# NazirNayal8/RbA

Hardware: AMD Instinct MI355X
Metric: images/sec @1024x2048 Swin-B-1dl (RbA inference hot path) (higher is better)
Workload: dtype f32 (f16x3 split-MFMA GEMMs, fp32 accumulate)

## Files before the change

### include/rba_hip.h

```cpp
#ifndef RBA_HIP_H
#define RBA_HIP_H

#include <stdint.h>

#ifdef __cplusplus
extern "C" {
#endif

int rba_hip_version(void);

int rba_set_concurrent_streams(int n);

int rba_reduce_f32(const float* mask, const float* cls_prob, float* rba, float* sem_seg, int32_t* argmax,
                   int Q, int K, int64_t HW, int score_mode, void* stream);

int rba_reduce_ws_f32(const float* mask, const float* cls_prob, float* rba, float* sem_seg, int32_t* argmax, int Q, int K,
                      int64_t HW, int score_mode, void* workspace, void* stream);

int rba_reduce_up4_f32(const float* mask_lowres, const float* cls_prob, float* rba, float* sem_seg,
                       int32_t* argmax, int Q, int K, int h, int w, int crop_h, int crop_w, int score_mode, void* stream);

int rba_reduce_bwd_workspace_f32(int Q, int K, int64_t HW, int64_t* bytes);
int rba_reduce_bwd_f32(const float* mask, const float* cls_prob, const float* grad_score,
                       float* grad_mask , float* grad_prob ,
                       int Q, int K, int64_t HW, int score_mode,
                       void* workspace, int64_t workspace_bytes, void* stream);

int rba_resample_bilinear_f32(const float* in, const float* add, float* out, int C, int h, int w, int H, int W,
                              void* stream);

int rba_ms_deform_attn_fwd_f32(const float* value, const int64_t* spatial_shapes, const int64_t* level_start_index,
                               const float* sampling_loc, const float* attn_weight, float* out,
                               int N, int S, int M, int D, int L, int Lq, int P, void* stream);
int rba_ms_deform_attn_fwd_f64(const double* value, const int64_t* spatial_shapes, const int64_t* level_start_index,
                               const double* sampling_loc, const double* attn_weight, double* out,
                               int N, int S, int M, int D, int L, int Lq, int P, void* stream);

int rba_ms_deform_attn_bwd_f32(const float* value, const int64_t* spatial_shapes, const int64_t* level_start_index,
                               const float* sampling_loc, const float* attn_weight, const float* grad_out,
                               float* grad_value, float* grad_sampling_loc, float* grad_attn_weight,
                               int N, int S, int M, int D, int L, int Lq, int P, void* stream);
int rba_ms_deform_attn_bwd_f64(const double* value, const int64_t* spatial_shapes, const int64_t* level_start_index,
                               const double* sampling_loc, const double* attn_weight, const double* grad_out,
                               double* grad_value, double* grad_sampling_loc, double* grad_attn_weight,
                               int N, int S, int M, int D, int L, int Lq, int P, void* stream);

int rba_msda_prepare_f32(const float* raw, const float* reference_points, const int64_t* spatial_shapes, float* loc, float* attw,
                         int64_t rows, int M, int L, int P, void* stream);

int rba_msda_fused_f32(const float* value, const int64_t* spatial_shapes, const int64_t* level_start_index, const float* raw,
                       const float* reference_points, float* out, int N, int S, int M, int D, int L, int Lq, int P, void* stream);

int64_t rba_masked_xattn_workspace_bytes(int B, int Q, int S, int nH);
int rba_masked_xattn_f32(const float* q, const float* k, const float* v, const float* mask_logits, float* out,
                         float* workspace, int B, int Q, int S, int nH, int hd, void* stream);

int rba_mask_logits_f32(const float* embed, const float* feat, float* out, int B, int Q, int C, int64_t N,
                        void* stream);
int rba_mask_logits_f16x3_f32(const float* embed, const float* feat, float* out, int B, int Q, int C, int64_t N,
                              void* stream);

int rba_mask_logits_bwd_workspace_f32(int B, int Q, int C, int64_t N, int64_t* bytes);
int rba_mask_logits_bwd_f32(const float* embed, const float* feat, const float* grad_out,
                            float* grad_embed , float* grad_feat ,
                            int B, int Q, int C, int64_t N, void* workspace, int64_t workspace_bytes, void* stream);

int rba_point_sample_f32(const float* planes, const int64_t* plane_index , const float* coords, float* out,
                         int64_t num_planes, int N, int h, int w, int P, int shared_coords, void* stream);

int rba_mask_point_loss_fwd_f32(const float* pred_masks, const int64_t* plane_index, const float* coords, const float* labels,
                                float* sums, float* losses, int64_t num_planes, int N, int h, int w, int P, float num_masks, void* stream);
int rba_mask_point_loss_bwd_f32(const float* pred_masks, const int64_t* plane_index, const float* coords, const float* labels,
                                const float* sums, const float* grad_loss_mask , const float* grad_loss_dice ,
                                float* grad_masks, int64_t num_planes, int N, int h, int w, int P, float num_masks, void* stream);

int rba_match_cost_workspace_f32(int Q, int T, int P, int64_t* bytes);
int rba_match_cost_f32(const float* pred_masks, const float* tgt_masks, const float* coords, const float* cls_prob, const int64_t* tgt_ids,
                       float* cost, int Q, int T, int P, int h, int w, int H, int W, int K1, float w_mask, float w_class, float w_dice,
                       void* workspace, int64_t workspace_bytes, void* stream);

int rba_swin_window_attn_f32(const float* qkv, const float* qkv_bias, const float* bias, const float* bias_frag,
                             float* out, int B, int H, int W, int nH, int hd, int ws, int shift, void* stream);
int64_t rba_swin_bias_fragments_elems(int nH, int ws);
int rba_swin_bias_fragments_f32(const float* bias, float* frag, int nH, int ws, void* stream);

int64_t rba_group_norm_workspace_bytes(int B, int C, int HW, int G);
int rba_group_norm_f32(const float* x, const float* gamma, const float* beta, float* y, float* workspace,
                       int B, int C, int HW, int G, float eps, int relu, void* stream);

int64_t rba_group_norm_nhwc_workspace_bytes(int B, int P, int C, int G);
int rba_group_norm_nhwc_f32(const float* x, const float* gamma, const float* beta, float* y, float* workspace, int B, int P, int C,
                            int G, float eps, int relu, void* stream);
int rba_resample_bilinear_nhwc_f32(const float* in, const float* add, float* out, int C, int h, int w, int H, int W, void* stream);

int rba_add_layer_norm_f32(const float* x, const float* t, const float* t_bias, const float* gamma, const float* beta,
                           float* sum_out, float* y, int64_t rows, int C, float eps, void* stream);

int rba_merge_layer_norm_f32(const float* x, const float* gamma, const float* beta, float* y, int B, int H, int W, int Cin, float eps,
                             void* stream);

int rba_skinny_linear_f32(const float* x, const float* weight, const float* bias, float* out, int M, int N, int K,
                          int relu, void* stream);
int rba_skinny_linear_add_f32(const float* x, const float* x_add, int add_cols, const float* weight, const float* bias, float* out,
                              int M, int N, int K, int relu, int seg_n, void* stream);

int rba_split_weight_bf16x3(const float* weight, void* packed, int N, int K, void* stream);
int rba_split_linear_f32(const float* x, const void* weight_packed, const float* bias, float* out, int64_t M, int N, int K,
                         int act, void* stream);

int rba_split_weight_f16x2(const float* weight, void* packed, int N, int K, void* stream);
int rba_split_linear_f16x3_f32(const float* x, const void* weight_packed, const float* bias, float* out, int64_t M, int N, int K,
                               int act, void* stream);
int rba_split_linear_f16x3_res_f32(const float* x, const void* weight_packed, const float* bias, const float* residual, float* out,
                                   int64_t M, int N, int K, void* stream);

int rba_add_layer_norm_frag_f32(const float* x, const float* t, const float* t_bias, const float* gamma, const float* beta,
                                float* sum_out, void* y_frag, int64_t rows, int C, float eps, void* stream);
int rba_split_linear_f16x3_frag_f32(const void* x_frag, const void* weight_packed, const float* bias, const float* residual, float* out,
                                    int64_t M, int N, int K, int act, void* stream);
int rba_swin_window_attn_split_out_f32(const float* qkv, const float* qkv_bias, const float* bias_frag, void* out_frag, int B, int H, int W,
                                       int nH, int hd, int ws, int shift, void* stream);
int rba_swin_attn_block_supported(int C, int ws);
int64_t rba_swin_attn_block_weight_bytes(int C);
int rba_swin_attn_block_pack_f32(const float* qkv_weight, const float* proj_weight, void* image, int C, void* stream);
int rba_swin_attn_block_f32(float* x, float* y2, const float* norm1_weight, const float* norm1_bias, float eps1, const void* weight_image,
                            const float* qkv_bias, const float* bias_frag, const float* proj_bias, const float* norm2_weight,
                            const float* norm2_bias, float eps2, int B, int H, int W, int C, int ws, int shift, void* stream);
int rba_swin_attn_qkv_supported(int C, int ws);
int rba_swin_attn_qkv_split_out_f32(const float* x, void* out_frag, const float* norm1_weight, const float* norm1_bias, float eps1,
                                    const void* weight_image, const float* qkv_bias, const float* bias_frag, int B, int H, int W, int C, int ws,
                                    int shift, void* stream);
int rba_resample_bilinear_nhwc_split_out_f32(const float* in, const float* add, void* out_frag, int C, int h, int w, int H, int W,
                                             int64_t row0, void* stream);

int rba_resample_bilinear_nhwc_gn_f32(const float* in, const float* in_mr, const float* in_gamma, const float* in_beta, int in_relu,
                                      const float* add, const float* add_mr, const float* add_gamma, const float* add_beta, void* out,
                                      int split_out, int C, int G, int h, int w, int H, int W, int64_t row0, void* stream);
int rba_group_norm_nhwc_stats_f32(const float* x, float* mr, float* workspace, int B, int P, int C, int G, float eps, void* stream);
int rba_conv3x3_nhwc_f16x3_split_in_f32(const void* x_frag, const void* weight_packed, const float* bias, float* out, int B, int H, int W,
                                        int C, int N, void* stream);
int rba_swin_mlp_fused_f16x3_f32(const float* x, const void* w1_packed, const float* b1, const void* w2_packed, const float* b2,
                                 const float* residual, float* out, int64_t M, int C, int HID, void* stream);
int rba_swin_mlp_fused_ln_f16x3_f32(float* x, const float* norm_weight, const float* norm_bias, float eps, const void* w1_packed, const float* b1,
                                    const void* w2_packed, const float* b2, int64_t M, int C, int HID, void* stream);
int rba_split_linear_f16x3_gelu_split_out(const void* x, int x_is_split, const void* weight_packed, const float* bias, void* out_frag,
                                          int64_t M, int N, int K, void* stream);

int rba_split_linear_nchw_out_f32(const float* x, const void* weight_packed, const float* bias, float* out, int64_t M, int N,
                                  int K, int rows_per_image, void* stream);

int rba_split_linear_nchw_out_f16x3_f32(const float* x, const void* weight_packed, const float* bias, float* out, int64_t M, int N, int K,
                                        int rows_per_image, void* stream);

int rba_split_linear_nchw_out_gn_f16x3_f32(const float* x, const float* mr, const float* gamma, const float* beta, int G, int relu,
                                           const void* weight_packed, const float* bias, float* out, int64_t M, int N, int K,
                                           int rows_per_image, void* stream);

int rba_conv3x3_nhwc_f32(const float* x, const void* weight_packed, const float* bias, float* out, int B, int H, int W, int C,
                         int N, void* stream);

int rba_conv3x3_nhwc_f16x3_f32(const float* x, const void* weight_packed, const float* bias, float* out, int B, int H, int W, int C,
                               int N, void* stream);

int rba_split_linear_f16x3_gn_moments_f32(const float* x, const void* weight_packed, const float* bias, float* out, int64_t M, int N, int K,
                                          int rows_per_image, int G, float* moments, void* stream);
int rba_conv3x3_nhwc_f16x3_split_in_gn_moments_f32(const void* x_frag, const void* weight_packed, const float* bias, float* out, int B, int H,
                                                   int W, int C, int N, int G, float* moments, void* stream);
int rba_group_norm_nhwc_merge_f32(const float* moments, float* mr, int B, int G, int splits, float eps, void* stream);

int rba_patch_im2col_u8(const uint8_t* image, float* out, int h, int w, int Hp, int Wp, const float* mean, const float* std, void* stream);
int rba_patch_im2col_f32(const float* image, float* out, int h, int w, int Hp, int Wp, const float* mean, const float* std, void* stream);

int rba_gaussian_blur_f32(const float* in, float* out, int H, int W, int kernel_size, float sigma, void* stream);

int rba_quad_mean_f32(const float* v, float* out, int64_t rows, int S, void* stream);
int rba_softmax_drop_last_f32(const float* logits, float* prob, int64_t rows, int K1, void* stream);

int rba_threshold_u8(const float* score, uint8_t* out, int64_t n, float threshold, void* stream);
int rba_morph3x3_u8(const uint8_t* in, uint8_t* out, int H, int W, int dilate, void* stream);
int rba_ccl4_roots_i32(const uint8_t* mask, int32_t* roots, int H, int W, void* stream);

int rba_bn_relu_conv1x1_f32(const float* x, const float* scale, const float* shift, const float* weight, const float* bias, float* out,
                            int B, int C, int O, int64_t P, void* stream);
int rba_resample_bilinear_ac_f32(const float* x, float* out, int C, int h, int w, int H, int W, void* stream);

typedef struct {
  const float* x_add;
  const void* packed;
  const float* bias;
  float* out;
  int N;
  int ld_out;
  int act;
} rba_token_linear_problem;
int rba_token_linear_pack_f16x2(const float* weight, void* packed, int N, int K, void* stream);
int rba_token_linear_f32(const float* x, const float* x_add, const void* packed, const float* bias, const float* residual,
                         const float* ln_weight, const float* ln_bias, float ln_eps, float* out, int64_t M, int N, int K, int act,
                         void* stream);
int rba_token_linear_multi_f32(const float* x, const rba_token_linear_problem* problems, int n_problems, int64_t M, int K, void* stream);

#ifdef __cplusplus
}
#endif
#endif
```

### rba_amd/_lib.py

```python
import ctypes
import os

_HERE = os.path.dirname(os.path.abspath(__file__))
LIB_PATH = os.environ.get("RBA_HIP_LIB") or os.path.join(_HERE, "csrc", "librba_hip.so")
KNOBS_LIB_PATH = os.path.join(_HERE, "csrc", "librba_hip_knobs.so")

_i = ctypes.c_int
_i64 = ctypes.c_int64
_vp = ctypes.c_void_p

SIGNATURES = {
    "rba_hip_version": [],
    "rba_set_concurrent_streams": [_i],
    "rba_reduce_f32": [_vp, _vp, _vp, _vp, _vp, _i, _i, _i64, _i, _vp],
    "rba_reduce_ws_f32": [_vp, _vp, _vp, _vp, _vp, _i, _i, _i64, _i, _vp, _vp],
    "rba_reduce_up4_f32": [_vp, _vp, _vp, _vp, _vp, _i, _i, _i, _i, _i, _i, _i, _vp],
    "rba_reduce_bwd_workspace_f32": [_i, _i, _i64, _vp],
    "rba_reduce_bwd_f32": [_vp, _vp, _vp, _vp, _vp, _i, _i, _i64, _i, _vp, _i64, _vp],
    "rba_resample_bilinear_f32": [_vp, _vp, _vp, _i, _i, _i, _i, _i, _vp],
    "rba_ms_deform_attn_fwd_f32": [_vp, _vp, _vp, _vp, _vp, _vp, _i, _i, _i, _i, _i, _i, _i, _vp],
    "rba_ms_deform_attn_fwd_f64": [_vp, _vp, _vp, _vp, _vp, _vp, _i, _i, _i, _i, _i, _i, _i, _vp],
    "rba_ms_deform_attn_bwd_f32": [_vp, _vp, _vp, _vp, _vp, _vp, _vp, _vp, _vp, _i, _i, _i, _i, _i, _i, _i, _vp],
    "rba_ms_deform_attn_bwd_f64": [_vp, _vp, _vp, _vp, _vp, _vp, _vp, _vp, _vp, _i, _i, _i, _i, _i, _i, _i, _vp],
    "rba_msda_prepare_f32": [_vp, _vp, _vp, _vp, _vp, _i64, _i, _i, _i, _vp],
    "rba_resample_bilinear_nhwc_gn_f32": [_vp, _vp, _vp, _vp, _i, _vp, _vp, _vp, _vp, _vp, _i, _i, _i, _i, _i, _i, _i, _i64, _vp],
    "rba_group_norm_nhwc_stats_f32": [_vp, _vp, _vp, _i, _i, _i, _i, ctypes.c_float, _vp],
    "rba_msda_fused_f32": [_vp, _vp, _vp, _vp, _vp, _vp, _i, _i, _i, _i, _i, _i, _i, _vp],
    "rba_masked_xattn_workspace_bytes": [_i, _i, _i, _i],
    "rba_masked_xattn_f32": [_vp, _vp, _vp, _vp, _vp, _vp, _i, _i, _i, _i, _i, _vp],
    "rba_mask_logits_f32": [_vp, _vp, _vp, _i, _i, _i, _i64, _vp],
    "rba_mask_logits_f16x3_f32": [_vp, _vp, _vp, _i, _i, _i, _i64, _vp],
    "rba_mask_logits_bwd_workspace_f32": [_i, _i, _i, _i64, _vp],
    "rba_mask_logits_bwd_f32": [_vp, _vp, _vp, _vp, _vp, _i, _i, _i, _i64, _vp, _i64, _vp],
    "rba_point_sample_f32": [_vp, _vp, _vp, _vp, _i64, _i, _i, _i, _i, _i, _vp],
    "rba_mask_point_loss_fwd_f32": [_vp, _vp, _vp, _vp, _vp, _vp, _i64, _i, _i, _i, _i, ctypes.c_float, _vp],
    "rba_mask_point_loss_bwd_f32": [_vp, _vp, _vp, _vp, _vp, _vp, _vp, _vp, _i64, _i, _i, _i, _i, ctypes.c_float, _vp],
    "rba_match_cost_workspace_f32": [_i, _i, _i, _vp],
    "rba_match_cost_f32": [_vp, _vp, _vp, _vp, _vp, _vp, _i, _i, _i, _i, _i, _i, _i, _i, ctypes.c_float, ctypes.c_float, ctypes.c_float, _vp, _i64, _vp],
    "rba_swin_window_attn_f32": [_vp, _vp, _vp, _vp, _vp, _i, _i, _i, _i, _i, _i, _i, _vp],
    "rba_swin_window_attn_split_out_f32": [_vp, _vp, _vp, _vp, _i, _i, _i, _i, _i, _i, _i, _vp],
    "rba_swin_bias_fragments_elems": [_i, _i],
    "rba_swin_attn_block_supported": [_i, _i],
    "rba_swin_attn_block_weight_bytes": [_i],
    "rba_swin_attn_qkv_supported": [_i, _i],
    "rba_swin_attn_qkv_split_out_f32": [_vp, _vp, _vp, _vp, ctypes.c_float, _vp, _vp, _vp, _i, _i, _i, _i, _i, _i, _vp],
    "rba_swin_attn_block_pack_f32": [_vp, _vp, _vp, _i, _vp],
    "rba_swin_attn_block_f32": [_vp, _vp, _vp, _vp, ctypes.c_float, _vp, _vp, _vp, _vp, _vp, _vp, ctypes.c_float, _i, _i, _i, _i, _i, _i, _vp],
    "rba_swin_bias_fragments_f32": [_vp, _vp, _i, _i, _vp],
    "rba_skinny_linear_f32": [_vp, _vp, _vp, _vp, _i, _i, _i, _i, _vp],
    "rba_skinny_linear_add_f32": [_vp, _vp, _i, _vp, _vp, _vp, _i, _i, _i, _i, _i, _vp],
    "rba_split_weight_bf16x3": [_vp, _vp, _i, _i, _vp],
    "rba_split_linear_f32": [_vp, _vp, _vp, _vp, _i64, _i, _i, _i, _vp],
    "rba_split_weight_f16x2": [_vp, _vp, _i, _i, _vp],
    "rba_split_linear_f16x3_f32": [_vp, _vp, _vp, _vp, _i64, _i, _i, _i, _vp],
    "rba_split_linear_f16x3_res_f32": [_vp, _vp, _vp, _vp, _vp, _i64, _i, _i, _vp],
    "rba_split_linear_f16x3_frag_f32": [_vp, _vp, _vp, _vp, _vp, _i64, _i, _i, _i, _vp],
    "rba_swin_mlp_fused_f16x3_f32": [_vp, _vp, _vp, _vp, _vp, _vp, _vp, _i64, _i, _i, _vp],
    "rba_swin_mlp_fused_ln_f16x3_f32": [_vp, _vp, _vp, ctypes.c_float, _vp, _vp, _vp, _vp, _i64, _i, _i, _vp],
    "rba_split_linear_f16x3_gelu_split_out": [_vp, _i, _vp, _vp, _vp, _i64, _i, _i, _vp],
    "rba_split_linear_nchw_out_f32": [_vp, _vp, _vp, _vp, _i64, _i, _i, _i, _vp],
    "rba_split_linear_nchw_out_f16x3_f32": [_vp, _vp, _vp, _vp, _i64, _i, _i, _i, _vp],
    "rba_split_linear_f16x3_gn_moments_f32": [_vp, _vp, _vp, _vp, _i64, _i, _i, _i, _i, _vp, _vp],
    "rba_conv3x3_nhwc_f16x3_split_in_gn_moments_f32": [_vp, _vp, _vp, _vp, _i, _i, _i, _i, _i, _i, _vp, _vp],
    "rba_group_norm_nhwc_merge_f32": [_vp, _vp, _i, _i, _i, ctypes.c_float, _vp],
    "rba_split_linear_nchw_out_gn_f16x3_f32": [_vp, _vp, _vp, _vp, _i, _i, _vp, _vp, _vp, _i64, _i, _i, _i, _vp],
    "rba_conv3x3_nhwc_f32": [_vp, _vp, _vp, _vp, _i, _i, _i, _i, _i, _vp],
    "rba_conv3x3_nhwc_f16x3_f32": [_vp, _vp, _vp, _vp, _i, _i, _i, _i, _i, _vp],
    "rba_conv3x3_nhwc_f16x3_split_in_f32": [_vp, _vp, _vp, _vp, _i, _i, _i, _i, _i, _vp],
    "rba_resample_bilinear_nhwc_split_out_f32": [_vp, _vp, _vp, _i, _i, _i, _i, _i, _i64, _vp],
    "rba_patch_im2col_u8": [_vp, _vp, _i, _i, _i, _i, _vp, _vp, _vp],
    "rba_patch_im2col_f32": [_vp, _vp, _i, _i, _i, _i, _vp, _vp, _vp],
    "rba_group_norm_nhwc_workspace_bytes": [_i, _i, _i, _i],
    "rba_group_norm_nhwc_f32": [_vp, _vp, _vp, _vp, _vp, _i, _i, _i, _i, ctypes.c_float, _i, _vp],
    "rba_resample_bilinear_nhwc_f32": [_vp, _vp, _vp, _i, _i, _i, _i, _i, _vp],
    "rba_bn_relu_conv1x1_f32": [_vp, _vp, _vp, _vp, _vp, _vp, _i, _i, _i, _i64, _vp],
    "rba_resample_bilinear_ac_f32": [_vp, _vp, _i, _i, _i, _i, _i, _vp],
    "rba_gaussian_blur_f32": [_vp, _vp, _i, _i, _i, ctypes.c_float, _vp],
    "rba_quad_mean_f32": [_vp, _vp, _i64, _i, _vp],
    "rba_softmax_drop_last_f32": [_vp, _vp, _i64, _i, _vp],
    "rba_threshold_u8": [_vp, _vp, _i64, ctypes.c_float, _vp],
    "rba_morph3x3_u8": [_vp, _vp, _i, _i, _i, _vp],
    "rba_ccl4_roots_i32": [_vp, _vp, _i, _i, _vp],
    "rba_add_layer_norm_f32": [_vp, _vp, _vp, _vp, _vp, _vp, _vp, _i64, _i, ctypes.c_float, _vp],
    "rba_add_layer_norm_frag_f32": [_vp, _vp, _vp, _vp, _vp, _vp, _vp, _i64, _i, ctypes.c_float, _vp],
    "rba_merge_layer_norm_f32": [_vp, _vp, _vp, _vp, _i, _i, _i, _i, ctypes.c_float, _vp],
    "rba_group_norm_workspace_bytes": [_i, _i, _i, _i],
    "rba_group_norm_f32": [_vp, _vp, _vp, _vp, _vp, _i, _i, _i, _i, ctypes.c_float, _i, _vp],
    "rba_token_linear_pack_f16x2": [_vp, _vp, _i, _i, _vp],
    "rba_token_linear_f32": [_vp, _vp, _vp, _vp, _vp, _vp, _vp, ctypes.c_float, _vp, _i64, _i, _i, _i, _vp],
    "rba_token_linear_multi_f32": [_vp, _vp, _i, _i64, _i, _vp],
}

class TokenLinearProblem(ctypes.Structure):
    _fields_ = [("x_add", ctypes.c_void_p), ("packed", ctypes.c_void_p), ("bias", ctypes.c_void_p), ("out", ctypes.c_void_p),
                ("N", ctypes.c_int), ("ld_out", ctypes.c_int), ("act", ctypes.c_int)]


EXPECTED_ABI = 191

_lib = None


class RbaHipError(RuntimeError):
    pass


def load():
    global _lib
    if _lib is not None:
        return _lib
    _lib = _open(LIB_PATH)
    return _lib


_handles = {}


def _open(path):
    if path in _handles:
        return _handles[path]
    import torch
    if not os.path.exists(path):
        raise RbaHipError(
            f"{path} not found: build it with `python -m rba_amd.csrc.build` (hipcc --offload-arch=gfx950; --knobs for the knobs build). "
            "rba_amd has no CPU or PyTorch fallback for its HIP kernels.")
    lib = ctypes.CDLL(path)
    for name, argtypes in SIGNATURES.items():
        try:
            fn = getattr(lib, name)
        except AttributeError as e:
            raise RbaHipError(f"{path} does not export {name}; rebuild it") from e
        fn.argtypes = argtypes
        fn.restype = ctypes.c_int64 if name.endswith(("_bytes", "_elems")) else ctypes.c_int
    abi = int(lib.rba_hip_version())
    if abi != EXPECTED_ABI:
        raise RbaHipError(f"{path} has ABI version {abi}, these bindings are written for {EXPECTED_ABI}; rebuild it "
                          "(python -m rba_amd.csrc.build)")
    _handles[path] = lib
    return lib


class use_library:

    def __init__(self, path):
        self.path = path

    def __enter__(self):
        global _lib
        self.prev = _lib
        _lib = _open(self.path)
        return _lib

    def __exit__(self, *exc):
        global _lib
        _lib = self.prev
        return False


def knob(name):
    try:
        return ctypes.c_int.in_dll(load(), name)
    except ValueError as e:
        raise RbaHipError(f"{name} is a compile-time constant in the product library: run on the knobs build (RBA_HIP_LIB={KNOBS_LIB_PATH} or "
                          "rba_amd._lib.use_library(KNOBS_LIB_PATH); python -m rba_amd.csrc.build --knobs)") from e


def hip_error_string(code: int) -> str:
    try:
        hip = ctypes.CDLL("libamdhip64.so")
        hip.hipGetErrorString.restype = ctypes.c_char_p
        hip.hipGetErrorString.argtypes = [ctypes.c_int]
        return hip.hipGetErrorString(code).decode()
    except Exception:
        return "hipError"


def check(code: int, what: str):
    if code != 0:
        raise RbaHipError(f"{what} failed: hipError {code} ({hip_error_string(code)})")
```

### rba_amd/csrc/split_linear_dma.hip

```cpp
#include "split_linear_h3.h"
#include "split_linear_h3q.h"
#include "mlp_fused_h3.h"

RBA_KNOB(rba_k6_variant, 0);
RBA_KNOB_DEFINE(rba_k6_stagger, 0);
RBA_KNOB_DEFINE(rba_k6_occ, 2);
RBA_KNOB_DEFINE(rba_k6_rs_min_k, 512);
RBA_KNOB_DEFINE(rba_k6_ks, 0);
RBA_KNOB_DEFINE(rba_k6_rs, 0);
extern "C" __attribute__((visibility("hidden"))) int rba_concurrent_streams_hint = 1;

extern "C" int rba_set_concurrent_streams(int n) {
  const int prev = rba_concurrent_streams_hint;
  rba_concurrent_streams_hint = n >= 1 ? n : 1;
  return prev;
}

extern "C" int rba_split_linear_f32(const float* x, const void* weight_planes, const float* bias, float* out, int64_t M, int N,
                                    int K, int act, void* stream) {
  RBA_CHECK_ARG(N >= 1 && act >= 0 && act <= 2);
  RBA_GEMM_PROLOGUE(M, K, x && weight_planes && out, x, weight_planes, out);
  const u32x4_t* wp = reinterpret_cast<const u32x4_t*>(weight_planes);
  hipStream_t st = (hipStream_t)stream;
  return rba_gemm_status((tiles128(M, N) < 256 && N > 64 && (K >> 5) >= 2) ? launch_v5_act<1, 2, 2, 2, 4>(act, x, wp, bias, out, M, N, K, 2, st)
                                                                           : launch_v4_act<1, 4, 1, 2, 4>(act, x, wp, bias, out, M, N, K, st));
}

extern "C" int rba_split_weight_f16x2(const float* weight, void* packed, int N, int K, void* stream) {
  RBA_CHECK_ARG(N >= 0 && K >= 0 && (K % 32) == 0);
  if (N == 0 || K == 0) return 0;
  RBA_CHECK_ARG(weight && packed && (((uintptr_t)weight | (uintptr_t)packed) & 15) == 0);
  rba_begin();
  const int64_t total = (int64_t)((N + 127) >> 7) * (K >> 4) * 256;
  const unsigned grid = (unsigned)((total + 255) / 256 < 4096 ? (total + 255) / 256 : 4096);
  hipLaunchKernelGGL(split_weight_f16x2_kernel, dim3(grid), dim3(256), 0, (hipStream_t)stream, weight, reinterpret_cast<u32x4_t*>(packed),
                     N, K);
  return rba_launch_status();
}

extern "C" int rba_split_linear_f16x3_f32(const float* x, const void* weight_packed, const float* bias, float* out, int64_t M, int N,
                                          int K, int act, void* stream) {
  RBA_CHECK_ARG(N >= 1 && act >= 0 && act <= 2);
  RBA_GEMM_PROLOGUE(M, K, x && weight_packed && out, x, weight_packed, out);
  const H3Args a{x, reinterpret_cast<const u32x4_t*>(weight_packed), bias, out, M, N, K, (hipStream_t)stream};
  return rba_gemm_status(h3_with_act(act, [&](auto ACT) { return launch_h3_rows<ACT, 0>(a); }));
}

extern "C" int rba_conv3x3_nhwc_f16x3_f32(const float* x, const void* weight_packed, const float* bias, float* out, int B, int H, int W,
                                          int C, int N, void* stream) {
  RBA_CHECK_ARG(B >= 0 && H >= 1 && W >= 1 && N >= 1);
  const int64_t M = (int64_t)B * H * W;
  RBA_GEMM_PROLOGUE(M, C, x && weight_packed && out && M * C < (int64_t)1 << 30, x, weight_packed, out);
  H3Args a{x, reinterpret_cast<const u32x4_t*>(weight_packed), bias, out, M, N, 9 * C, (hipStream_t)stream};
  a.cs = ConvShape{H, W, C};
  return rba_gemm_status((tiles128(M, N) >= 256 || N <= 64) ? launch_h3l<0, 4, H3_CONV>(a) : launch_h3l<0, 2, H3_CONV>(a));
}

extern "C" int rba_split_linear_f16x3_gn_moments_f32(const float* x, const void* weight_packed, const float* bias, float* out, int64_t M, int N, int K,
                                                     int rows_per_image, int G, float* moments, void* stream) {
  RBA_CHECK_ARG(N >= 128 && (N % 128) == 0 && K <= 256 && G >= 1 && (N % G) == 0 && rows_per_image >= 128);
  const int cpg = N / G;
  RBA_CHECK_ARG((cpg == 4 || cpg == 8 || cpg == 16 || cpg == 32) && (rows_per_image % 128) == 0);
  RBA_GEMM_PROLOGUE(M, K, x && weight_packed && out && moments && (M % rows_per_image) == 0, x, weight_packed, out);
  H3Args a{x, reinterpret_cast<const u32x4_t*>(weight_packed), bias, out, M, N, K, (hipStream_t)stream};
  a.gm = GnMoments{moments, G, cpg, rows_per_image};
  return rba_gemm_status(launch_h3l<0, 4, H3_GNM>(a));
}

extern "C" int rba_conv3x3_nhwc_f16x3_split_in_gn_moments_f32(const void* x_frag, const void* weight_packed, const float* bias, float* out, int B, int H,
                                                              int W, int C, int N, int G, float* moments, void* stream) {
  RBA_CHECK_ARG(B >= 0 && H >= 1 && W >= 1 && C <= 2048 && N >= 128 && (N % 128) == 0 && G >= 1 && (N % G) == 0);
  const int cpg = N / G;
  const int64_t P = (int64_t)H * W, M = (int64_t)B * P;
  RBA_CHECK_ARG((cpg == 4 || cpg == 8 || cpg == 16 || cpg == 32) && (P % 128) == 0 && P < (int64_t)1 << 31);
  RBA_GEMM_PROLOGUE(M, C, x_frag && weight_packed && out && moments, x_frag, weight_packed, out, bias);
  H3Args a{x_frag, reinterpret_cast<const u32x4_t*>(weight_packed), bias, out, M, N, 9 * C, (hipStream_t)stream};
  a.cs = ConvShape{H, W, C};
  a.gm = GnMoments{moments, G, cpg, (int)P};
  return rba_gemm_status(launch_h3p_by_shape<0, H3_PRE | H3_CONVP | H3_GNM, H3_RS2>(a));
}

extern "C" int rba_split_linear_f16x3_res_f32(const float* x, const void* weight_packed, const float* bias, const float* residual, float* out,
                                              int64_t M, int N, int K, void* stream) {
  RBA_CHECK_ARG(N >= 1);
  RBA_GEMM_PROLOGUE(M, K, x && weight_packed && residual && out, x, weight_packed, out, residual);
  H3Args a{x, reinterpret_cast<const u32x4_t*>(weight_packed), bias, out, M, N, K, (hipStream_t)stream};
  a.res = residual;
  return rba_gemm_status(launch_h3_rows<0, H3_RES>(a));
}

extern "C" int rba_split_linear_f16x3_frag_f32(const void* x_frag, const void* weight_packed, const float* bias, const float* residual,
                                               float* out, int64_t M, int N, int K, int act, void* stream) {
  RBA_CHECK_ARG(N >= 1 && act >= 0 && act <= 2 && !(residual && act));
  RBA_GEMM_PROLOGUE(M, K, x_frag && weight_packed && out, x_frag, weight_packed, out, residual);
  const u32x4_t* wp = reinterpret_cast<const u32x4_t*>(weight_packed);
  hipStream_t st = (hipStream_t)stream;
  int rc;
  const bool sub_tiles = rba_k6_variant == 2 || (rba_k6_variant == 0 && tiles128(M, N) < (residual ? 256 : 200));
  if (sub_tiles && h3q_supported(M, N, K)) {
    rc = residual ? launch_h3q<H3Q_RES, 0>(x_frag, wp, bias, residual, out, M, N, K, st)
                  : h3_with_act(act, [&](auto ACT) { return launch_h3q<H3Q_F32, ACT>(x_frag, wp, bias, nullptr, out, M, N, K, st); });
  } else {
    constexpr unsigned GEOMETRIES = H3_OCC1 | H3_KS2 | H3_RS2;
    H3Args a{x_frag, wp, bias, out, M, N, K, st};
    a.res = residual;
    a.stagger = rba_k6_stagger;
    rc = residual ? launch_h3p_by_shape<0, H3_PRE | H3_RES, GEOMETRIES>(a)
                  : h3_with_act(act, [&](auto ACT) { return launch_h3p_by_shape<ACT, H3_PRE, GEOMETRIES>(a); });
  }
  return rba_gemm_status(rc);
}

extern "C" int rba_split_linear_f16x3_gelu_split_out(const void* x, int x_is_split, const void* weight_packed, const float* bias,
                                                     void* out_frag, int64_t M, int N, int K, void* stream) {
  RBA_CHECK_ARG(N >= 32 && (N % 32) == 0);
  RBA_GEMM_PROLOGUE(M, K, x && weight_packed && out_frag, x, weight_packed, out_frag, bias);
  const u32x4_t* wp = reinterpret_cast<const u32x4_t*>(weight_packed);
  hipStream_t st = (hipStream_t)stream;
  int rc;
  if (x_is_split && rba_k6_variant >= 100 && h3q_supported(M, N, K)) {
    switch (rba_k6_variant - 100) {
#define H3Q_PROBE(P) case P: rc = launch_h3q<H3Q_SPLIT, 1, P>(x, wp, bias, nullptr, out_frag, M, N, K, st); break;
      H3Q_PROBE(1) H3Q_PROBE(2) H3Q_PROBE(4) H3Q_PROBE(8) H3Q_PROBE(16) H3Q_PROBE(3) H3Q_PROBE(7) H3Q_PROBE(15) H3Q_PROBE(31) H3Q_PROBE(5)
#undef H3Q_PROBE
      default: rc = launch_h3q<H3Q_SPLIT, 1>(x, wp, bias, nullptr, out_frag, M, N, K, st);
    }
  } else if (x_is_split && h3q_supported(M, N, K) &&
             (rba_k6_variant == 2 || (rba_k6_variant == 0 && K >= 768 && tiles128(M, N) > 512 && !h3p_use_rs2(M, N, K))))
    rc = launch_h3q<H3Q_SPLIT, 1>(x, wp, bias, nullptr, out_frag, M, N, K, st);
  else {
    H3Args a{x, wp, bias, out_frag, M, N, K, st};
    a.stagger = rba_k6_stagger;
    rc = x_is_split ? launch_h3p_by_shape<1, H3_PRE | H3_FOUT, H3_OCC1 | H3_RS2>(a) : launch_h3p_by_shape<1, H3_FOUT, H3_OCC1>(a);
  }
  return rba_gemm_status(rc);
}

extern "C" int rba_conv3x3_nhwc_f16x3_split_in_f32(const void* x_frag, const void* weight_packed, const float* bias, float* out, int B, int H,
                                                   int W, int C, int N, void* stream) {
  RBA_CHECK_ARG(B >= 0 && H >= 1 && W >= 1 && C <= 2048 && N >= 1);
  const int64_t M = (int64_t)B * H * W;
  RBA_GEMM_PROLOGUE(M, C, x_frag && weight_packed && out, x_frag, weight_packed, out, bias);
  H3Args a{x_frag, reinterpret_cast<const u32x4_t*>(weight_packed), bias, out, M, N, 9 * C, (hipStream_t)stream};
  a.cs = ConvShape{H, W, C};
  return rba_gemm_status(launch_h3p_by_shape<0, H3_PRE | H3_CONVP, H3_RS2>(a));
}

extern "C" int rba_swin_mlp_fused_f16x3_f32(const float* x, const void* w1_packed, const float* b1, const void* w2_packed, const float* b2,
                                            const float* residual, float* out, int64_t M, int C, int HID, void* stream) {
  RBA_CHECK_ARG(C == 128 && HID >= 64 && (HID % 32) == 0);
  RBA_GEMM_PROLOGUE(M, C, x && w1_packed && b1 && w2_packed && residual && out, x, w1_packed, w2_packed, residual, out, b1);
  return rba_gemm_status(launch_mlp_fused(x, reinterpret_cast<const u32x4_t*>(w1_packed), b1, reinterpret_cast<const u32x4_t*>(w2_packed), b2, residual, out, M,
                                          HID, (hipStream_t)stream));
}

extern "C" int rba_swin_mlp_fused_ln_f16x3_f32(float* x, const float* norm_weight, const float* norm_bias, float eps, const void* w1_packed, const float* b1,
                                               const void* w2_packed, const float* b2, int64_t M, int C, int HID, void* stream) {
  RBA_CHECK_ARG(C == 128 && HID >= 64 && (HID % 32) == 0);
  RBA_GEMM_PROLOGUE(M, C, x && norm_weight && norm_bias && w1_packed && b1 && w2_packed, x, w1_packed, w2_packed, b1, norm_weight, norm_bias);
  return rba_gemm_status(launch_mlp_fused(x, reinterpret_cast<const u32x4_t*>(w1_packed), b1, reinterpret_cast<const u32x4_t*>(w2_packed), b2, x, x, M, HID,
                                          (hipStream_t)stream, norm_weight, norm_bias, eps));
}

extern "C" int rba_split_linear_nchw_out_f16x3_f32(const float* x, const void* weight_packed, const float* bias, float* out, int64_t M, int N,
                                                   int K, int rows_per_image, void* stream) {
  RBA_CHECK_ARG(N >= 1 && rows_per_image >= 1);
  RBA_GEMM_PROLOGUE(M, K, x && weight_packed && out && (M % rows_per_image) == 0, x, weight_packed, out);
  H3Args a{x, reinterpret_cast<const u32x4_t*>(weight_packed), bias, out, M, N, K, (hipStream_t)stream};
  a.rows_per_image = rows_per_image;
  return rba_gemm_status(h3_wide(M, N) ? launch_h3l<0, 4, H3_NCHW>(a) : launch_h3l<0, 2, H3_NCHW>(a));
}
```

### rba_amd/csrc/split_linear_gnf.hip

```cpp
#include "split_linear_h3.h"

extern "C" int rba_split_linear_nchw_out_gn_f16x3_f32(const float* x, const float* mr, const float* gamma, const float* beta, int G, int relu,
                                                      const void* weight_packed, const float* bias, float* out, int64_t M, int N, int K,
                                                      int rows_per_image, void* stream) {
  RBA_CHECK_ARG(N >= 1 && rows_per_image >= 1 && G >= 1 && (K % G) == 0 && ((K / G) % 4) == 0);
  RBA_GEMM_PROLOGUE(M, K, x && mr && gamma && beta && weight_packed && out && (M % rows_per_image) == 0 && (rows_per_image % 128) == 0, x, weight_packed, out,
                    gamma, beta);
  H3Args a{x, reinterpret_cast<const u32x4_t*>(weight_packed), bias, out, M, N, K, (hipStream_t)stream};
  a.rows_per_image = rows_per_image;
  a.gn = GnFold{mr, gamma, beta, G, K / G, relu ? 1 : 0};
  return rba_gemm_status(h3_wide(M, N) ? launch_h3l<0, 4, H3_NCHW | H3_GNF>(a) : launch_h3l<0, 2, H3_NCHW | H3_GNF>(a));
}
```

### rba_amd/csrc/split_linear_h3.h

```cpp
#pragma once
#include <type_traits>

#include "split_linear_dma.h"

RBA_KNOB_EXTERN(rba_k6_stagger, 0);

namespace {

typedef _Float16 f16x8_t __attribute__((ext_vector_type(8)));

__device__ __forceinline__ void split_h3(const f32x4 u, const f32x4 v, f16x8_t& h, f16x8_t& l) {
  const float x[8] = {u.x, u.y, u.z, u.w, v.x, v.y, v.z, v.w};
  u32x4_t hp, lp;
#pragma unroll
  for (int i = 0; i < 4; ++i) {
    uint32_t a, r;
    rba_split_f16x2(x[2 * i], x[2 * i + 1], a, r);
    hp[i] = a;
    lp[i] = r;
  }
  h = __builtin_bit_cast(f16x8_t, hp);
  l = __builtin_bit_cast(f16x8_t, lp);
}

__device__ __forceinline__ f32x2 gelu_erf2(f32x2 v) {
  const f32x2 a = {fabsf(v.x), fabsf(v.y)};
  const f32x2 d = a * 0.23164189f + 1.0f;
  const f32x2 t = {__builtin_amdgcn_rcpf(d.x), __builtin_amdgcn_rcpf(d.y)};
  f32x2 p = t * 0.5307027145f + -0.7265760135f;
  p = p * t + 0.7107068705f;
  p = p * t + -0.142248368f;
  p = p * t + 0.127414796f;
  const f32x2 u = a * 0.8493218003f;
  const f32x2 s = -u * u;
  const f32x2 ex = {__builtin_amdgcn_exp2f(s.x), __builtin_amdgcn_exp2f(s.y)};
  const f32x2 q = p * t * ex;
  const f32x2 r = (v + a) * 0.5f;
  return r - a * q;
}

#ifndef RBA_H3_HELPERS_ONLY
__global__ void split_weight_f16x2_kernel(const float* __restrict__ w, u32x4_t* __restrict__ packed, int N, int K) {
  const int S = K >> 4;
  const int64_t total = (int64_t)((N + 127) >> 7) * S * 256;
  for (int64_t i = (int64_t)blockIdx.x * blockDim.x + threadIdx.x; i < total; i += (int64_t)gridDim.x * blockDim.x) {
    const int slot = (int)(i & 1), r = (int)((i >> 1) & 127);
    const int64_t ts = i >> 8;
    const int s = (int)(ts % S), nt = (int)(ts / S);
    const int h = slot ^ ((r >> 3) & 1);
    const int k0 = 32 * (s >> 1) + 16 * h + 8 * (s & 1);
    const int n = nt * 128 + r;
    f16x8_t p0, p1;
    if (n < N) {
      const f32x4* src = reinterpret_cast<const f32x4*>(w + (int64_t)n * K + k0);
      split_h3(src[0], src[1], p0, p1);
    } else {
#pragma unroll
      for (int e = 0; e < 8; ++e) p0[e] = p1[e] = (_Float16)0.f;
    }
    u32x4_t* dst = packed + ts * 512 + r * 2 + slot;
    dst[0] = __builtin_bit_cast(u32x4_t, p0);
    dst[256] = __builtin_bit_cast(u32x4_t, p1);
  }
}

#endif

struct GnMoments {
  float* ws;
  int G, cpg, P;
};
template <int ACT, int CT, int PROBE, bool RES, bool GNM = false>
__device__ __forceinline__ void h3_epilogue(const f32x16_t (&accm)[CT], const f32x16_t (&accl)[CT], const float* __restrict__ bias,
                                            float* C, const float* R, int M, int N, int m0, int n0, int BM, int BN, int wave, int l31,
                                            int lh, GnMoments gm = GnMoments{nullptr, 1, 1, 128}, float* sh = nullptr) {
  const bool interior = m0 + BM <= M && n0 + BN <= N;
  if (GNM) __syncthreads();
#pragma unroll
  for (int j = 0; j < CT; ++j) {
    const int col = n0 + 32 * j + l31;
    const float bv = (bias && col < N) ? bias[col] : 0.f;
    const int rbase = m0 + 32 * wave + 4 * lh;
    float* dst = C + (int64_t)rbase * N + col;
    f32x16_t res;
    if (RES) {
      const float* src = R + (int64_t)rbase * N + col;
#pragma unroll
      for (int r = 0; r < 16; ++r) {
        const int ro = 8 * (r >> 2) + (r & 3);
        res[r] = (interior || (col < N && rbase + ro < M)) ? src[(int64_t)ro * N] : 0.f;
      }
    }
    f32x16_t v;
#pragma unroll
    for (int r = 0; r < 16; r += 2) {
      f32x2 y = (f32x2){accl[j][r], accl[j][r + 1]} * 0.00048828125f + (f32x2){accm[j][r], accm[j][r + 1]};
      if (RES) y = (f32x2){res[r], res[r + 1]} + y;
      y = y + bv;
      if (ACT == 1) y = gelu_erf2(y);
      if (ACT == 2) y = (f32x2){rba_relu(y.x), rba_relu(y.y)};
      v[r] = y.x;
      v[r + 1] = y.y;
    }
    if (GNM) {
      float sm = 0.f, sq = 0.f;
#pragma unroll
      for (int r = 0; r < 16; ++r) {
        sm += v[r];
        sq = fmaf(v[r], v[r], sq);
      }
      sm += __shfl_xor(sm, 32, 64);
      sq += __shfl_xor(sq, 32, 64);
      for (int o = 1; o < gm.cpg; o <<= 1) {
        sm += __shfl_xor(sm, o, 64);
        sq += __shfl_xor(sq, o, 64);
      }
      if (lh == 0 && (l31 & (gm.cpg - 1)) == 0) {
        float* d = sh + ((wave * (BN / gm.cpg)) + (32 * j + l31) / gm.cpg) * 2;
        d[0] = sm;
        d[1] = sq;
      }
    }
    if (PROBE & 4) {
      float sum = 0.f;
#pragma unroll
      for (int r = 0; r < 16; ++r) sum += v[r];
      if (sum == 1234.5f) dst[0] = sum;
    } else if (interior) {
#pragma unroll
      for (int r = 0; r < 16; ++r) dst[(int64_t)(8 * (r >> 2) + (r & 3)) * N] = v[r];
    } else if (col < N) {
#pragma unroll
      for (int r = 0; r < 16; ++r) {
        const int ro = 8 * (r >> 2) + (r & 3);
        if (rbase + ro < M) dst[(int64_t)ro * N] = v[r];
      }
    }
  }
  if (GNM) {
    __syncthreads();
    const int gpt = BN / gm.cpg, t = 64 * wave + 32 * lh + l31;
    if (t < gpt && m0 < M) {
      double ds = 0, dq = 0;
#pragma unroll
      for (int w = 0; w < 4; ++w) {
        ds += (double)sh[(w * gpt + t) * 2];
        dq += (double)sh[(w * gpt + t) * 2 + 1];
      }
      const double n = 128.0 * gm.cpg, mean = ds / n, m2 = dq - ds * mean;
      const int b = m0 / gm.P, sp = (m0 - b * gm.P) >> 7, splits = gm.P >> 7, g = n0 / gm.cpg + t;
      float* o = gm.ws + (((int64_t)b * gm.G + g) * splits + sp) * 3;
      o[0] = (float)n;
      o[1] = (float)mean;
      o[2] = (float)(m2 > 0 ? m2 : 0);
    }
  }
}

#ifndef RBA_H3_HELPERS_ONLY
template <int CT>
__device__ __forceinline__ void h3_epilogue_nchw(const f32x16_t (&accm)[CT], const f32x16_t (&accl)[CT], const float* __restrict__ bias, float* C,
                                                 int M, int N, int P, int m0, int n0, int wave, int l31, int lh) {
  const bool vec = (P & 3) == 0;
#pragma unroll
  for (int j = 0; j < CT; ++j) {
    const int col = n0 + 32 * j + l31;
    if (col >= N) continue;
    const float bv = bias ? bias[col] : 0.f;
#pragma unroll
    for (int q = 0; q < 4; ++q) {
      const int row = m0 + 32 * wave + 8 * q + 4 * lh;
      if (row >= M) continue;
      f32x4 v;
#pragma unroll
      for (int i = 0; i < 4; ++i) v[i] = fmaf(accl[j][4 * q + i], 0.00048828125f, accm[j][4 * q + i]) + bv;
      if (vec && row + 3 < M) {
        const int b = row / P, p = row - b * P;
        *reinterpret_cast<f32x4*>(C + ((int64_t)b * N + col) * P + p) = v;
      } else {
#pragma unroll
        for (int i = 0; i < 4; ++i)
          if (row + i < M) {
            const int b = (row + i) / P, p = row + i - b * P;
            C[((int64_t)b * N + col) * P + p] = v[i];
          }
      }
    }
  }
}

enum : unsigned {
  H3_TIMING = 1u << 0,
  H3_RES = 1u << 1,
  H3_GNM = 1u << 2,
  H3_CONV = 1u << 3,
  H3_NCHW = 1u << 4,
  H3_GNF = 1u << 5,
  H3_PRE = 1u << 6,
  H3_FOUT = 1u << 7,
  H3_CONVP = 1u << 8,
  H3_OCC1 = 1u << 9,
  H3_KS2 = 1u << 10,
  H3_RS2 = 1u << 11,
  H3_PROBE_SHIFT = 16,
};
constexpr unsigned h3_probe(int p) { return (unsigned)p << H3_PROBE_SHIFT; }
constexpr int h3_probe_of(unsigned form) { return (int)(form >> H3_PROBE_SHIFT); }
constexpr unsigned H3_FORMS = H3_TIMING | H3_RES, H3L_FORMS = H3_FORMS | H3_GNM | H3_CONV | H3_NCHW | H3_GNF,
                   H3P_FORMS = H3_FORMS | H3_GNM | H3_PRE | H3_FOUT | H3_CONVP | H3_OCC1 | H3_KS2 | H3_RS2;
constexpr bool h3_form_within(unsigned form, unsigned allowed) { return (form & ~allowed & ((1u << H3_PROBE_SHIFT) - 1)) == 0; }
constexpr int h3_tile_rows(unsigned form) { return (form & H3_RS2) ? 256 : 128; }
constexpr int h3_threads(unsigned form) { return (form & (H3_KS2 | H3_RS2)) ? 512 : 256; }
constexpr int h3_occupancy(unsigned form) { return (form & (H3_KS2 | H3_RS2 | H3_OCC1)) ? 1 : 2; }

template <int ACT, int CT, unsigned FORM = 0>
__global__ __launch_bounds__(256, 2) void split_linear_h3_kernel(const float* __restrict__ A, const u32x4_t* __restrict__ Wp,
                                                                const float* __restrict__ bias, float* C, int M, int N,
                                                                int K, int MT, int NT, unsigned long long* dbg = nullptr,
                                                                const float* R = nullptr) {
  static_assert(h3_form_within(FORM, H3_FORMS), "split_linear_h3_kernel: H3_TIMING, H3_RES, h3_probe()");
  constexpr int PROBE = h3_probe_of(FORM);
  constexpr bool TIMING = FORM & H3_TIMING, RES = FORM & H3_RES;
  unsigned long long tm[4];
  if (TIMING) tm[0] = wall_clock64();
  constexpr int BM = 128, BN = 32 * CT;
  constexpr int SUBW = 4 * BN;
  constexpr int BLK = 2 * SUBW;
  constexpr int UPL = BLK / 256;
  static_assert(BLK % 256 == 0 && 128 % BN == 0, "tile width");
  __shared__ __attribute__((aligned(16))) u32x4_t lds[2 * BLK];

  const int tid = threadIdx.x, lane = tid & 63;
  const int wave = __builtin_amdgcn_readfirstlane(tid >> 6);
  int bid = blockIdx.x;
  const int nb = MT * NT;
  if ((nb & 7) == 0) bid = (bid & 7) * (nb >> 3) + (bid >> 3);
  const int mt = bid / NT, nt = bid - mt * NT;
  const int m0 = mt * BM, n0 = nt * BN;
  const int NB = K >> 5, S16 = K >> 4;
  const int l31 = lane & 31, lh = lane >> 5;

  constexpr int QSTEP = (CT == 4) ? 256 : 512;
  const char* wbase = reinterpret_cast<const char*>(Wp + (int64_t)(n0 >> 7) * S16 * 512 + (n0 & 127) * 2);
  uint32_t woff;
  {
    const int g = tid / SUBW, rem = tid - g * SUBW, p = rem / (2 * BN), rr = rem - p * (2 * BN);
    woff = (uint32_t)(g * 512 + p * 256 + rr) * 16u;
  }
  int row = m0 + 32 * wave + l31;
  row = (row < M ? row : M - 1) - m0;
  const char* xbase = reinterpret_cast<const char*>(A + (int64_t)m0 * K);
  const uint32_t xoff = ((uint32_t)row * (uint32_t)K + 16u * lh) * 4u;

  f32x16_t accm[CT], accl[CT];
#pragma unroll
  for (int j = 0; j < CT; ++j)
#pragma unroll
    for (int r = 0; r < 16; ++r) accm[j][r] = accl[j][r] = 0.f;

  u32x4_t wr[UPL];
  f32x4 xr[2][4];
  const int last = NB - 1;
  auto wload = [&](int c, u32x4_t (&r)[UPL]) {
    const char* src = wbase + (int64_t)(c < last ? c : last) * 16384;
#pragma unroll
    for (int q = 0; q < UPL; ++q) r[q] = *reinterpret_cast<const u32x4_t*>(src + q * (QSTEP * 16) + woff);
  };
  auto xload = [&](int c, f32x4 (&r)[4]) {
    const char* src = xbase + (c < last ? c : last) * 128;
#pragma unroll
    for (int q = 0; q < 4; ++q) r[q] = *reinterpret_cast<const f32x4*>(src + q * 16 + xoff);
  };
  wload(0, wr);
  xload(0, xr[0]);
  xload(1, xr[1]);
#pragma unroll
  for (int q = 0; q < UPL; ++q) lds[tid + 256 * q] = wr[q];
  wload(1, wr);
  asm volatile("s_waitcnt lgkmcnt(0)\n\ts_barrier" ::: "memory");

  const int fb = l31 * 2 + (lh ^ ((l31 >> 3) & 1));
  if (TIMING) tm[1] = wall_clock64();
  auto block = [&](int b, const u32x4_t* img, u32x4_t* nxt, f32x4 (&xc)[4]) {
    if (!(PROBE & 32)) {
#pragma unroll
      for (int q = 0; q < UPL; ++q) nxt[tid + 256 * q] = wr[q];
    }
    if (!(PROBE & 1)) wload(b + 2, wr);
    f16x8_t ah[2], al[2];
    if (PROBE & 16) {
      ah[0] = __builtin_bit_cast(f16x8_t, xc[0]); al[0] = __builtin_bit_cast(f16x8_t, xc[1]);
      ah[1] = __builtin_bit_cast(f16x8_t, xc[2]); al[1] = __builtin_bit_cast(f16x8_t, xc[3]);
    } else {
      split_h3(xc[0], xc[1], ah[0], al[0]);
      split_h3(xc[2], xc[3], ah[1], al[1]);
    }
    if (!(PROBE & 2)) xload(b + 2, xc);
#pragma unroll
    for (int g = 0; g < 2; ++g) {
      __builtin_amdgcn_sched_barrier(0);
      f16x8_t bh[CT], bl[CT];
#pragma unroll
      for (int j = 0; j < CT; ++j) {
        const u32x4_t* im = (PROBE & 8) ? lds : img;
        bh[j] = __builtin_bit_cast(f16x8_t, im[g * SUBW + fb + 64 * j]);
        bl[j] = __builtin_bit_cast(f16x8_t, im[g * SUBW + fb + 2 * BN + 64 * j]);
      }
#pragma unroll
      for (int j = 0; j < CT; ++j) accm[j] = __builtin_amdgcn_mfma_f32_32x32x16_f16(ah[g], bh[j], accm[j], 0, 0, 0);
#pragma unroll
      for (int j = 0; j < CT; ++j) accl[j] = __builtin_amdgcn_mfma_f32_32x32x16_f16(ah[g], bl[j], accl[j], 0, 0, 0);
#pragma unroll
      for (int j = 0; j < CT; ++j) accl[j] = __builtin_amdgcn_mfma_f32_32x32x16_f16(al[g], bh[j], accl[j], 0, 0, 0);
    }
    if (!(PROBE & 64)) asm volatile("s_waitcnt lgkmcnt(0)\n\ts_barrier" ::: "memory");
  };
  int b = 0;
  if (NB & 1) {
    block(0, lds, lds + BLK, xr[0]);
    b = 1;
    for (; b < NB; b += 2) {
      block(b, lds + BLK, lds, xr[1]);
      block(b + 1, lds, lds + BLK, xr[0]);
    }
  } else {
    for (; b < NB; b += 2) {
      block(b, lds, lds + BLK, xr[0]);
      block(b + 1, lds + BLK, lds, xr[1]);
    }
  }

  if (TIMING) tm[2] = wall_clock64();
  h3_epilogue<ACT, CT, PROBE, RES>(accm, accl, bias, C, R, M, N, m0, n0, BM, BN, wave, l31, lh);
  if (TIMING && tid == 0) {
    tm[3] = wall_clock64();
    unsigned xcc;
    asm volatile("s_getreg_b32 %0, hwreg(HW_REG_XCC_ID)" : "=s"(xcc));
    unsigned hw;
    asm volatile("s_getreg_b32 %0, hwreg(HW_REG_HW_ID)" : "=s"(hw));
#pragma unroll
    for (int i = 0; i < 4; ++i) dbg[6 * blockIdx.x + i] = tm[i];
    dbg[6 * blockIdx.x + 4] = xcc;
    dbg[6 * blockIdx.x + 5] = hw;
  }
}

struct ConvShape {
  int H, W, Cin;
};
struct GnFold {
  const float* mr;
  const float* gamma;
  const float* beta;
  int G, cpg, relu;
};
template <int ACT, int CT, unsigned FORM = 0>
__global__ __launch_bounds__(256, 2) void split_linear_h3l_kernel(const float* __restrict__ A, const u32x4_t* __restrict__ Wp,
                                                                 const float* __restrict__ bias, float* C, int M, int N,
                                                                 int K, int MT, int NT, unsigned long long* dbg = nullptr,
                                                                 ConvShape cs = ConvShape{0, 0, 0}, const float* R = nullptr, int rows_per_image = 0,
                                                                 GnFold gn = GnFold{nullptr, nullptr, nullptr, 1, 1, 0},
                                                                 GnMoments gm = GnMoments{nullptr, 1, 1, 128}) {
  static_assert(h3_form_within(FORM, H3L_FORMS), "split_linear_h3l_kernel: H3_TIMING, H3_RES, H3_GNM, H3_CONV, H3_NCHW, H3_GNF, h3_probe()");
  constexpr int PROBE = h3_probe_of(FORM);
  constexpr bool TIMING = FORM & H3_TIMING, CONV = FORM & H3_CONV, RES = FORM & H3_RES, NCHW = FORM & H3_NCHW, GNF = FORM & H3_GNF, GNM = FORM & H3_GNM;
  unsigned long long tm[4];
  if (TIMING) tm[0] = wall_clock64();
  constexpr int BM = 128, BN = 32 * CT;
  constexpr int SUBW = 4 * BN;
  constexpr int BLK = 2 * SUBW;
  constexpr int UPL = BLK / 256;
  constexpr int XBLK = BM * 8;
  constexpr int BUF = BLK + XBLK;
  static_assert(BLK % 256 == 0 && 128 % BN == 0, "tile width");
  __shared__ __attribute__((aligned(16))) u32x4_t lds[2 * BUF];

  const int tid = threadIdx.x, lane = tid & 63;
  const int wave = __builtin_amdgcn_readfirstlane(tid >> 6);
  int bid = blockIdx.x;
  const int nb = MT * NT;
  if ((nb & 7) == 0) bid = (bid & 7) * (nb >> 3) + (bid >> 3);
  const int mt = bid / NT, nt = bid - mt * NT;
  const int m0 = mt * BM, n0 = nt * BN;
  const int NB = K >> 5, S16 = K >> 4;
  const int l31 = lane & 31, lh = lane >> 5;

  constexpr int QSTEP = (CT == 4) ? 256 : 512;
  const char* wbase = reinterpret_cast<const char*>(Wp + (int64_t)(n0 >> 7) * S16 * 512 + (n0 & 127) * 2);
  uint32_t woff;
  {
    const int g = tid / SUBW, rem = tid - g * SUBW, p = rem / (2 * BN), rr = rem - p * (2 * BN);
    woff = (uint32_t)(g * 512 + p * 256 + rr) * 16u;
  }
  const char* xbase = reinterpret_cast<const char*>(CONV ? A : A + (int64_t)m0 * K);
  uint32_t xoff[4];
  int py[4], px[4];
#pragma unroll
  for (int q = 0; q < 4; ++q) {
    int r = m0 + (tid >> 3) + 32 * q;
    r = r < M ? r : M - 1;
    if (CONV) {
      const int pix = r % (cs.H * cs.W);
      py[q] = pix / cs.W;
      px[q] = pix - py[q] * cs.W;
      xoff[q] = ((uint32_t)r * (uint32_t)cs.Cin + 4u * (tid & 7)) * 4u;
    } else {
      xoff[q] = ((uint32_t)(r - m0) * (uint32_t)K + 4u * (tid & 7)) * 4u;
    }
  }
  const int xdst = BLK + (tid >> 3) * 8 + ((tid & 7) ^ ((tid >> 4) & 7));
  const int frow = 32 * wave + l31;
  const int fa = BLK + frow * 8, fsw = (frow >> 1) & 7;

  f32x16_t accm[CT], accl[CT];
#pragma unroll
  for (int j = 0; j < CT; ++j)
#pragma unroll
    for (int r = 0; r < 16; ++r) accm[j][r] = accl[j][r] = 0.f;

  u32x4_t wr[UPL];
  f32x4 xr[4];
  f32x4 gga = {0.f, 0.f, 0.f, 0.f}, gbe = {0.f, 0.f, 0.f, 0.f};
  float gmean = 0.f, grstd = 0.f;
  const float* gmr = GNF ? gn.mr + (int64_t)(m0 / rows_per_image) * gn.G * 2 : nullptr;
  const int last = NB - 1;
  auto gload = [&](int c) {
    const int cc = c < last ? c : last;
    const char* ws = wbase + (int64_t)cc * 16384;
#pragma unroll
    for (int q = 0; q < UPL; ++q) wr[q] = *reinterpret_cast<const u32x4_t*>(ws + q * (QSTEP * 16) + woff);
    if (GNF) {
      const int ch = cc * 32 + 4 * (tid & 7);
      gga = *reinterpret_cast<const f32x4*>(gn.gamma + ch);
      gbe = *reinterpret_cast<const f32x4*>(gn.beta + ch);
      const int g = ch / gn.cpg;
      gmean = gmr[2 * g];
      grstd = gmr[2 * g + 1];
    }
    if (CONV) {
      const int k0 = cc * 32, tap = k0 / cs.Cin, ch0 = k0 - tap * cs.Cin;
      const int ky = tap / 3, dy = ky - 1, dx = tap - 3 * ky - 1;
      const int delta = ((dy * cs.W + dx) * cs.Cin + ch0) * 4;
#pragma unroll
      for (int q = 0; q < 4; ++q) {
        const bool ok = (unsigned)(py[q] + dy) < (unsigned)cs.H && (unsigned)(px[q] + dx) < (unsigned)cs.W;
        const f32x4 v = *reinterpret_cast<const f32x4*>(xbase + (int64_t)(ok ? delta : ch0 * 4) + xoff[q]);
        xr[q] = ok ? v : (f32x4){0.f, 0.f, 0.f, 0.f};
      }
    } else {
      const char* xs = xbase + cc * 128;
#pragma unroll
      for (int q = 0; q < 4; ++q) xr[q] = *reinterpret_cast<const f32x4*>(xs + xoff[q]);
    }
  };
  f32x4 xst[4];
#if defined(RBA_GNF_DEBUG)
  int gnf_blk = 0;
#endif
  auto lstore = [&](u32x4_t* buf) {
#pragma unroll
    for (int q = 0; q < UPL; ++q) buf[tid + 256 * q] = wr[q];
    if (GNF) {
      f32x4 a, b;
      const float relu_floor = gn.relu ? 0.f : -INFINITY;
      const float poison = (grstd - grstd) + (gmean - gmean);
#pragma unroll
      for (int i = 0; i < 4; ++i) {
        a[i] = gga[i] * grstd;
        b[i] = fmaf(-gmean, a[i], gbe[i]);
      }
#pragma unroll
      for (int q = 0; q < 4; ++q)
#pragma unroll
        for (int i = 0; i < 4; ++i) {
#if defined(RBA_GNF_FORM) && RBA_GNF_FORM == 1
          const float y = fmaf(xr[q][i], a[i], b[i]);
          xst[q][i] = fmaxf(y, relu_floor) + (y - y);
#else
          xst[q][i] = fmaxf(fmaf(xr[q][i], a[i], b[i]), relu_floor) + poison;
#endif
        }
#if defined(RBA_GNF_DEBUG)
      if (dbg && gnf_blk < NB) {
        float* d = reinterpret_cast<float*>(dbg) + (((int64_t)(mt * NT + nt) * NB + gnf_blk) * 256 + tid) * 40;
#pragma unroll
        for (int q = 0; q < 4; ++q) {
          *reinterpret_cast<f32x4*>(d + 4 * q) = xr[q];
          *reinterpret_cast<f32x4*>(d + 16 + 4 * q) = xst[q];
        }
        *reinterpret_cast<f32x4*>(d + 32) = a;
        *reinterpret_cast<f32x4*>(d + 36) = b;
      }
      ++gnf_blk;
#endif
#pragma unroll
      for (int q = 0; q < 4; ++q) buf[xdst + 256 * q] = __builtin_bit_cast(u32x4_t, xst[q]);
    } else {
#pragma unroll
      for (int q = 0; q < 4; ++q) buf[xdst + 256 * q] = __builtin_bit_cast(u32x4_t, xr[q]);
    }
  };
  gload(0);
  lstore(lds);
  gload(1);
  asm volatile("s_waitcnt lgkmcnt(0)\n\ts_barrier" ::: "memory");

  const int fb = l31 * 2 + (lh ^ ((l31 >> 3) & 1));
  if (TIMING) tm[1] = wall_clock64();
  for (int b = 0; b < NB; ++b) {
    const u32x4_t* img = lds + (b & 1) * BUF;
    if (!(PROBE & 32)) lstore(lds + ((b + 1) & 1) * BUF);
    if (!(PROBE & 1)) gload(b + 2);
    f16x8_t ah[2], al[2];
#pragma unroll
    for (int g = 0; g < 2; ++g) {
      const f32x4 u = __builtin_bit_cast(f32x4, img[fa + ((4 * lh + 2 * g) ^ fsw)]);
      const f32x4 v = __builtin_bit_cast(f32x4, img[fa + ((4 * lh + 2 * g + 1) ^ fsw)]);
      if (PROBE & 16) {
        ah[g] = __builtin_bit_cast(f16x8_t, u);
        al[g] = __builtin_bit_cast(f16x8_t, v);
      } else {
        split_h3(u, v, ah[g], al[g]);
      }
    }
#pragma unroll
    for (int g = 0; g < 2; ++g) {
      if (PROBE & 128) __builtin_amdgcn_sched_barrier(0);
      f16x8_t bh[CT], bl[CT];
#pragma unroll
      for (int j = 0; j < CT; ++j) {
        bh[j] = __builtin_bit_cast(f16x8_t, img[g * SUBW + fb + 64 * j]);
        bl[j] = __builtin_bit_cast(f16x8_t, img[g * SUBW + fb + 2 * BN + 64 * j]);
      }
#pragma unroll
      for (int j = 0; j < CT; ++j) accm[j] = __builtin_amdgcn_mfma_f32_32x32x16_f16(ah[g], bh[j], accm[j], 0, 0, 0);
#pragma unroll
      for (int j = 0; j < CT; ++j) accl[j] = __builtin_amdgcn_mfma_f32_32x32x16_f16(ah[g], bl[j], accl[j], 0, 0, 0);
#pragma unroll
      for (int j = 0; j < CT; ++j) accl[j] = __builtin_amdgcn_mfma_f32_32x32x16_f16(al[g], bh[j], accl[j], 0, 0, 0);
    }
    if (!(PROBE & 64)) asm volatile("s_waitcnt lgkmcnt(0)\n\ts_barrier" ::: "memory");
  }

  if (TIMING) tm[2] = wall_clock64();
  if (NCHW) h3_epilogue_nchw<CT>(accm, accl, bias, C, M, N, rows_per_image, m0, n0, wave, l31, lh);
  else h3_epilogue<ACT, CT, PROBE, RES, GNM>(accm, accl, bias, C, R, M, N, m0, n0, BM, BN, wave, l31, lh, gm, reinterpret_cast<float*>(lds));
  if (TIMING && tid == 0) {
    tm[3] = wall_clock64();
#pragma unroll
    for (int i = 0; i < 4; ++i) dbg[6 * blockIdx.x + i] = tm[i];
    dbg[6 * blockIdx.x + 4] = dbg[6 * blockIdx.x + 5] = 0;
  }
}

#endif

template <int ACT, int CT>
__device__ __forceinline__ void h3_epilogue_split(const f32x16_t (&accm)[CT], const f32x16_t (&accl)[CT], const float* __restrict__ bias,
                                                  void* out_frag, int M, int N, int m0, int n0, int wave, int l31, int lh) {
  const int row = m0 + 32 * wave + l31;
  const bool full = m0 + 128 <= M;
  const int NBo = N >> 5;
  char* base = reinterpret_cast<char*>(out_frag) + ((int64_t)((m0 >> 5) + wave) * NBo) * 4096 + l31 * 16 + lh * 1024;
#pragma unroll
  for (int j = 0; j < CT; ++j) {
    const int nj = n0 + 32 * j;
    if (nj >= N) break;
#pragma unroll
    for (int q = 0; q < 4; ++q) {
      const int n = nj + 8 * q + 4 * lh;
      const f32x4 bv = bias ? *reinterpret_cast<const f32x4*>(bias + n) : (f32x4){0.f, 0.f, 0.f, 0.f};
      f32x2 y0 = (f32x2){accl[j][4 * q], accl[j][4 * q + 1]} * 0.00048828125f + (f32x2){accm[j][4 * q], accm[j][4 * q + 1]};
      f32x2 y1 = (f32x2){accl[j][4 * q + 2], accl[j][4 * q + 3]} * 0.00048828125f + (f32x2){accm[j][4 * q + 2], accm[j][4 * q + 3]};
      y0 = y0 + (f32x2){bv.x, bv.y};
      y1 = y1 + (f32x2){bv.z, bv.w};
      if (ACT == 1) {
        y0 = gelu_erf2(y0);
        y1 = gelu_erf2(y1);
      }
      if (ACT == 2) {
        y0 = (f32x2){rba_relu(y0.x), rba_relu(y0.y)};
        y1 = (f32x2){rba_relu(y1.x), rba_relu(y1.y)};
      }
      uint32_t h0, l0, h1, l1;
      rba_split_f16x2(y0.x, y0.y, h0, l0);
      rba_split_f16x2(y1.x, y1.y, h1, l1);
      const auto p0 = __builtin_amdgcn_permlane32_swap(h0, l0, false, false), p1 = __builtin_amdgcn_permlane32_swap(h1, l1, false, false);
      const u32x4_t piece = {p0[0], p1[0], p0[1], p1[1]};
      if (full || row < M) *reinterpret_cast<u32x4_t*>(base + (int64_t)((nj >> 5)) * 4096 + (q & 1) * 2048 + (q >> 1) * 512) = piece;
    }
  }
}

#ifndef RBA_H3_HELPERS_ONLY
template <int ACT, unsigned FORM = 0>
__global__ __launch_bounds__(h3_threads(FORM), h3_occupancy(FORM)) void split_linear_h3p_kernel(const float* __restrict__ A, const u32x4_t* __restrict__ Wp,
                                                                 const float* __restrict__ bias, float* C, int M, int N,
                                                                 int K, int MT, int NT, unsigned long long* dbg = nullptr,
                                                                 const float* R = nullptr, ConvShape cs = ConvShape{0, 0, 0}, int stagger = 0,
                                                                 GnMoments gm = GnMoments{nullptr, 1, 1, 128}) {
  static_assert(h3_form_within(FORM, H3P_FORMS), "split_linear_h3p_kernel: H3_TIMING, H3_RES, H3_GNM, H3_PRE, H3_FOUT, H3_CONVP, H3_OCC1, H3_KS2, H3_RS2, h3_probe()");
  constexpr int PROBE = h3_probe_of(FORM), OCC = (FORM & H3_OCC1) ? 1 : 2, KS = (FORM & H3_KS2) ? 2 : 1, RS = (FORM & H3_RS2) ? 2 : 1;
  constexpr bool TIMING = FORM & H3_TIMING, RES = FORM & H3_RES, PRE = FORM & H3_PRE, FOUT = FORM & H3_FOUT, CONVP = FORM & H3_CONVP, GNM = FORM & H3_GNM;
  static_assert(!GNM || (KS == 1 && !FOUT), "output moments: fp32-row epilogue, one wave set per K");
  unsigned long long tm[4];
  if (TIMING) tm[0] = wall_clock64();
  if (stagger > 0 && blockIdx.x >= 256 && blockIdx.x < 512) {
    const unsigned long long t0 = wall_clock64();
    while (wall_clock64() - t0 < (unsigned long long)stagger) __builtin_amdgcn_s_sleep(8);
  }
  constexpr int CT = 4, BM = 128, BN = 128;
  constexpr int SUBW = 4 * BN, BLK = 2 * SUBW, UPL = BLK / 256;
  __shared__ __attribute__((aligned(16))) u32x4_t lds_all[2 * BLK * KS];

  static_assert(KS * RS <= 2, "K split and row split are alternatives");
  const int tid = threadIdx.x & 255, lane = tid & 63;
  const int ks = KS == 2 ? __builtin_amdgcn_readfirstlane(threadIdx.x >> 8) : 0;
  const int rs = RS == 2 ? __builtin_amdgcn_readfirstlane(threadIdx.x >> 8) : 0;
  const int wtid = RS == 2 ? (int)threadIdx.x : tid;
  constexpr int UPLW = UPL / RS;
  u32x4_t* const lds = lds_all + ks * 2 * BLK;
  const int wave = __builtin_amdgcn_readfirstlane(tid >> 6);
  int bid = blockIdx.x;
  const int nb = MT * NT;
  if ((nb & 7) == 0) bid = (bid & 7) * (nb >> 3) + (bid >> 3);
  const int mt = bid / NT, nt = bid - mt * NT;
  const int m0 = (mt * RS + rs) * BM, n0 = nt * BN;
  const int NB = (K >> 5) / KS, S16 = K >> 4;
  const int l31 = lane & 31, lh = lane >> 5;

  const char* wbase = reinterpret_cast<const char*>(Wp + (int64_t)(n0 >> 7) * S16 * 512);
  const uint32_t woff = (uint32_t)wtid * 16u;
  int row = m0 + 32 * wave + l31;
  row = (row < M ? row : M - 1) - m0;
  const char* xbase = reinterpret_cast<const char*>(A + (int64_t)m0 * K);
  const uint32_t xoff = ((uint32_t)row * (uint32_t)K + 16u * lh) * 4u;

  f32x16_t accm[CT], accl[CT];
#pragma unroll
  for (int j = 0; j < CT; ++j)
#pragma unroll
    for (int r = 0; r < 16; ++r) accm[j][r] = accl[j][r] = 0.f;

  u32x4_t wr[UPLW];
  constexpr bool TWO = OCC == 2 || KS == 2 || RS == 2;
  constexpr bool DEEP = !TWO;
  constexpr bool DIRECT = PRE && TWO;
  f32x4 xr[DEEP ? 2 : 1][4];
  f16x8_t ah[2][2], al[2][2];
  u32x4_t bq[2][4];
  const int last = NB - 1;
  auto bix = [&](int c) { return (c < last ? c : last) * KS + ks; };
  auto wload = [&](int c) {
    const char* src = wbase + (int64_t)bix(c) * 16384;
#pragma unroll
    for (int q = 0; q < UPLW; ++q) wr[q] = *reinterpret_cast<const u32x4_t*>(src + q * (4096 * RS) + woff);
  };
  const int rgrp = min((m0 >> 5) + wave, ((M + 31) >> 5) - 1);
  const char* fbase = reinterpret_cast<const char*>(A) + ((int64_t)rgrp * (K >> 5)) * 4096 + lane * 16;
  auto xload = [&](int c, f32x4 (&d)[4]) {
    if (PRE) {
      const char* src = fbase + bix(c) * 4096;
#pragma unroll
      for (int q = 0; q < 4; ++q) d[q] = *reinterpret_cast<const f32x4*>(src + q * 1024);
      return;
    }
    if (PROBE & 2048) {
      const char* src = xbase + (uint32_t)(32 * wave) * (uint32_t)K * 4u + bix(c) * 4096 + lane * 16;
#pragma unroll
      for (int q = 0; q < 4; ++q) d[q] = *reinterpret_cast<const f32x4*>(src + q * 1024);
      return;
    }
    const char* src = xbase + bix(c) * 128;
#pragma unroll
    for (int q = 0; q < 4; ++q) d[q] = *reinterpret_cast<const f32x4*>(src + q * 16 + xoff);
  };
  const int fb = l31 * 2 + (lh ^ ((l31 >> 3) & 1));
  auto bread = [&](const u32x4_t* img, int j, u32x4_t (&d)[4]) {
    d[0] = img[fb + 64 * j];
    d[1] = img[fb + 2 * BN + 64 * j];
    d[2] = img[SUBW + fb + 64 * j];
    d[3] = img[SUBW + fb + 2 * BN + 64 * j];
  };

  int cpy = 0, cpx = 0, crow = 0, cNB = 1, cinv = 0;
  if (CONVP) {
    crow = min(m0 + 32 * wave + l31, M - 1);
    const int pix = crow % (cs.H * cs.W);
    cpy = pix / cs.W;
    cpx = pix - cpy * cs.W;
    cNB = cs.Cin >> 5;
    cinv = (65536 + cNB - 1) / cNB;
  }
  auto xloadset = [&](int c, int p) {
    if (CONVP) {
      const int cc = bix(c);
      const int tap = (cc * cinv) >> 16, cb = cc - tap * cNB;
      const int ky = (tap * 11) >> 5, dy = ky - 1, dx = tap - 3 * ky - 1;
      const bool ok = (unsigned)(cpy + dy) < (unsigned)cs.H && (unsigned)(cpx + dx) < (unsigned)cs.W;
      const int rs = ok ? crow + dy * cs.W + dx : crow;
      const char* src = reinterpret_cast<const char*>(A) + ((int64_t)(rs >> 5) * cNB + cb) * 4096 + (lh * 32 + (rs & 31)) * 16;
      const f16x8_t z = {0, 0, 0, 0, 0, 0, 0, 0};
      const f16x8_t v0 = *reinterpret_cast<const f16x8_t*>(src), v1 = *reinterpret_cast<const f16x8_t*>(src + 1024);
      const f16x8_t v2 = *reinterpret_cast<const f16x8_t*>(src + 2048), v3 = *reinterpret_cast<const f16x8_t*>(src + 3072);
      ah[p][0] = ok ? v0 : z;
      al[p][0] = ok ? v1 : z;
      ah[p][1] = ok ? v2 : z;
      al[p][1] = ok ? v3 : z;
      return;
    }
    const char* src = fbase + bix(c) * 4096;
    ah[p][0] = *reinterpret_cast<const f16x8_t*>(src);
    al[p][0] = *reinterpret_cast<const f16x8_t*>(src + 1024);
    ah[p][1] = *reinterpret_cast<const f16x8_t*>(src + 2048);
    al[p][1] = *reinterpret_cast<const f16x8_t*>(src + 3072);
  };
  auto psplit = [&](const f32x4 u, const f32x4 v, f16x8_t& h, f16x8_t& l) {
    if (PRE || (PROBE & 512)) {
      h = __builtin_bit_cast(f16x8_t, u);
      l = __builtin_bit_cast(f16x8_t, v);
    } else {
      split_h3(u, v, h, l);
    }
  };
  auto pbread = [&](const u32x4_t* img, int j, u32x4_t (&d)[4]) {
    if (!(PROBE & 1024)) bread(img, j, d);
  };
  wload(0);
  if (DIRECT) xloadset(0, 0);
  else xload(0, xr[0]);
#pragma unroll
  for (int q = 0; q < UPLW; ++q) lds[wtid + 256 * RS * q] = wr[q];
  if (!DIRECT) {
    psplit(xr[0][0], xr[0][1], ah[0][0], al[0][0]);
    psplit(xr[0][2], xr[0][3], ah[0][1], al[0][1]);
  }
  wload(1);
  if (DIRECT) {
  } else if (DEEP) {
    xload(1, xr[DEEP ? 1 : 0]);
    xload(2, xr[0]);
  } else {
    xload(1, xr[0]);
  }
  asm volatile("s_waitcnt lgkmcnt(0)\n\ts_barrier" ::: "memory");
  bread(lds, 0, bq[0]);
  bread(lds, 1, bq[1]);
  unsigned long long cyc = 0;
  if (TIMING) {
    tm[1] = wall_clock64();
    cyc = __builtin_readcyclecounter();
  }

  auto mm = [](const f16x8_t a, const f16x8_t b, const f32x16_t c) {
    return FOUT ? __builtin_amdgcn_mfma_f32_32x32x16_f16(b, a, c, 0, 0, 0) : __builtin_amdgcn_mfma_f32_32x32x16_f16(a, b, c, 0, 0, 0);
  };
#define RBA_MFMA6(J, Q, P)                                                                                              \
  {                                                                                                                     \
    const f16x8_t bh0 = __builtin_bit_cast(f16x8_t, bq[Q][0]), bl0 = __builtin_bit_cast(f16x8_t, bq[Q][1]);             \
    const f16x8_t bh1 = __builtin_bit_cast(f16x8_t, bq[Q][2]), bl1 = __builtin_bit_cast(f16x8_t, bq[Q][3]);             \
    accm[J] = mm(ah[P][0], bh0, accm[J]);                                                                               \
    accl[J] = mm(ah[P][0], bl0, accl[J]);                                                                               \
    accm[J] = mm(ah[P][1], bh1, accm[J]);                                                                               \
    accl[J] = mm(al[P][0], bh0, accl[J]);                                                                               \
    accl[J] = mm(ah[P][1], bl1, accl[J]);                                                                               \
    accl[J] = mm(al[P][1], bh1, accl[J]);                                                                               \
  }
#define RBA_PIPE_MFMA_DSR                                                                                               \
  _Pragma("unroll") for (int i_ = 0; i_ < 4; ++i_) {                                                                    \
    __builtin_amdgcn_sched_group_barrier(0x008, 1, 0);                                                                  \
    __builtin_amdgcn_sched_group_barrier(0x100, 1, 0);                                                                  \
  }                                                                                                                     \
  __builtin_amdgcn_sched_group_barrier(0x008, 2, 0);
#define RBA_PIPE_MFMA_DSR_VALU                                                                                          \
  _Pragma("unroll") for (int i_ = 0; i_ < 4; ++i_) {                                                                    \
    __builtin_amdgcn_sched_group_barrier(0x008, 1, 0);                                                                  \
    __builtin_amdgcn_sched_group_barrier(0x100, 1, 0);                                                                  \
    __builtin_amdgcn_sched_group_barrier(0x002, 4, 0);                                                                  \
  }                                                                                                                     \
  __builtin_amdgcn_sched_group_barrier(0x008, 1, 0);                                                                    \
  __builtin_amdgcn_sched_group_barrier(0x002, 4, 0);                                                                    \
  __builtin_amdgcn_sched_group_barrier(0x008, 1, 0);
#define RBA_XI(P) (DEEP ? (P) ^ 1 : 0)
#define RBA_BLOCK(B, P, CUR, NXT)                                                                                       \
  {                                                                                                                     \
    if (!(PROBE & 256)) { _Pragma("unroll") for (int q = 0; q < UPLW; ++q)(NXT)[wtid + 256 * RS * q] = wr[q]; }        \
    if (!(PROBE & 1)) wload((B) + 2);                                                                                   \
    if (DIRECT) xloadset((B) + 1, (P) ^ 1);                                                                             \
    __builtin_amdgcn_sched_barrier(0);                                                                                  \
    RBA_MFMA6(0, 0, P)                                                                                                  \
    pbread(CUR, 2, bq[0]);                                                                                              \
    if (!DIRECT) psplit(xr[RBA_XI(P)][0], xr[RBA_XI(P)][1], ah[(P) ^ 1][0], al[(P) ^ 1][0]);                                                           \
    RBA_PIPE_MFMA_DSR_VALU                                                                                              \
    __builtin_amdgcn_sched_barrier(0);                                                                                  \
    RBA_MFMA6(1, 1, P)                                                                                                  \
    pbread(CUR, 3, bq[1]);                                                                                              \
    if (!DIRECT) psplit(xr[RBA_XI(P)][2], xr[RBA_XI(P)][3], ah[(P) ^ 1][1], al[(P) ^ 1][1]);                                                           \
    RBA_PIPE_MFMA_DSR_VALU                                                                                              \
    __builtin_amdgcn_sched_barrier(0);                                                                                  \
    if (!DIRECT && !(PROBE & 2)) xload((B) + (DEEP ? 3 : 2), xr[RBA_XI(P)]);                                                                                 \
    RBA_MFMA6(2, 0, P)                                                                                                  \
    if (!(PROBE & 64)) asm volatile("s_waitcnt lgkmcnt(0)\n\ts_barrier" ::: "memory");                               \
    __builtin_amdgcn_sched_barrier(0);                                                                                  \
    RBA_MFMA6(3, 1, P)                                                                                                  \
    pbread(NXT, 0, bq[0]);                                                                                              \
    RBA_PIPE_MFMA_DSR                                                                                                   \
    __builtin_amdgcn_sched_barrier(0);                                                                                  \
    pbread(NXT, 1, bq[1]);                                                                                              \
    __builtin_amdgcn_sched_barrier(0);                                                                                  \
  }
  int b = 0;
  if (NB & 1) {
    RBA_BLOCK(0, 0, lds, lds + BLK)
    for (b = 1; b < NB; b += 2) {
      RBA_BLOCK(b, 1, lds + BLK, lds)
      RBA_BLOCK(b + 1, 0, lds, lds + BLK)
    }
  } else {
    for (; b < NB; b += 2) {
      RBA_BLOCK(b, 0, lds, lds + BLK)
      RBA_BLOCK(b + 1, 1, lds + BLK, lds)
    }
  }
#undef RBA_BLOCK
#undef RBA_XI
#undef RBA_PIPE_MFMA_DSR
#undef RBA_PIPE_MFMA_DSR_VALU
#undef RBA_MFMA6

  if (TIMING) {
    tm[2] = wall_clock64();
    cyc = __builtin_readcyclecounter() - cyc;
  }
  if (KS == 2) {
    f32x4* red = reinterpret_cast<f32x4*>(lds_all);
#pragma unroll
    for (int pass = 0; pass < 2; ++pass) {
      __syncthreads();
      if (ks == 1) {
#pragma unroll
        for (int j = 0; j < CT; ++j)
#pragma unroll
          for (int q = 0; q < 4; ++q) {
            const f32x16_t& a = pass ? accl[j] : accm[j];
            red[(j * 4 + q) * 256 + tid] = (f32x4){a[4 * q], a[4 * q + 1], a[4 * q + 2], a[4 * q + 3]};
          }
      }
      __syncthreads();
      if (ks == 0) {
#pragma unroll
        for (int j = 0; j < CT; ++j)
#pragma unroll
          for (int q = 0; q < 4; ++q) {
            const f32x4 v = red[(j * 4 + q) * 256 + tid];
            f32x16_t& a = pass ? accl[j] : accm[j];
            a[4 * q] += v.x;
            a[4 * q + 1] += v.y;
            a[4 * q + 2] += v.z;
            a[4 * q + 3] += v.w;
          }
      }
    }
    if (ks == 1) return;
  }
  if (FOUT) h3_epilogue_split<ACT, CT>(accm, accl, bias, C, M, N, m0, n0, wave, l31, lh);
  else h3_epilogue<ACT, CT, PROBE, RES, GNM>(accm, accl, bias, C, R, M, N, m0, n0, BM, BN, wave, l31, lh, gm, reinterpret_cast<float*>(lds_all) + rs * 512);
  if (TIMING && tid == 0) {
    tm[3] = wall_clock64();
#pragma unroll
    for (int i = 0; i < 4; ++i) dbg[6 * blockIdx.x + i] = tm[i];
    dbg[6 * blockIdx.x + 4] = cyc;
    dbg[6 * blockIdx.x + 5] = 0;
  }
}

struct H3Args {
  const void* x;
  const u32x4_t* wp;
  const float* bias;
  void* out;
  int64_t M;
  int N, K;
  hipStream_t stream;
  const float* res = nullptr;
  unsigned long long* dbg = nullptr;
  ConvShape cs = ConvShape{0, 0, 0};
  int rows_per_image = 0;
  GnFold gn = GnFold{nullptr, nullptr, nullptr, 1, 1, 0};
  GnMoments gm = GnMoments{nullptr, 1, 1, 128};
  int stagger = 0;
};

inline bool h3_grid(const H3Args& a, int rows, int cols, int& MT, int& NT) {
  const int64_t mt = (a.M + rows - 1) / rows;
  MT = (int)mt;
  NT = (a.N + cols - 1) / cols;
  return mt * NT < (int64_t)1 << 31;
}

template <int ACT, int CT, unsigned FORM = 0>
int launch_h3(const H3Args& a) {
  int MT, NT;
  if (!h3_grid(a, 128, 32 * CT, MT, NT)) return (int)hipErrorInvalidValue;
  hipLaunchKernelGGL((split_linear_h3_kernel<ACT, CT, FORM>), dim3((unsigned)MT * NT), dim3(256), 0, a.stream, reinterpret_cast<const float*>(a.x), a.wp, a.bias,
                     reinterpret_cast<float*>(a.out), (int)a.M, a.N, a.K, MT, NT, a.dbg, a.res);
  return 0;
}

template <int ACT, int CT, unsigned FORM = 0>
int launch_h3l(const H3Args& a) {
  int MT, NT;
  if (!h3_grid(a, 128, 32 * CT, MT, NT)) return (int)hipErrorInvalidValue;
  hipLaunchKernelGGL((split_linear_h3l_kernel<ACT, CT, FORM>), dim3((unsigned)MT * NT), dim3(256), 0, a.stream, reinterpret_cast<const float*>(a.x), a.wp, a.bias,
                     reinterpret_cast<float*>(a.out), (int)a.M, a.N, a.K, MT, NT, a.dbg, a.cs, a.res, a.rows_per_image, a.gn, a.gm);
  return 0;
}

template <int ACT, unsigned FORM = 0>
int launch_h3p(const H3Args& a) {
  int MT, NT;
  if (!h3_grid(a, h3_tile_rows(FORM), 128, MT, NT)) return (int)hipErrorInvalidValue;
  hipLaunchKernelGGL((split_linear_h3p_kernel<ACT, FORM>), dim3((unsigned)MT * NT), dim3(h3_threads(FORM)), 0, a.stream, reinterpret_cast<const float*>(a.x), a.wp,
                     a.bias, reinterpret_cast<float*>(a.out), (int)a.M, a.N, a.K, MT, NT, a.dbg, a.res, a.cs, h3_threads(FORM) == 256 ? a.stagger : 0, a.gm);
  return 0;
}

template <class F>
int h3_with_act(int act, F&& f) {
  if (act == 1) return f(std::integral_constant<int, 1>{});
  if (act == 2) return f(std::integral_constant<int, 2>{});
  return f(std::integral_constant<int, 0>{});
}

inline int64_t tiles128(int64_t M, int N) { return ((M + 127) / 128) * ((N + 127) / 128); }

RBA_KNOB_EXTERN(rba_k6_occ, 2);
inline bool h3p_single_resident(int64_t M, int N) { return rba_k6_occ == 1 && tiles128(M, N) <= 256; }

RBA_KNOB_EXTERN(rba_k6_rs, 0);
RBA_KNOB_EXTERN(rba_k6_rs_min_k, 512);
extern "C" int rba_concurrent_streams_hint;
inline bool h3p_multi_stream() { return rba_k6_rs == 3 || (rba_k6_rs == 0 && rba_concurrent_streams_hint >= 2); }
inline bool h3p_use_rs2(int64_t M, int N, int K) {
  if (rba_k6_rs == 1 || K < rba_k6_rs_min_k) return false;
  const int64_t t = ((M + 255) / 256) * ((N + 127) / 128);
  if (h3p_multi_stream()) return t >= 64;
  if (t < 160) return false;
  if (rba_k6_rs == 2) return true;
  const int64_t last = t % 256;
  return last == 0 || last >= 192;
}

RBA_KNOB_EXTERN(rba_k6_ks, 0);
inline bool h3p_use_ks2(int64_t M, int N, int K) {
  if (rba_k6_ks == 1 || (K & 63) || K < 128) return false;
  if (rba_k6_ks == 2) return true;
  const int64_t t = tiles128(M, N);
  return !h3p_multi_stream() && t > 128 && t <= 256 && K >= 1024;
}

template <int ACT, unsigned FORM, unsigned ALT>
int launch_h3p_by_shape(const H3Args& a) {
  static_assert((ALT & ~(H3_OCC1 | H3_KS2 | H3_RS2)) == 0 && (FORM & (H3_OCC1 | H3_KS2 | H3_RS2)) == 0, "FORM: the base form; ALT: geometry bits");
  if constexpr ((ALT & H3_OCC1) != 0) {
    if (h3p_single_resident(a.M, a.N)) return launch_h3p<ACT, FORM | H3_OCC1>(a);
  }
  if constexpr ((ALT & H3_KS2) != 0) {
    if (h3p_use_ks2(a.M, a.N, a.K)) return launch_h3p<ACT, FORM | H3_KS2>(a);
  }
  if constexpr ((ALT & H3_RS2) != 0) {
    if ((!(FORM & H3_GNM) || (a.M & 255) == 0) && h3p_use_rs2(a.M, a.N, a.K)) return launch_h3p<ACT, FORM | H3_RS2>(a);
  }
  return launch_h3p<ACT, FORM>(a);
}

inline bool h3_wide(int64_t M, int N) { return tiles128(M, N) >= 160 || N <= 64; }
template <int ACT, unsigned FORM>
int launch_h3_rows(const H3Args& a) {
  const bool wide = h3_wide(a.M, a.N);
  if (a.K <= 256) return wide ? launch_h3l<ACT, 4, FORM>(a) : launch_h3l<ACT, 2, FORM>(a);
  return wide ? launch_h3p_by_shape<ACT, FORM, H3_OCC1>(a) : launch_h3<ACT, 2, FORM>(a);
}

inline int h3_forms_compiled_in_every_unit(const H3Args& a) {
  return h3_with_act(0, [&](auto ACT) { return launch_h3p_by_shape<ACT, 0, H3_OCC1>(a); }) | launch_h3p_by_shape<0, H3_RES, H3_OCC1>(a) |
         launch_h3p_by_shape<0, H3_PRE | H3_CONVP, H3_RS2>(a) | launch_h3p_by_shape<0, H3_PRE | H3_CONVP | H3_GNM, H3_RS2>(a) | launch_h3l<0, 4, H3_GNM>(a);
}

#endif

}
```

### rba_amd/maskformer_model.py

```python
import itertools

import torch
import torch.nn as nn
import torch.nn.functional as F

from . import ops
from .h2d import to_device
from .arch import backbone_name as _backbone_name, complete
from .graph_replay import GraphKey, GraphReplay, capture
from .lru import ShapeCache
from .modeling.backbone import resnet as _resnet
from .modeling.backbone import swin as _swin
from .modeling.meta_arch import mask_former_head as _head
from .registry import BACKBONE_REGISTRY, META_ARCH_REGISTRY, SEM_SEG_HEADS_REGISTRY

_REGISTRATIONS = [0]
_EPOCHS = itertools.count(1)


def _registered(*_):
    _REGISTRATIONS[0] += 1


for _hook in (nn.modules.module.register_module_parameter_registration_hook, nn.modules.module.register_module_buffer_registration_hook,
              nn.modules.module.register_module_module_registration_hook):
    _hook(_registered)


def _class_prob(mask_cls):
    if 2 <= mask_cls.shape[-1] <= 64:
        return ops.softmax_drop_last(mask_cls.contiguous())
    return F.softmax(mask_cls, dim=-1)[..., :-1].contiguous()


@META_ARCH_REGISTRY.register()
class MaskFormer(nn.Module):
    def __init__(self, arch, backbone_name=None, head_name="MaskFormerHead"):
        super().__init__()
        a = complete(arch)
        self.arch = a
        self.backbone = BACKBONE_REGISTRY.get(backbone_name or _backbone_name(a))(a)
        self.sem_seg_head = SEM_SEG_HEADS_REGISTRY.get(head_name)(a)
        self.num_queries = a["num_queries"]
        self.size_divisibility = a["size_divisibility"] if a["size_divisibility"] > 0 else self.backbone.size_divisibility
        self.register_buffer("pixel_mean", torch.tensor(a["pixel_mean"], dtype=torch.float32).view(-1, 1, 1), False)
        self.register_buffer("pixel_std", torch.tensor(a["pixel_std"], dtype=torch.float32).view(-1, 1, 1), False)
        self._mean3 = tuple(float(torch.tensor(v, dtype=torch.float32)) for v in a["pixel_mean"])
        self._std3 = tuple(float(torch.tensor(v, dtype=torch.float32)) for v in a["pixel_std"])
        self.fused_front_end = True
        self.graph_replay = "auto"
        self.fused_upsample = True
        self.panoptic_on, self.open_panoptic = bool(a["panoptic_on"]), bool(a["open_panoptic"])
        self.sem_seg_postprocess_before_inference = bool(a["postprocess_before_inference"]) or self.panoptic_on
        self.object_mask_threshold, self.overlap_threshold = float(a["object_mask_threshold"]), float(a["overlap_threshold"])
        self.thing_classes = frozenset(int(c) for c in a["thing_classes"])
        self.eval()

    @property
    def device(self):
        return self.pixel_mean.device

    def preprocess(self, batched_inputs):
        images = [(to_device(x["image"], self.device).float() - self.pixel_mean) / self.pixel_std for x in batched_inputs]
        sizes = [tuple(int(v) for v in im.shape[-2:]) for im in images]
        d = self.size_divisibility
        H = (max(s[0] for s in sizes) + d - 1) // d * d
        W = (max(s[1] for s in sizes) + d - 1) // d * d
        batch = images[0].new_zeros((len(images), images[0].shape[0], H, W))
        for i, im in enumerate(images):
            batch[i, :, : sizes[i][0], : sizes[i][1]] = im
        return batch, sizes

    @torch.no_grad()
    def _predict_outputs(self, batched_inputs):
        pe = getattr(self.backbone, "patch_embed", None)
        if (self.fused_front_end and pe is not None and hasattr(self.backbone, "forward_images") and pe.fused_ok()
                and all(x["image"].dim() == 3 and x["image"].shape[0] == 3 and x["image"].dtype in (torch.uint8, torch.float32)
                        for x in batched_inputs)):
            images = [to_device(x["image"], self.device).contiguous() for x in batched_inputs]
            sizes = [tuple(int(v) for v in im.shape[-2:]) for im in images]
            d = self.size_divisibility
            H = (max(s[0] for s in sizes) + d - 1) // d * d
            W = (max(s[1] for s in sizes) + d - 1) // d * d
            features = self.backbone.forward_images(images, self._mean3, self._std3, H, W)
            return self.sem_seg_head(features), sizes, (H, W)
        batch, sizes = self.preprocess(batched_inputs)
        features = self.backbone(batch)
        return self.sem_seg_head(features), sizes, tuple(batch.shape[-2:])

    @torch.no_grad()
    def predict(self, batched_inputs):
        outputs, sizes, padded = self._predict_outputs(batched_inputs)
        return outputs["pred_logits"], outputs["pred_masks"], sizes, padded

    def finetune_outputs(self, batched_inputs):
        predictor = self.sem_seg_head.predictor
        if not getattr(predictor, "differentiable_heads", False):
            raise ops.RbaHipError("finetune_outputs: set model.sem_seg_head.predictor.differentiable_heads = True first (without it the outputs "
                                  "carry no autograd graph)")
        with torch.no_grad():
            pe = getattr(self.backbone, "patch_embed", None)
            if (self.fused_front_end and pe is not None and hasattr(self.backbone, "forward_images") and pe.fused_ok()
                    and all(x["image"].dim() == 3 and x["image"].shape[0] == 3 and x["image"].dtype in (torch.uint8, torch.float32)
                            for x in batched_inputs)):
                images = [to_device(x["image"], self.device).contiguous() for x in batched_inputs]
                sizes = [tuple(int(v) for v in im.shape[-2:]) for im in images]
                d = self.size_divisibility
                padded = ((max(s[0] for s in sizes) + d - 1) // d * d, (max(s[1] for s in sizes) + d - 1) // d * d)
                features = self.backbone.forward_images(images, self._mean3, self._std3, *padded)
            else:
                batch, sizes = self.preprocess(batched_inputs)
                padded = tuple(batch.shape[-2:])
                features = self.backbone(batch)
            mask_features, _, multi_scale_features = self.sem_seg_head.pixel_decoder.forward_features(features)
        return predictor(multi_scale_features, mask_features), sizes, padded

    def _post(self, mask_cls, mask_pred, image_size, padded, want_sem_seg, want_argmax, score="rba"):
        prob = _class_prob(mask_cls)
        H, W = padded
        exact4 = mask_pred.shape[-2] * 4 == H and mask_pred.shape[-1] * 4 == W
        if self.fused_upsample and exact4 and prob.shape[1] <= 32:
            return ops.rba_reduce_up4(mask_pred.contiguous(), prob, image_size, want_sem_seg, want_argmax, score)
        up = ops.resample_bilinear(mask_pred.contiguous(), (H, W))
        rba, sem, arg = ops.rba_reduce(up, prob, want_sem_seg, want_argmax, score)
        h, w = image_size
        if (h, w) != (H, W):
            rba = rba[:h, :w].contiguous()
            sem = sem[:, :h, :w].contiguous() if sem is not None else None
            arg = arg[:h, :w].contiguous() if arg is not None else None
        return rba, sem, arg

    @torch.no_grad()
    def panoptic_inference(self, mask_cls, mask_pred, open_panoptic=False, ood_threshold=-0.1, pixel_min=300,
                           return_ood_pred=False):
        Q, H, W = mask_pred.shape
        K = mask_cls.shape[-1] - 1
        prob_all = F.softmax(mask_cls, dim=-1)
        scores, labels = prob_all.max(-1)
        keep = labels.ne(K) & (scores > self.object_mask_threshold)
        panoptic_seg = torch.zeros((H, W), dtype=torch.int32, device=mask_pred.device)
        segments_info = []
        if not bool(keep.any()):
            return panoptic_seg, segments_info
        cur_scores, cur_classes = scores[keep], labels[keep]
        cur_masks = mask_pred[keep].sigmoid()
        cur_mask_ids = (cur_scores.view(-1, 1, 1) * cur_masks).argmax(0)
        current = 0
        stuff_ids = {}
        for k in range(cur_classes.shape[0]):
            cls = int(cur_classes[k])
            won = cur_mask_ids == k
            solid = cur_masks[k] >= 0.5
            mask = won & solid
            mask_area, original_area, inter = int(won.sum()), int(solid.sum()), int(mask.sum())
            if mask_area == 0 or original_area == 0 or inter == 0 or mask_area / original_area < self.overlap_threshold:
                continue
            isthing = cls in self.thing_classes
            if not isthing:
                if cls in stuff_ids:
                    panoptic_seg[mask] = stuff_ids[cls]
                    continue
                stuff_ids[cls] = current + 1
            current += 1
            panoptic_seg[mask] = current
            segments_info.append({"id": current, "isthing": bool(isthing), "category_id": cls})
        if not open_panoptic:
            return panoptic_seg, segments_info
        ood_mask = ops.rba_reduce(mask_pred.contiguous(), prob_all[:, :-1].contiguous())[0]
        comp, n = ops.ood_components(ood_mask, ood_threshold)
        if n:
            free = panoptic_seg == 0
            sizes = torch.bincount(comp[free].long(), minlength=n + 1)
            ok = sizes >= pixel_min
            ok[0] = False
            new_id = current + torch.cumsum(ok.to(torch.int32), 0, dtype=torch.int32)
            sel = free & ok[comp.long()]
            panoptic_seg[sel] = new_id[comp.long()][sel]
            for _ in range(int(ok.sum())):
                current += 1
                segments_info.append({"id": current, "isthing": True, "category_id": 255})
        if return_ood_pred:
            return panoptic_seg, segments_info, ood_mask
        return panoptic_seg, segments_info

    @torch.no_grad()
    def forward(self, batched_inputs, include_void=False, return_separately=False, return_aux=False,
                return_ood_pred=False, return_argmax=False, panoptic_ood_threshold=-0.3, panoptic_pixel_min=200,
                return_panoptic_ood=False, **kwargs):
        if include_void or return_separately or return_aux or kwargs:
            raise NotImplementedError("only the semantic and (open-set) panoptic inference paths of MaskFormer.forward are provided")
        outputs, sizes, padded = self._predict_outputs(batched_inputs)
        mask_cls, mask_pred = outputs["pred_logits"], outputs["pred_masks"]
        ood_pred = None
        if return_ood_pred:
            if "ood_pred" not in outputs:
                raise KeyError("ood_pred: the model has no DenseHybrid head (MODEL.MASK_FORMER.DENSE_HYBRID_LOSS)")
            ood_pred = ops.resample_bilinear_ac(outputs["ood_pred"].contiguous(), sizes[0])
        results = []
        for i, inp in enumerate(batched_inputs):
            height, width = inp.get("height", sizes[i][0]), inp.get("width", sizes[i][1])
            if (height, width) != sizes[i] and self.sem_seg_postprocess_before_inference:
                up = ops.resample_bilinear(mask_pred[i].contiguous(), padded)[:, : sizes[i][0], : sizes[i][1]].contiguous()
                up = ops.resample_bilinear(up, (height, width))
                prob = _class_prob(mask_cls[i])
                rba, sem, arg = ops.rba_reduce(up, prob, True, return_argmax)
            else:
                rba, sem, arg = self._post(mask_cls[i], mask_pred[i], sizes[i], padded, True, return_argmax)
                if (height, width) != sizes[i]:
                    sem = ops.resample_bilinear(sem, (height, width))
                    rba = -sem.tanh().sum(dim=0)
                    arg = sem.argmax(0).to(torch.int32) if return_argmax else None
            r = {"sem_seg": sem, "rba": rba}
            if return_argmax:
                r["argmax"] = arg
            if self.panoptic_on:
                mp = ops.resample_bilinear(mask_pred[i].contiguous(), padded)[:, : sizes[i][0], : sizes[i][1]].contiguous()
                if (height, width) != sizes[i]:
                    mp = ops.resample_bilinear(mp, (height, width))
                r["panoptic_seg"] = self.panoptic_inference(mask_cls[i], mp, self.open_panoptic, panoptic_ood_threshold,
                                                            panoptic_pixel_min, return_panoptic_ood)
            results.append(r)
        if return_ood_pred:
            return results, ood_pred
        return results

    GRAPH_MAX = 8
    GRAPH_THRASH_MAX = 4
    LAUNCH_BOUND_RATIO = 0.95
    GRAPH_REMEASURE_EVERY = 32

    def _replay_state(self):
        return self.__dict__.get("_replay") or self.__dict__.setdefault("_replay", GraphReplay())

    def graph_decisions(self):
        return dict(self._replay_state().decisions)

    def _measured_eager(self, key, batched_inputs, return_argmax, score):
        import time
        dev = self.device
        e0, e1 = torch.cuda.Event(enable_timing=True), torch.cuda.Event(enable_timing=True)
        t0 = time.perf_counter()
        e0.record(torch.cuda.current_stream(dev))
        out = self._rba_scores_eager(batched_inputs, return_argmax, score)
        e1.record(torch.cuda.current_stream(dev))
        self._replay_state().measured(key, time.perf_counter() - t0, e0, e1)
        return out

    def _weights_version(self):
        st = self.__dict__.get("_param_flat")
        gen = _REGISTRATIONS[0]
        if st is None or st[0] != gen:
            flat = list(self.parameters()) + list(self.buffers())
            same = st is not None and len(flat) == len(st[2]) and all(a is b for a, b in zip(flat, st[2]))
            st = self.__dict__["_param_flat"] = [gen, st[1] if same else next(_EPOCHS), flat, st[3] if same else None]
        v = 0
        for t_ in st[2]:
            v += t_._version
        ptrs = [t_.data_ptr() for t_ in st[2]]
        if ptrs != st[3]:
            if st[3] is not None:
                st[1] = next(_EPOCHS)
            st[3] = ptrs
        return st[1], v

    def _graph_key(self, image, return_argmax, score):
        return GraphKey(tuple(image.shape), image.dtype, image.device, torch.cuda.current_stream(image.device).cuda_stream, bool(return_argmax), score,
                        self.fused_upsample, self.fused_front_end, ops.SPLIT_MODE, ops.SPLIT_ACTIVATIONS, ops.TILES_MIN, ops.MLP_FUSED_MIN_ROWS,
                        ops.concurrent_streams(), ops.SWIN_ATTN_FUSED,
                        getattr(self.sem_seg_head.predictor, "sparse_intermediate_heads", None), self._weights_version())

    def drop_graphs(self, release_constants=False):
        if release_constants:
            for m_ in self.modules():
                for v_ in vars(m_).values():
                    if isinstance(v_, ShapeCache):
                        v_.unpin()
        self._replay_state().drop()

    _TRANSIENT = ("_replay", "_param_flat")

    def __getstate__(self):
        st = dict(super().__getstate__() if hasattr(super(), "__getstate__") else self.__dict__)
        for k in self._TRANSIENT:
            st.pop(k, None)
        return st

    def __deepcopy__(self, memo):
        import copy
        cls = self.__class__
        new = cls.__new__(cls)
        memo[id(self)] = new
        for k, v in self.__dict__.items():
            if k not in self._TRANSIENT:
                new.__dict__[k] = copy.deepcopy(v, memo)
        return new

    def _apply(self, fn, *args, **kwargs):
        self.__dict__.pop("_param_flat", None)
        self.drop_graphs(release_constants=True)
        return super()._apply(fn, *args, **kwargs)

    def _graphed_scores(self, image, return_argmax, score):
        state = self._replay_state()
        key = self._graph_key(image, return_argmax, score)
        what = state.step(key, self.graph_replay == "auto", self)
        if what == "measure":
            return key
        if what == "capture":
            try:
                cap = torch.cuda.Stream(device=image.device)
                state.captured(key, *capture(lambda x: self._rba_scores_eager([{"image": x}], return_argmax, score)[0], image, cap), stream=cap)
            except Exception as e:
                import sys
                print(f"[rba_amd] hipGraph capture failed for image shape {tuple(image.shape)} ({type(e).__name__}: {e}); eager launches",
                      file=sys.stderr)
                torch.cuda.synchronize(image.device)
                state.captured(key)
        rec = state.graphs.get(key) if what in ("replay", "capture") else None
        if rec is None or rec.state != "captured":
            return None
        rec.static_in.copy_(image, non_blocking=True)
        rec.graph.replay()
        r = rec.static_out
        return (r[0].clone(), r[1].clone()) if return_argmax else r.clone()

    def live_graphs(self):
        return self._replay_state().live()

    @torch.no_grad()
    def rba_scores(self, batched_inputs, return_argmax=False, score="rba"):
        if (self.graph_replay and len(batched_inputs) == 1 and self.device.type == "cuda"
                and not torch.cuda.is_current_stream_capturing()):
            image = batched_inputs[0]["image"]
            if torch.is_tensor(image) and image.dim() == 3 and image.dtype in (torch.uint8, torch.float32) \
                    and set(batched_inputs[0]) <= {"image"}:
                image = to_device(image, self.device).contiguous()
                batched_inputs = [{"image": image}]
                if self.graph_replay == "auto":
                    fast = self._replay_state().eager_left
                    fk = (tuple(image.shape), image.dtype, bool(return_argmax), score, ops.SPLIT_MODE, torch.cuda.current_stream(image.device).cuda_stream)
                    left = fast.get(fk, 0)
                    if left > 0:
                        fast[fk] = left - 1
                        return self._rba_scores_eager(batched_inputs, return_argmax, score)
                r = self._graphed_scores(image, return_argmax, score)
                if isinstance(r, GraphKey):
                    return self._measured_eager(r, batched_inputs, return_argmax, score)
                if r is not None:
                    return [r]
        return self._rba_scores_eager(batched_inputs, return_argmax, score)

    @torch.no_grad()
    def _rba_scores_eager(self, batched_inputs, return_argmax=False, score="rba"):
        mask_cls, mask_pred, sizes, padded = self.predict(batched_inputs)
        out = []
        for i in range(len(batched_inputs)):
            rba, _, arg = self._post(mask_cls[i], mask_pred[i], sizes[i], padded, False, return_argmax, score)
            out.append((rba, arg) if return_argmax else rba)
        return out
```

### rba_amd/modeling/meta_arch/mask_former_head.py

```python
import torch.nn as nn

from ...registry import SEM_SEG_HEADS_REGISTRY, TRANSFORMER_DECODER_REGISTRY
from ..pixel_decoder import msdeformattn as _pd
from ..transformer_decoder import mask2former_transformer_decoder as _td


@SEM_SEG_HEADS_REGISTRY.register()
class MaskFormerHead(nn.Module):
    def __init__(self, arch, pixel_decoder_name="MSDeformAttnPixelDecoder",
                 transformer_decoder_name="MultiScaleMaskedTransformerDecoder"):
        super().__init__()
        self.num_classes = arch["num_classes"]
        self.pixel_decoder = SEM_SEG_HEADS_REGISTRY.get(pixel_decoder_name)(arch)
        self.predictor = TRANSFORMER_DECODER_REGISTRY.get(transformer_decoder_name)(arch)
        self.transformer_in_feature = "multi_scale_pixel_decoder"

    def _load_from_state_dict(self, state_dict, prefix, *args, **kwargs):
        for k in list(state_dict.keys()):
            if k.startswith(prefix) and not k.startswith(prefix + "predictor") and not k.startswith(prefix + "pixel_decoder"):
                state_dict[k.replace(prefix, prefix + "pixel_decoder.", 1)] = state_dict.pop(k)
        super()._load_from_state_dict(state_dict, prefix, *args, **kwargs)

    def forward(self, features, mask=None):
        return self.layers(features, mask)

    def layers(self, features, mask=None):
        mask_features, _, multi_scale_features = self.pixel_decoder.forward_features(features)
        return self.predictor(multi_scale_features, mask_features, mask)
```

### rba_amd/modeling/pixel_decoder/msdeformattn.py

```python
import os

import torch
import torch.nn as nn
import torch.nn.functional as F

from ... import ops
from ...arch import FEATURE_NAMES, feature_channels, num_fpn_levels
from ...lru import ShapeCache, derived, source_key
from ...registry import SEM_SEG_HEADS_REGISTRY
from ..transformer_decoder.position_encoding import PositionEmbeddingSine
from .ops.ms_deform_attn import MSDeformAttn

FOLD_MASK_FEATURE_NORM = os.environ.get("RBA_MF_GN_FOLD", "1") != "0"


class _LinearView:

    def __init__(self, weight, bias):
        self.weight, self.bias = weight, bias


def _cached_linear_view(mod):
    w, b = mod.weight, mod.bias
    return derived(mod, "linear_view", (w, b), lambda: _LinearView(w.view(w.shape[0], -1), b))


def _conv3x3_planes(mod):
    w = mod.weight
    return derived(mod, ("conv3x3", ops.SPLIT_MODE), (w, mod.bias), lambda: ops.conv3x3_weight(w.detach()))


def _conv1x1_nchw(x, mod):
    B, C, h, w = x.shape
    y = ops.linear(x.permute(0, 2, 3, 1).reshape(B * h * w, C), _cached_linear_view(mod))
    return y.view(B, h, w, -1).permute(0, 3, 1, 2).contiguous()


class ConvNorm(nn.Module):

    def __init__(self, cin, cout, k, bias, norm, relu=False):
        super().__init__()
        self.weight = nn.Parameter(torch.zeros(cout, cin, k, k))
        self.bias = nn.Parameter(torch.zeros(cout)) if bias else None
        self.norm = nn.GroupNorm(32, cout) if norm else None
        self.padding, self.relu = k // 2, relu

    def forward(self, x):
        if self.padding == 0:
            x = _conv1x1_nchw(x, self)
        elif self.weight.shape[1] % 32 == 0:
            y = ops.conv3x3_nhwc(x.permute(0, 2, 3, 1).contiguous(), _conv3x3_planes(self), self.bias, out_features=self.weight.shape[0])
            x = y.permute(0, 3, 1, 2).contiguous()
        else:
            x = F.conv2d(x, self.weight, self.bias, padding=self.padding)
        if self.norm is not None:
            return ops.group_norm(x.contiguous(), 32, self.norm.weight, self.norm.bias, self.norm.eps, relu=self.relu)
        return F.relu(x) if self.relu else x


class MSDeformAttnTransformerEncoderLayer(nn.Module):
    def __init__(self, d_model, d_ffn, n_levels, n_heads, n_points):
        super().__init__()
        self.self_attn = MSDeformAttn(d_model, n_levels, n_heads, n_points)
        self.norm1 = nn.LayerNorm(d_model)
        self.linear1 = nn.Linear(d_model, d_ffn)
        self.linear2 = nn.Linear(d_ffn, d_model)
        self.norm2 = nn.LayerNorm(d_model)

    def forward(self, src, pos, reference_points, spatial_shapes, level_start_index):
        src = self.self_attn(src, reference_points, src, spatial_shapes, level_start_index, query_pos=pos, post=(src, self.norm1))
        hid = ops.linear(src, self.linear1, relu=True)
        N2, K2 = self.linear2.weight.shape
        if ops.token_linear_pays(hid.numel() // K2, N2, K2):
            return ops.token_linear(hid, self.linear2, residual=src, norm=self.norm2)
        src2 = ops.linear(hid, self.linear2, use_bias=False)
        return ops.add_layer_norm(src, self.norm2.weight, self.norm2.bias, self.norm2.eps, src2, self.linear2.bias)[1]


class MSDeformAttnTransformerEncoder(nn.Module):
    def __init__(self, layer_args, num_layers):
        super().__init__()
        self.layers = nn.ModuleList(MSDeformAttnTransformerEncoderLayer(*layer_args) for _ in range(num_layers))

    @staticmethod
    def get_reference_points(spatial_shapes, device):
        refs = []
        for H_, W_ in spatial_shapes:
            ry = (torch.arange(H_, dtype=torch.float32, device=device) + 0.5) / H_
            rx = (torch.arange(W_, dtype=torch.float32, device=device) + 0.5) / W_
            refs.append(torch.stack((rx[None, :].expand(H_, W_), ry[:, None].expand(H_, W_)), -1).reshape(-1, 2))
        ref = torch.cat(refs, 0)[None]
        return ref[:, :, None, :].repeat(1, 1, len(spatial_shapes), 1).contiguous()


class MSDeformAttnTransformerEncoderOnly(nn.Module):
    def __init__(self, d_model, nhead, num_encoder_layers, dim_feedforward, num_feature_levels, enc_n_points):
        super().__init__()
        self.encoder = MSDeformAttnTransformerEncoder(
            (d_model, dim_feedforward, num_feature_levels, nhead, enc_n_points), num_encoder_layers)
        self.level_embed = nn.Parameter(torch.zeros(num_feature_levels, d_model))
        self._ref_cache = ShapeCache(8)
        self._pos_cache = ShapeCache(8)

    def forward(self, srcs, pos_embeds, tokens=None):
        dev = srcs[0].device
        shapes = [tuple(int(v) for v in s.shape[-2:]) for s in srcs]
        B = srcs[0].shape[0]
        if tokens is not None:
            src = tokens[0].contiguous() if len(tokens) == 1 else torch.cat(tokens, 1)
        else:
            src = torch.cat([s.flatten(2).transpose(1, 2) for s in srcs], 1)

        def build_pos():
            p_ = torch.cat([p.flatten(2).transpose(1, 2) + self.level_embed[l].view(1, 1, -1) for l, p in enumerate(pos_embeds)], 1)
            return p_.expand(B, -1, -1).contiguous()

        pos = self._pos_cache.get((tuple(shapes), B, dev, source_key(self.level_embed)), build_pos)

        def build():
            sh_ = torch.as_tensor(shapes, dtype=torch.long, device=dev)
            lsi_ = torch.cat((sh_.new_zeros((1,)), sh_.prod(1).cumsum(0)[:-1]))
            return sh_, lsi_, MSDeformAttnTransformerEncoder.get_reference_points(shapes, dev)

        sh, lsi, ref = self._ref_cache.get((tuple(shapes), dev), build)
        if B > 1:
            ref = ref.expand(B, -1, -1, -1).contiguous()
        out = src
        for layer in self.encoder.layers:
            out = layer(out, pos, ref, sh, lsi)
        return out, shapes


@SEM_SEG_HEADS_REGISTRY.register()
class MSDeformAttnPixelDecoder(nn.Module):
    def __init__(self, arch):
        super().__init__()
        a = arch
        d = a["conv_dim"]
        chans = feature_channels(a)
        self.in_features = list(FEATURE_NAMES)
        self.transformer_in_features = list(a["enc_in"])
        self.transformer_num_feature_levels = len(a["enc_in"])
        self.maskformer_num_feature_levels = len(a["enc_in"])
        self.input_proj = nn.ModuleList(
            nn.Sequential(nn.Conv2d(chans[f], d, kernel_size=1), nn.GroupNorm(32, d)) for f in a["enc_in"][::-1])
        self.transformer = MSDeformAttnTransformerEncoderOnly(
            d, a["nheads"], a["enc_layers"], a["enc_dim_feedforward"], len(a["enc_in"]), a["enc_points"])
        self.pe_layer = PositionEmbeddingSine(d // 2, normalize=True)
        self.mask_features = nn.Conv2d(d, a["mask_dim"], kernel_size=1)
        self.num_fpn_levels = num_fpn_levels(a)
        self.fold_group_norm = os.environ.get("RBA_FOLD_GN", "1") != "0"
        for j in range(1, self.num_fpn_levels + 1):
            self.add_module(f"adapter_{j}", ConvNorm(chans[FEATURE_NAMES[j - 1]], d, 1, bias=False, norm=True))
            self.add_module(f"layer_{j}", ConvNorm(d, d, 3, bias=False, norm=True, relu=True))

    @staticmethod
    def _tokens(x):
        t = x.permute(0, 2, 3, 1)
        return t.reshape(x.shape[0], -1, x.shape[1]) if (x.is_cuda and x.dtype == torch.float32 and t.is_contiguous()) else None

    def _conv1x1(self, tok, mod, use_bias=True):
        lin = _cached_linear_view(mod)
        N, K = lin.weight.shape
        M = tok.numel() // K
        if not ops.split_linear_pays(M, N, K) and ops.token_linear_pays(M, N, K) and tok.is_contiguous():
            return ops.token_linear(tok, lin, use_bias=use_bias)
        return ops.linear(tok, lin, use_bias=use_bias)

    def _channels_last_ok(self, features):
        d = self.mask_features.weight.shape[1]
        if d % 32 or (d // 32) % 4 or 256 % (d // 4) or d > 1024:
            return False
        need = set(self.transformer_in_features) | set(self.in_features[:self.num_fpn_levels])
        return all(self._tokens(features[f]) is not None and features[f].shape[1] % 32 == 0 for f in need)

    def _forward_features_channels_last(self, features):
        srcs, pos, tks = [], [], []
        for idx, f in enumerate(self.transformer_in_features[::-1]):
            x = features[f]
            B, _, h, w = x.shape
            conv, gn = self.input_proj[idx][0], self.input_proj[idx][1]
            y = ops.group_norm_nhwc(self._conv1x1(self._tokens(x), conv), 32, gn.weight, gn.bias, gn.eps)
            tks.append(y.view(B, h * w, -1))
            srcs.append(y.view(B, h, w, -1).permute(0, 3, 1, 2))
            pos.append(self.pe_layer(x))
        y, shapes = self.transformer(srcs, pos, tokens=tks)
        B, d = y.shape[0], y.shape[2]
        toks = [z.contiguous() for z in torch.split(y, [h * w for h, w in shapes], dim=1)]
        outs = [z.view(B, h, w, d).permute(0, 3, 1, 2) for z, (h, w) in zip(toks, shapes)]
        prev, (ph, pw) = toks[-1], shapes[-1]
        prev_norm = None
        fold = self.fold_group_norm
        for idx, f in enumerate(self.in_features[:self.num_fpn_levels][::-1]):
            j = self.num_fpn_levels - idx
            x = features[f]
            h, w = int(x.shape[-2]), int(x.shape[-1])
            ad, ly = getattr(self, f"adapter_{j}"), getattr(self, f"layer_{j}")
            tok = self._tokens(x)
            lat_mr = None
            if fold and tok.is_contiguous() and ops.linear_emits_gn_moments(B * h * w, d, tok.shape[-1], h * w, 32):
                lat, lat_mr = ops.linear_gn_stats(tok, _cached_linear_view(ad), 32, ad.norm.eps, h * w, use_bias=False)
            else:
                lat = self._conv1x1(tok, ad, use_bias=False)
            split = ops.conv3x3_takes_split(B * h * w, d) and d % 32 == 0
            yy = ops.SplitActivations.empty((B, h, w, d), prev.device) if split else None
            if fold:
                if lat_mr is None:
                    lat_mr = ops.group_norm_nhwc_stats(lat, 32, ad.norm.eps)
                ups = []
                for b in range(B):
                    xn = None if prev_norm is None else (prev_norm[0][b], prev_norm[1].weight, prev_norm[1].bias, True)
                    r = ops.resample_bilinear_nhwc_gn(prev[b].view(ph, pw, d), (h, w), lat[b].view(h, w, d), 32, x_norm=xn,
                                                      add_norm=(lat_mr[b], ad.norm.weight, ad.norm.bias), split_into=yy, image=b)
                    if not split:
                        ups.append(r)
                if not split:
                    yy = ups[0][None] if B == 1 else torch.stack(ups)
            else:
                if prev_norm is not None:
                    prev = ops.group_norm_nhwc(prev, 32, prev_norm[1].weight, prev_norm[1].bias, prev_norm[1].eps, relu=True)
                cur = ops.group_norm_nhwc(lat, 32, ad.norm.weight, ad.norm.bias, ad.norm.eps)
                if split:
                    for b in range(B):
                        ops.resample_bilinear_nhwc(prev[b].view(ph, pw, d), (h, w), add=cur[b].view(h, w, d), split_into=yy, image=b)
                else:
                    ups = [ops.resample_bilinear_nhwc(prev[b].view(ph, pw, d), (h, w), add=cur[b].view(h, w, d))
                           for b in range(B)]
                    yy = ups[0][None] if B == 1 else torch.stack(ups)
            planes = _conv3x3_planes(ly)
            last = idx == self.num_fpn_levels - 1
            if fold and split and ops.conv3x3_emits_gn_moments(B, h, w, d, 32):
                prev, mr = ops.conv3x3_nhwc_gn_stats(yy, planes, 32, ly.norm.eps, None, out_features=d)
                prev_norm = (mr, ly.norm)
                prev = prev.view(B, h * w, d)
            else:
                prev = ops.conv3x3_nhwc(yy, planes, None, out_features=d).view(B, h * w, d)
                prev_norm = (ops.group_norm_nhwc_stats(prev, 32, ly.norm.eps) if fold and not last else None, ly.norm)
            ph, pw = h, w
        mfw = self.mask_features.weight
        planes = derived(self.mask_features, ("mf_planes", ops.SPLIT_MODE), (mfw, self.mask_features.bias),
                         lambda: ops.split_weight(mfw.detach().view(mfw.shape[0], -1).contiguous()))
        if prev_norm is not None and fold and FOLD_MASK_FEATURE_NORM and ops.split_linear_nchw_out_takes_gn(planes, ph * pw, d, 32):
            mr = prev_norm[0] if prev_norm[0] is not None else ops.group_norm_nhwc_stats(prev, 32, prev_norm[1].eps)
            mf = ops.split_linear_nchw_out_gn(prev.view(B * ph * pw, d), mr, prev_norm[1].weight, prev_norm[1].bias, 32, True, planes,
                                              self.mask_features.bias, ph * pw, out_features=mfw.shape[0]).view(B, mfw.shape[0], ph, pw)
            return mf, outs[0], outs[:self.maskformer_num_feature_levels]
        if prev_norm is not None:
            prev = ops.group_norm_nhwc(prev, 32, prev_norm[1].weight, prev_norm[1].bias, prev_norm[1].eps, relu=True)
        mf = ops.split_linear_nchw_out(prev.view(B * ph * pw, d), planes, self.mask_features.bias, ph * pw,
                                       out_features=mfw.shape[0]).view(B, mfw.shape[0], ph, pw)
        return mf, outs[0], outs[:self.maskformer_num_feature_levels]

    def forward_features(self, features):
        if self.num_fpn_levels > 0 and self._channels_last_ok(features):
            return self._forward_features_channels_last(features)
        srcs, pos = [], []
        for idx, f in enumerate(self.transformer_in_features[::-1]):
            x = features[f].float().contiguous()
            conv, gn = self.input_proj[idx][0], self.input_proj[idx][1]
            srcs.append(ops.group_norm(_conv1x1_nchw(x, conv), 32, gn.weight, gn.bias, gn.eps))
            pos.append(self.pe_layer(x))
        y, shapes = self.transformer(srcs, pos)
        B = y.shape[0]
        outs = [z.transpose(1, 2).reshape(B, -1, shapes[i][0], shapes[i][1]).contiguous()
                for i, z in enumerate(torch.split(y, [h * w for h, w in shapes], dim=1))]
        for idx, f in enumerate(self.in_features[:self.num_fpn_levels][::-1]):
            j = self.num_fpn_levels - idx
            cur = getattr(self, f"adapter_{j}")(features[f].float().contiguous())
            yy = ops.resample_bilinear(outs[-1], cur.shape[-2:], add=cur.contiguous())
            outs.append(getattr(self, f"layer_{j}")(yy))
        mf = _conv1x1_nchw(outs[-1], self.mask_features)
        return mf, outs[0], outs[:self.maskformer_num_feature_levels]
```

### rba_amd/modeling/transformer_decoder/mask2former_transformer_decoder.py

```python
import contextlib
from types import SimpleNamespace

import torch
import torch.nn as nn
import torch.nn.functional as F
from torch.autograd import Function
from torch.autograd.function import once_differentiable

from ... import ops
from ...lru import ShapeCache, derived, source_key
from ...registry import TRANSFORMER_DECODER_REGISTRY
from .position_encoding import PositionEmbeddingSine


def _qlinear(x, weight, bias=None, relu=False, x_add=None):
    K = x.shape[-1]
    if K % 32:
        raise ops.RbaHipError("query Linears need K % 32 == 0 (hidden_dim 256 in every released architecture)")
    M = x.numel() // K
    x2 = x.contiguous().view(M, K)
    a2 = None if x_add is None else x_add.contiguous().view(M, K)
    if M <= 128:
        return ops.skinny_linear(x2, weight, bias, relu, x_add=a2).view(tuple(x.shape[:-1]) + (weight.shape[0],))
    out = torch.empty((M, weight.shape[0]), dtype=torch.float32, device=x.device)
    for r0 in range(0, M, 128):
        ops.skinny_linear(x2[r0:r0 + 128], weight, bias, relu, x_add=None if a2 is None else a2[r0:r0 + 128], out=out[r0:r0 + 128])
    return out.view(tuple(x.shape[:-1]) + (weight.shape[0],))


class MaskLogitsFunction(Function):

    @staticmethod
    def forward(ctx, embed, feat):
        embed, feat = embed.contiguous(), feat.contiguous()
        need_embed, need_feat = ctx.needs_input_grad[0], ctx.needs_input_grad[1]
        ctx.save_for_backward(embed if need_feat else None, feat if need_embed else None)
        return ops.mask_logits(embed, feat)

    @staticmethod
    @once_differentiable
    def backward(ctx, grad_out):
        embed, feat = ctx.saved_tensors
        need_embed, need_feat = ctx.needs_input_grad[0], ctx.needs_input_grad[1]
        if not (need_embed or need_feat):
            return None, None
        grad_out = grad_out.contiguous()
        return ops.mask_logits_backward(embed, feat, grad_out, need_embed=need_embed, need_feat=need_feat)


class _HeadLayerNormFunction(Function):

    @staticmethod
    def forward(ctx, x, weight, bias, eps):
        ctx.eps = eps
        ctx.save_for_backward(x, weight, bias)
        return ops.add_layer_norm(x, weight, bias, eps)[1]

    @staticmethod
    @once_differentiable
    def backward(ctx, grad_y):
        x, weight, bias = ctx.saved_tensors
        with torch.enable_grad():
            w, b = weight.detach().requires_grad_(True), bias.detach().requires_grad_(True)
            y = F.layer_norm(x, (x.shape[-1],), w, b, ctx.eps)
        gw, gb = torch.autograd.grad(y, (w, b), grad_y)
        return None, gw, gb, None


class _HeadLinearFunction(Function):

    @staticmethod
    def forward(ctx, x, weight, bias, relu):
        y = _qlinear(x, weight, bias, relu)
        ctx.relu = relu
        ctx.save_for_backward(x, weight, y if relu else None)
        return y

    @staticmethod
    @once_differentiable
    def backward(ctx, grad_y):
        x, weight, y = ctx.saved_tensors
        g = grad_y.reshape(-1, grad_y.shape[-1])
        if ctx.relu:
            g = g * (y.reshape(g.shape) > 0)
        gx = (g @ weight).view(x.shape) if ctx.needs_input_grad[0] else None
        gw = g.t() @ x.reshape(-1, x.shape[-1]) if ctx.needs_input_grad[1] else None
        return gx, gw, g.sum(0) if ctx.needs_input_grad[2] else None, None


class _MHAParams(nn.Module):

    def __init__(self, d_model, nhead):
        super().__init__()
        self.embed_dim, self.num_heads = d_model, nhead
        self.in_proj_weight = nn.Parameter(torch.zeros(3 * d_model, d_model))
        self.in_proj_bias = nn.Parameter(torch.zeros(3 * d_model))
        self.out_proj = nn.Linear(d_model, d_model)

    def _kv_views(self):
        w, b, E = self.in_proj_weight, self.in_proj_bias, self.embed_dim
        return derived(self, "kv_views", (w, b),
                       lambda: (SimpleNamespace(weight=w[E:2 * E], bias=b[E:2 * E]), SimpleNamespace(weight=w[2 * E:], bias=b[2 * E:])))

    def forward(self, query, key, value, mask_logits=None, key_add=None, query_add=None):
        E, nH = self.embed_dim, self.num_heads
        B, Q, _ = query.shape
        S = key.shape[1]
        w, b = self.in_proj_weight, self.in_proj_bias
        if (query is key and key is value and key_add is query_add and B * Q <= 128 and E % 32 == 0 and E % 16 == 0
                and w.is_contiguous() and query.is_contiguous()):
            q, k, v = ops.skinny_linear(query, w, b, x_add=None if query_add is None else query_add.contiguous(), add_cols=2 * E, segments=3)
            o = ops.masked_xattn(q.view(B, Q, nH, E // nH), k.view(B, S, nH, E // nH), v.view(B, S, nH, E // nH), mask_logits)
            return _qlinear(o, self.out_proj.weight)
        q = _qlinear(query, w[:E], b[:E], x_add=query_add).view(B, Q, nH, E // nH)
        if (key is value and B * S > 128 and key.is_contiguous() and ops.token_linear_pays(B * S, E, E)
                and (key_add is None or (key_add.is_contiguous() and tuple(key_add.shape) == tuple(key.shape)))):
            lk, lv = self._kv_views()
            k, v = ops.token_linear_multi(key, [(lk, key_add, None, 0, False), (lv, None, None, 0, False)])
            o = ops.masked_xattn(q, k.view(B, S, nH, E // nH), v.view(B, S, nH, E // nH), mask_logits)
            return _qlinear(o, self.out_proj.weight)
        if key_add is not None:
            key = key + key_add
        if B * S > 128:
            lk, lv = self._kv_views()
            k = ops.linear(key.contiguous(), lk).view(B, S, nH, E // nH)
            v = ops.linear(value.contiguous(), lv).view(B, S, nH, E // nH)
            o = ops.masked_xattn(q, k, v, mask_logits)
            return _qlinear(o, self.out_proj.weight)
        k = _qlinear(key, w[E:2 * E], b[E:2 * E]).view(B, S, nH, E // nH)
        v = _qlinear(value, w[2 * E:], b[2 * E:]).view(B, S, nH, E // nH)
        o = ops.masked_xattn(q, k, v, mask_logits)
        return _qlinear(o, self.out_proj.weight)


class SelfAttentionLayer(nn.Module):
    def __init__(self, d_model, nhead):
        super().__init__()
        self.self_attn = _MHAParams(d_model, nhead)
        self.norm = nn.LayerNorm(d_model)

    def forward(self, tgt, query_pos):
        tgt = tgt.contiguous()
        t2 = self.self_attn(tgt, tgt, tgt, key_add=query_pos, query_add=query_pos)
        return ops.add_layer_norm(tgt.contiguous(), self.norm.weight, self.norm.bias, self.norm.eps, t2,
                                  self.self_attn.out_proj.bias)[1]


class CrossAttentionLayer(nn.Module):
    def __init__(self, d_model, nhead):
        super().__init__()
        self.multihead_attn = _MHAParams(d_model, nhead)
        self.norm = nn.LayerNorm(d_model)

    def forward(self, tgt, memory, mask_logits, pos, query_pos):
        t2 = self.multihead_attn(tgt, memory, memory, mask_logits, key_add=pos, query_add=query_pos)
        return ops.add_layer_norm(tgt.contiguous(), self.norm.weight, self.norm.bias, self.norm.eps, t2,
                                  self.multihead_attn.out_proj.bias)[1]


class FFNLayer(nn.Module):
    def __init__(self, d_model, dim_feedforward):
        super().__init__()
        self.linear1 = nn.Linear(d_model, dim_feedforward)
        self.linear2 = nn.Linear(dim_feedforward, d_model)
        self.norm = nn.LayerNorm(d_model)

    def forward(self, tgt):
        t2 = _qlinear(_qlinear(tgt, self.linear1.weight, self.linear1.bias, relu=True), self.linear2.weight)
        return ops.add_layer_norm(tgt.contiguous(), self.norm.weight, self.norm.bias, self.norm.eps, t2,
                                  self.linear2.bias)[1]


class MLP(nn.Module):
    def __init__(self, input_dim, hidden_dim, output_dim, num_layers):
        super().__init__()
        self.num_layers = num_layers
        h = [hidden_dim] * (num_layers - 1)
        self.layers = nn.ModuleList(nn.Linear(n, k) for n, k in zip([input_dim] + h, h + [output_dim]))

    def forward(self, x):
        for i, layer in enumerate(self.layers):
            x = _qlinear(x, layer.weight, layer.bias, relu=i < self.num_layers - 1)
        return x


class BNReluConv(nn.Module):

    def __init__(self, num_maps_in, num_maps_out):
        super().__init__()
        self.norm = nn.BatchNorm2d(num_maps_in, momentum=0.01)
        self.conv = nn.Conv2d(num_maps_in, num_maps_out, kernel_size=1, bias=True)

    def forward(self, x):
        n = self.norm
        scale = n.weight * torch.rsqrt(n.running_var + n.eps)
        shift = n.bias - n.running_mean * scale
        return ops.bn_relu_conv1x1(x.contiguous(), scale.contiguous(), shift.contiguous(),
                                   self.conv.weight.flatten(1).contiguous(), self.conv.bias)


@TRANSFORMER_DECODER_REGISTRY.register()
class MultiScaleMaskedTransformerDecoder(nn.Module):

    differentiable_heads = False

    def __init__(self, arch):
        super().__init__()
        a = arch
        d = a["conv_dim"]
        self.num_heads, self.num_layers = a["nheads"], a["dec_layers"]
        self.num_queries, self.num_feature_levels = a["num_queries"], len(a["enc_in"])
        self.pe_layer = PositionEmbeddingSine(d // 2, normalize=True)
        self.transformer_self_attention_layers = nn.ModuleList(SelfAttentionLayer(d, a["nheads"]) for _ in range(self.num_layers))
        self.transformer_cross_attention_layers = nn.ModuleList(CrossAttentionLayer(d, a["nheads"]) for _ in range(self.num_layers))
        self.transformer_ffn_layers = nn.ModuleList(FFNLayer(d, a["dim_feedforward"]) for _ in range(self.num_layers))
        self.decoder_norm = nn.LayerNorm(d)
        self.query_feat = nn.Embedding(a["num_queries"], d)
        self.query_embed = nn.Embedding(a["num_queries"], d)
        self.level_embed = nn.Embedding(self.num_feature_levels, d)
        self.class_embed = nn.Linear(d, a["num_classes"] + 1)
        self.mask_embed = MLP(d, d, a["mask_dim"], 3)
        self.ood_prediction = bool(a.get("dense_hybrid", False))
        if self.ood_prediction:
            self.ood_pred = BNReluConv(d, 2)
        self.sparse_intermediate_heads = True
        self.cache_initial_heads = True
        self._plan_cache = ShapeCache(8)

    def _load_from_state_dict(self, state_dict, prefix, *args, **kwargs):
        for k in list(state_dict.keys()):
            if k.startswith(prefix) and "static_query" in k:
                state_dict[k.replace("static_query", "query_feat")] = state_dict.pop(k)
        super()._load_from_state_dict(state_dict, prefix, *args, **kwargs)

    def _sparse_plan(self, feat_hw, target_hw, device):
        key = (tuple(feat_hw), tuple(target_hw), device)

        def build():
            (H, W), (h, w) = feat_hw, target_hw
            if not (h > 0 and w > 0 and H % h == 0 and W % w == 0 and (H // h) % 2 == 0 and (W // w) % 2 == 0 and 4 * h * w < H * W):
                return False
            fy, fx = H // h, W // w
            r0 = torch.arange(h, device=device) * fy + fy // 2 - 1
            c0 = torch.arange(w, device=device) * fx + fx // 2 - 1
            idx = [((r0 + dr)[:, None] * W + (c0 + dc)[None, :]).reshape(-1) for dr in (0, 1) for dc in (0, 1)]
            return torch.stack(idx).contiguous()

        plan = self._plan_cache.get(key, build)
        return None if plan is False else plan

    def _query_side_heads(self, output):
        dec = ops.add_layer_norm(output.contiguous(), self.decoder_norm.weight, self.decoder_norm.bias, self.decoder_norm.eps)[1]
        return _qlinear(dec, self.class_embed.weight, self.class_embed.bias), self.mask_embed(dec).contiguous()

    def _query_side_heads_differentiable(self, output):
        n = self.decoder_norm
        dec = _HeadLayerNormFunction.apply(output.detach().contiguous(), n.weight, n.bias, n.eps)
        outputs_class = _HeadLinearFunction.apply(dec, self.class_embed.weight, self.class_embed.bias, False)
        e = dec
        for i, layer in enumerate(self.mask_embed.layers):
            e = _HeadLinearFunction.apply(e, layer.weight, layer.bias, i < self.mask_embed.num_layers - 1)
        return outputs_class, e.contiguous()

    def _initial_query_side(self, B, device):
        ps = [self.query_feat.weight, self.decoder_norm.weight, self.decoder_norm.bias, self.class_embed.weight, self.class_embed.bias]
        for ly in self.mask_embed.layers:
            ps += [ly.weight, ly.bias]
        key = (B, device, source_key(*ps))
        cache = self.__dict__.get("_rba_heads0")
        if cache is None:
            cache = self.__dict__["_rba_heads0"] = ShapeCache(4)
        if key not in cache and torch.cuda.is_current_stream_capturing():
            return None

        def build():
            output = self.query_feat.weight[None].expand(B, -1, -1).contiguous()
            side = self._query_side_heads(output)
            torch.cuda.current_stream(device).synchronize()
            return output, side

        return cache.get(key, build)

    def forward_prediction_heads(self, output, mask_features, attn_mask_target_size, need_attn_mask=True, need_masks=True,
                                 gathered=None, query_side=None):
        if self.differentiable_heads and torch.is_grad_enabled() and need_masks and not need_attn_mask:
            outputs_class, mask_embed = self._query_side_heads_differentiable(output)
            return outputs_class, MaskLogitsFunction.apply(mask_embed, mask_features.detach()), None
        if query_side is not None:
            outputs_class, mask_embed = query_side
        else:
            outputs_class, mask_embed = self._query_side_heads(output)
        plan = None
        if need_attn_mask and not need_masks and self.sparse_intermediate_heads:
            plan = self._sparse_plan(mask_features.shape[-2:], attn_mask_target_size, mask_features.device)
        if plan is not None:
            B, C = mask_features.shape[:2]
            lvl = tuple(attn_mask_target_size)
            gathered = {} if gathered is None else gathered
            if lvl not in gathered:
                gathered[lvl] = mask_features.flatten(2).index_select(2, plan.reshape(-1)).contiguous()
            cols = gathered[lvl]
            v = ops.mask_logits(mask_embed, cols).view(B, -1, 4, plan.shape[1])
            return outputs_class, None, ops.quad_mean(v)
        outputs_mask = ops.mask_logits(mask_embed, mask_features)
        attn_logits = None
        if need_attn_mask:
            attn_logits = ops.resample_bilinear(outputs_mask, attn_mask_target_size).flatten(2)
        return outputs_class, outputs_mask, attn_logits

    def _level_pos(self, x, B):
        cache = self.__dict__.setdefault("_pos_tok_cache", ShapeCache(8))
        key = (tuple(x.shape[-2:]), B, x.device)
        return cache.get(key, lambda: self.pe_layer(x).flatten(2).transpose(1, 2).expand(B, -1, -1).contiguous())

    def forward(self, x, mask_features, mask=None):
        assert len(x) == self.num_feature_levels
        del mask
        frozen = torch.no_grad if self.differentiable_heads and torch.is_grad_enabled() else contextlib.nullcontext
        with frozen():
            output, mask_features, side, predictions_class, predictions_mask = self._decode(x, mask_features)
        cls, msk, _ = self.forward_prediction_heads(output, mask_features, None, need_attn_mask=False, need_masks=True, query_side=side)
        out = {
            "pred_logits": cls,
            "pred_masks": msk,
            "aux_outputs": [({"pred_logits": a, "pred_masks": b} if b is not None else {"pred_logits": a})
                            for a, b in zip(predictions_class, predictions_mask)],
        }
        if self.ood_prediction:
            with frozen():
                out["ood_pred"] = self.ood_pred(mask_features)
        return out

    def _decode(self, x, mask_features):
        src, pos, size_list = [], [], []
        B = x[0].shape[0]
        for i in range(self.num_feature_levels):
            size_list.append(tuple(int(v) for v in x[i].shape[-2:]))
            pos.append(self._level_pos(x[i], B))
            t = x[i].permute(0, 2, 3, 1)
            tok = t.reshape(B, -1, x[i].shape[1]) if t.is_contiguous() else x[i].flatten(2).transpose(1, 2)
            src.append(tok + self.level_embed.weight[i])
        query_embed = self.query_embed.weight[None].expand(B, -1, -1)
        first = self._initial_query_side(B, mask_features.device) if self.cache_initial_heads else None
        if first is not None:
            output, side0 = first
        else:
            output, side0 = self.query_feat.weight[None].expand(B, -1, -1).contiguous(), None
        mask_features = mask_features.contiguous()
        predictions_class, predictions_mask = [], []
        if self.num_layers == 0:
            return output, mask_features, side0, predictions_class, predictions_mask
        gathered = {}
        cls, msk, attn_logits = self.forward_prediction_heads(output, mask_features, size_list[0], True, need_masks=False, gathered=gathered,
                                                              query_side=side0)
        predictions_class.append(cls)
        predictions_mask.append(msk)
        for i in range(self.num_layers):
            li = i % self.num_feature_levels
            output = self.transformer_cross_attention_layers[i](output, src[li], attn_logits, pos[li], query_embed)
            output = self.transformer_self_attention_layers[i](output, query_embed)
            output = self.transformer_ffn_layers[i](output)
            if i == self.num_layers - 1:
                break
            cls, msk, attn_logits = self.forward_prediction_heads(
                output, mask_features, size_list[(i + 1) % self.num_feature_levels], need_attn_mask=True, need_masks=False, gathered=gathered)
            predictions_class.append(cls)
            predictions_mask.append(msk)
        return output, mask_features, None, predictions_class, predictions_mask
```

### rba_amd/ops.py

```python
import contextlib
import ctypes
import threading
import functools
import math
import os

import torch

from . import _lib
from ._lib import RbaHipError
from .lru import derived


def _stream():
    return torch.cuda.current_stream().cuda_stream


def _launch(name, *args, stream=None):
    code = getattr(_lib.load(), name)(*args, torch.cuda.current_stream().cuda_stream if stream is None else stream)
    if code:
        _lib.check(code, name)


def _query(name, *args):
# ... 694 lines not shown
        hl = img.permute(3, 0, 5, 1, 4, 2, 6).reshape(2, Mp, K).float()
        return (hl[0] + hl[1] / 2048.0)[:M].reshape(self.shape)


_SPLIT = threading.local()
_SPLIT_DEFAULT = "f16x3"
"""ops.SPLIT_MODE: arithmetic of the token Linear (K6), PER THREAD (round 5: it was a process global; a re-score on another thread, or a tool
flipping it, changed the kernels of every forward in flight).  Read it as `ops.SPLIT_MODE`, set it for a block with `ops.split_mode(mode)`.  "f16x3": two f16 pieces per operand, three f16 MFMAs per product -- as accurate as an
fp32 GEMM for |x|, |w| < 65504 (beyond f16's range the output is NaN, never silently wrong), twice the speed of "bf16x6": three
bf16 pieces, six MFMAs, fp32's full range."""


def _split_mode():
    return getattr(_SPLIT, "mode", _SPLIT_DEFAULT)


def __getattr__(name):
    if name == "SPLIT_MODE":
        return _split_mode()
    raise AttributeError(f"module {__name__!r} has no attribute {name!r}")


class _OpsModule(type(os)):

    def __setattr__(self, name, value):
        if name == "SPLIT_MODE":
            raise AttributeError('ops.SPLIT_MODE is read-only (the arithmetic mode is per thread): run the block inside `with ops.split_mode("bf16x6"):`')
        super().__setattr__(name, value)


import sys as _sys
_sys.modules[__name__].__class__ = _OpsModule


@_hip_op
def split_weight(weight, mode=None):
    _chk(weight, "weight", dim=2)
    N, K = weight.shape
    if not split_linear_supported(N, K):
        raise RbaHipError("split_weight needs weight [N,K] with K % 32 == 0")
    mode = _split_mode() if mode is None else mode
    if mode not in ("f16x3", "bf16x6"):
        raise RbaHipError(f"unknown split mode {mode!r}")
    f16 = mode == "f16x3"
    packed = torch.empty(((N + 127) // 128, K // 16, 2 if f16 else 3, 128, 2, 8), dtype=torch.float16 if f16 else torch.bfloat16, device=weight.device)
    _launch("rba_split_weight_f16x2" if f16 else "rba_split_weight_bf16x3", _p(weight), _p(packed), N, K)
    return packed


@_hip_op
def unpack_split_weight(packed):
    nt, S, P = packed.shape[:3]
    r = torch.arange(128, device=packed.device)
    flip = ((r >> 3) & 1).bool()
    un = torch.where(flip.view(1, 1, 1, 128, 1, 1), packed.flip(4), packed)
    if P == 2:
        un = un.reshape(nt, S // 2, 2, P, 128, 2, 8).permute(3, 0, 4, 1, 5, 2, 6)
        return un.reshape(P, nt * 128, S * 16)
    return un.permute(2, 0, 3, 1, 4, 5).reshape(3, nt * 128, S * 16)


def split_linear_supported(N, K):
    return K % 32 == 0 and N >= 1 and K >= 32


TILES_MIN = 64


def split_linear_pays(M, N, K, gelu=False):
    if not split_linear_supported(N, K) or K < 64:
        return False
    return _tiles128(M, N) >= TILES_MIN


@_hip_op
def linear(x, lin, use_bias=True, gelu=False, relu=False, residual=None, split_out=False):
    w = lin.weight
    N, K = w.shape
    M = x.numel() // K if K else 0
    bias = lin.bias if use_bias else None
    if isinstance(x, SplitActivations):
        if _split_mode() != "f16x3" or x.shape[-1] != K:
            raise RbaHipError("SplitActivations feed the f16x3 Linear only (check linear_takes_split(M, N, K) before producing them)")
        return split_linear(x, _cached_planes(lin, w), bias, gelu=gelu, out_features=N, relu=relu, residual=residual, split_out=split_out)
    _chk(x, "x") if x.is_contiguous() else _chk(x.contiguous(), "x")
    if split_out:
        if _split_mode() != "f16x3" or not split_linear_supported(N, K):
            raise RbaHipError("linear(split_out=True) needs the f16x3 mode and K % 32 == 0")
        return split_linear(x.contiguous(), _cached_planes(lin, w), bias, gelu=gelu, out_features=N, split_out=True)
    if residual is not None and not linear_residual_fused(M, N, K):
        raise RbaHipError("linear(residual=...) needs the fused f16x3 path: check linear_residual_fused(M, N, K) first")
    if split_linear_supported(N, K):
        return split_linear(x.contiguous(), _cached_planes(lin, w), bias, gelu=gelu, out_features=N, relu=relu, residual=residual)
    Kp = (K + 31) // 32 * 32
    xp = torch.zeros(tuple(x.shape[:-1]) + (Kp,), dtype=torch.float32, device=x.device)
    xp[..., :K] = x
    return split_linear(xp, _cached_planes(lin, w, pad_k=Kp), bias, gelu=gelu, out_features=N, relu=relu)


def _cached_planes(lin, w, pad_k=None):
    def build():
        w2 = w.detach().contiguous()
        if pad_k is not None:
            w2 = torch.nn.functional.pad(w2, (0, pad_k - w2.shape[1]))
        return split_weight(w2)

    return derived(lin, ("planes", _split_mode()), (w,), build, pad_k)


@contextlib.contextmanager
def split_mode(mode):
    if mode not in ("f16x3", "bf16x6"):
        raise RbaHipError(f"unknown split mode {mode!r}")
    prev = _split_mode()
    _SPLIT.mode = mode
    try:
        yield
    finally:
        _SPLIT.mode = prev


SPLIT_ACTIVATIONS = os.environ.get("RBA_SPLIT_ACTIVATIONS", "1") != "0"


SPLIT_MIN_K = int(os.environ.get("RBA_SPLIT_MIN_K", "128"))


def linear_takes_split(M, N, K):
    if not (SPLIT_ACTIVATIONS and _split_mode() == "f16x3" and K >= SPLIT_MIN_K and K % 32 == 0):
        return False
    tiles = _tiles128(M, N)
    return tiles >= 160 or (tiles >= 32 and K % 64 == 0 and K >= 256 and N % 32 == 0)


MLP_FUSED_MIN_ROWS = 32768


def mlp_fused_ok(M, C, hidden):
    return SPLIT_ACTIVATIONS and _split_mode() == "f16x3" and C == 128 and hidden % 32 == 0 and hidden >= 64 and M >= MLP_FUSED_MIN_ROWS


@_hip_op
def mlp_fused(x, fc1, fc2, residual):
    _chk(x, "x")
    _chk(residual, "residual")
    C, hidden = fc1.weight.shape[1], fc1.weight.shape[0]
    M = x.numel() // C
    if (x.shape[-1] != C or tuple(fc2.weight.shape) != (C, hidden) or tuple(residual.shape) != tuple(x.shape) or C != 128 or hidden % 32
            or _split_mode() != "f16x3"):
        raise RbaHipError("mlp_fused needs C == 128, hidden % 32 == 0, matching fc1 / fc2 and the f16x3 mode")
    _launch("rba_swin_mlp_fused_f16x3_f32", _p(x), _p(_cached_planes(fc1, fc1.weight)), _p(fc1.bias), _p(_cached_planes(fc2, fc2.weight)), _p(fc2.bias),
            _p(residual), _p(residual), M, C, hidden)
    return residual


@_hip_op
def mlp_fused_ln(x, norm, fc1, fc2):
    _chk(x, "x")
    g, b, eps = norm
    C, hidden = fc1.weight.shape[1], fc1.weight.shape[0]
    _vec(g, "norm.weight", C)
    _vec(b, "norm.bias", C)
    M = x.numel() // C
    if x.shape[-1] != C or tuple(fc2.weight.shape) != (C, hidden) or C != 128 or hidden % 32 or _split_mode() != "f16x3":
        raise RbaHipError("mlp_fused_ln needs C == 128, hidden % 32 == 0, matching fc1 / fc2 and the f16x3 mode")
    _launch("rba_swin_mlp_fused_ln_f16x3_f32", _p(x), _p(g), _p(b), float(eps), _p(_cached_planes(fc1, fc1.weight)), _p(fc1.bias),
            _p(_cached_planes(fc2, fc2.weight)), _p(fc2.bias), M, C, hidden)
    return x


def linear_residual_fused(M, N, K):
    return _split_mode() == "f16x3" and split_linear_pays(M, N, K)


@_hip_op
def split_linear(x, planes, bias=None, gelu=False, out_features=None, relu=False, residual=None, split_out=False):
    xp, pre = _split_x(x, "split_linear")
    K = x.shape[-1]
    N, f16 = _packed(planes, K, out_features)
    M = x.numel() // K if K else 0
    lead = tuple(x.shape[:-1])
    if not split_linear_supported(N, K):
        raise RbaHipError("split_linear needs x [..., K] and split_weight(W) of a weight [N,K] with K % 32 == 0")
    _vec(bias, "bias", N, optional=True)
    act = 1 if gelu else (2 if relu else 0)
    if split_out:
        if not f16 or act != 1 or residual is not None or N % 32:
            raise RbaHipError("split_out needs f16x3 planes, gelu=True, no residual and N % 32 == 0")
        out = SplitActivations.empty(lead + (N,), x.device)
        _launch("rba_split_linear_f16x3_gelu_split_out", xp, 1 if pre else 0, _p(planes), _p(bias), _p(out.data), M, N, K)
        return out
    if residual is not None:
        _chk(residual, "residual")
        if not f16 or act or tuple(residual.shape) != lead + (N,):
            raise RbaHipError("residual needs f16x3 planes, no activation and a [..., N] tensor")
        if pre:
            _launch("rba_split_linear_f16x3_frag_f32", xp, _p(planes), _p(bias), _p(residual), _p(residual), M, N, K, 0)
        else:
            _launch("rba_split_linear_f16x3_res_f32", xp, _p(planes), _p(bias), _p(residual), _p(residual), M, N, K)
        return residual
    if pre and not f16:
        raise RbaHipError("SplitActivations need f16x3 planes")
    out = torch.empty(lead + (N,), dtype=torch.float32, device=x.device)
    if pre:
        _launch("rba_split_linear_f16x3_frag_f32", xp, _p(planes), _p(bias), 0, _p(out), M, N, K, act)
    else:
        _launch("rba_split_linear_f16x3_f32" if f16 else "rba_split_linear_f32", xp, _p(planes), _p(bias), _p(out), M, N, K, act)
    return out


@_hip_op
def split_linear_nchw_out(x, planes, bias, rows_per_image, out_features=None):
    _chk(x, "x", dim=2)
    M, K = x.shape
    N, f16 = _packed(planes, K, out_features)
    if rows_per_image < 1 or M % rows_per_image:
        raise RbaHipError("split_linear_nchw_out needs x [B*P, K] with M % rows_per_image == 0")
    _vec(bias, "bias", N, optional=True)
    out = torch.empty((M // rows_per_image, N, rows_per_image), dtype=torch.float32, device=x.device)
    _launch("rba_split_linear_nchw_out_f16x3_f32" if f16 else "rba_split_linear_nchw_out_f32", _p(x), _p(planes), _p(bias), _p(out), M, N, K, rows_per_image)
    return out


GN_MOMENTS = os.environ.get("RBA_GN_MOMENTS", "1") != "0"


def _gn_moments_ok(rows_per_image, N, num_groups):
    return (GN_MOMENTS and _split_mode() == "f16x3" and rows_per_image % 128 == 0 and N % 128 == 0 and N % num_groups == 0
            and (N // num_groups) in (4, 8, 16, 32))


def linear_emits_gn_moments(M, N, K, rows_per_image, num_groups):
    return _gn_moments_ok(rows_per_image, N, num_groups) and K <= 256 and K % 32 == 0 and _tiles128(M, N) >= 160 and M % rows_per_image == 0


def conv3x3_emits_gn_moments(B, H, W, N, num_groups):
    return _gn_moments_ok(H * W, N, num_groups) and conv3x3_takes_split(B * H * W, N)


def _merge_gn_moments(moments, B, G, splits, eps):
    mr = torch.empty((B, G, 2), dtype=torch.float32, device=moments.device)
    _launch("rba_group_norm_nhwc_merge_f32", _p(moments), _p(mr), B, G, splits, float(eps))
    return mr


@_hip_op
def linear_gn_stats(x, lin, num_groups, eps, rows_per_image, use_bias=True):
    _chk(x, "x")
    w = lin.weight
    N, K = w.shape
    M = x.numel() // K
    if not linear_emits_gn_moments(M, N, K, rows_per_image, num_groups) or x.shape[-1] != K:
        raise RbaHipError("linear_gn_stats: check linear_emits_gn_moments(M, N, K, rows_per_image, G) first")
    bias = lin.bias if use_bias else None
    planes = _cached_planes(lin, w)
    B, splits = M // rows_per_image, rows_per_image // 128
    out = torch.empty(tuple(x.shape[:-1]) + (N,), dtype=torch.float32, device=x.device)
    mom = torch.empty((B, num_groups, splits, 3), dtype=torch.float32, device=x.device)
    _launch("rba_split_linear_f16x3_gn_moments_f32", _p(x), _p(planes), _p(bias), _p(out), M, N, K, rows_per_image, int(num_groups), _p(mom))
    return out, _merge_gn_moments(mom, B, int(num_groups), splits, eps)


@_hip_op
def conv3x3_nhwc_gn_stats(x, planes, num_groups, eps, bias=None, out_features=None):
    if not isinstance(x, SplitActivations):
        raise RbaHipError("conv3x3_nhwc_gn_stats needs SplitActivations of logical shape [B,H,W,C]")
    xp, _ = _split_x(x, "conv3x3_nhwc_gn_stats", dim=4)
    B, H, W, C = x.shape
    N, _ = _packed(planes, 9 * C, out_features, bf16x6=False)
    if C % 32 or not conv3x3_emits_gn_moments(B, H, W, N, num_groups):
        raise RbaHipError("conv3x3_nhwc_gn_stats: check conv3x3_emits_gn_moments(B, H, W, N, G) first")
    _vec(bias, "bias", N, optional=True)
    splits = H * W // 128
    out = torch.empty((B, H, W, N), dtype=torch.float32, device=x.device)
    mom = torch.empty((B, num_groups, splits, 3), dtype=torch.float32, device=x.device)
    _launch("rba_conv3x3_nhwc_f16x3_split_in_gn_moments_f32", xp, _p(planes), _p(bias), _p(out), B, H, W, C, N, int(num_groups), _p(mom))
    return out, _merge_gn_moments(mom, B, int(num_groups), splits, eps)


def split_linear_nchw_out_takes_gn(planes, rows_per_image, K, num_groups):
    return planes.dtype == torch.float16 and rows_per_image % 128 == 0 and K % num_groups == 0 and (K // num_groups) % 4 == 0 and K % 32 == 0


@_hip_op
def split_linear_nchw_out_gn(x, mr, weight, bias_gn, num_groups, relu, planes, bias, rows_per_image, out_features=None):
    _chk(x, "x", dim=2)
    _chk(mr, "mr", dim=3)
    M, K = x.shape
    N, _ = _packed(planes, K, out_features, bf16x6=False)
    if rows_per_image < 1 or M % rows_per_image or not split_linear_nchw_out_takes_gn(planes, rows_per_image, K, num_groups):
        raise RbaHipError("split_linear_nchw_out_gn needs x [B*P, K], P % 128 == 0 and (K / G) % 4 == 0")
    B = M // rows_per_image
    if tuple(mr.shape) != (B, num_groups, 2):
        raise RbaHipError("mr must be [B, G, 2]")
    _vec(weight, "weight", K)
    _vec(bias_gn, "bias_gn", K)
    _vec(bias, "bias", N, optional=True)
    out = torch.empty((B, N, rows_per_image), dtype=torch.float32, device=x.device)
    _launch("rba_split_linear_nchw_out_gn_f16x3_f32", _p(x), _p(mr), _p(weight), _p(bias_gn), int(num_groups), int(bool(relu)), _p(planes), _p(bias), _p(out),
            M, N, K, rows_per_image)
    return out


@_hip_op
def conv3x3_weight(weight, mode=None):
    _chk(weight, "weight", dim=4)
    N, C, kh, kw = weight.shape
    if (kh, kw) != (3, 3) or C % 32:
        raise RbaHipError("conv3x3_weight needs a [N, C, 3, 3] weight with C % 32 == 0")
    return split_weight(weight.permute(0, 2, 3, 1).reshape(N, 9 * C).contiguous(), mode=mode)


def conv3x3_takes_split(M, N):
    return SPLIT_ACTIVATIONS and _split_mode() == "f16x3" and _tiles128(M, N) >= 256


@_hip_op
def conv3x3_nhwc(x, planes, bias=None, out_features=None):
    xp, pre = _split_x(x, "conv3x3_nhwc", dim=4)
    B, H, W, C = x.shape
    N, f16 = _packed(planes, 9 * C, out_features)
    if C % 32:
        raise RbaHipError("conv3x3_nhwc needs x [B,H,W,C] with C % 32 == 0")
    _vec(bias, "bias", N, optional=True)
    if pre and not (f16 and conv3x3_takes_split(B * H * W, N)):
        raise RbaHipError("conv3x3_nhwc: SplitActivations need f16x3 planes and conv3x3_takes_split(B*H*W, N)")
    out = torch.empty((B, H, W, N), dtype=torch.float32, device=x.device)
    _launch("rba_conv3x3_nhwc_f16x3_split_in_f32" if pre else "rba_conv3x3_nhwc_f16x3_f32" if f16 else "rba_conv3x3_nhwc_f32",
            xp, _p(planes), _p(bias), _p(out), B, H, W, C, N)
    return out


_CONCURRENT_STREAMS = {}


def set_concurrent_streams(n):
    n = max(1, int(n))
    prev = int(_query("rba_set_concurrent_streams", n))
    _CONCURRENT_STREAMS[id(_lib.load())] = n
    return prev


def concurrent_streams():
    return _CONCURRENT_STREAMS.get(id(_lib.load()), 1)


TOKEN_LINEAR = os.environ.get("RBA_TOKEN_LINEAR", "1") != "0"


def token_linear_ok(N, K):
    return TOKEN_LINEAR and _split_mode() == "f16x3" and 1 <= N <= 256 and K >= 32 and K % 32 == 0


TOKEN_MAX_ROWS = 8192


def token_linear_pays(M, N, K):
    return token_linear_ok(N, K) and N % 4 == 0 and 1 <= M <= TOKEN_MAX_ROWS


def _token_planes(lin):
    w = lin.weight

    def build():
        w2 = w.detach().contiguous()
        _chk(w2, "weight", dim=2)
        N, K = w2.shape
        packed = torch.empty((((N + 15) // 16) * (K // 32) * 128, 4), dtype=torch.int32, device=w.device)
        _launch("rba_token_linear_pack_f16x2", _p(w2), _p(packed), N, K)
        return packed

    return derived(lin, "token_planes", (w,), build)


@_hip_op
def token_linear(x, lin, x_add=None, use_bias=True, relu=False, residual=None, norm=None):
    _chk(x, "x")
    N, K = lin.weight.shape
    if x.shape[-1] != K or not token_linear_ok(N, K):
        raise RbaHipError("token_linear: x [..., K] with K % 32 == 0, N <= 256 and the f16x3 mode (see token_linear_ok)")
    M = x.numel() // K
    _shaped(x_add, "x_add", x.shape, optional=True)
    bias = _vec(lin.bias if use_bias else None, "bias", N, optional=True)
    if (residual is None) != (norm is None):
        raise RbaHipError("token_linear: residual and norm come together")
    ln_w, ln_b, ln_eps, act = 0, 0, 0.0, 2 if relu else 0
    if norm is not None:
        _chk(residual, "residual")
        if tuple(residual.shape) != tuple(x.shape[:-1]) + (N,) or N % 16 or relu or norm.weight.numel() != N:
            raise RbaHipError("token_linear(norm=...): residual [..., N], N % 16 == 0, no activation")
        ln_w, ln_b, ln_eps = _p(norm.weight), _p(norm.bias), float(norm.eps)
    out = torch.empty(tuple(x.shape[:-1]) + (N,), dtype=torch.float32, device=x.device)
    _launch("rba_token_linear_f32", _p(x), _p(x_add), _p(_token_planes(lin)), _p(bias), _p(residual), ln_w, ln_b, ln_eps, _p(out), M, N, K, act)
    return out


@_hip_op
def token_linear_multi(x, specs):
    _chk(x, "x")
    K = x.shape[-1]
    M = x.numel() // K if K else 0
    lead = tuple(x.shape[:-1])
    if not 1 <= len(specs) <= 3:
        raise RbaHipError("token_linear_multi: one to three problems")
    arr = (_lib.TokenLinearProblem * len(specs))()
    outs, keep = [], []
    for i, (lin, x_add, out, col0, relu) in enumerate(specs):
        N, K_ = lin.weight.shape
        if K_ != K or not token_linear_ok(N, K) or N % 4:
            raise RbaHipError("token_linear_multi: weights [N <= 256, N % 4 == 0, K] with x's K % 32 == 0 (see token_linear_ok)")
        _shaped(x_add, "x_add", x.shape, optional=True)
        _vec(lin.bias, "bias", N, optional=True)
        if out is None:
            out, col0 = torch.empty(lead + (N,), dtype=torch.float32, device=x.device), 0
        else:
            _chk(out, "out")
            if tuple(out.shape[:-1]) != lead or col0 % 4 or col0 + N > out.shape[-1] or out.shape[-1] % 4:
                raise RbaHipError("token_linear_multi: out [..., ld] with ld % 4 == 0 and a column slice col0 % 4 == 0 inside it")
        planes = _token_planes(lin)
        keep.append(planes)
        arr[i] = _lib.TokenLinearProblem(_p(x_add) or None, _p(planes), _p(lin.bias) or None, out.data_ptr() + 4 * col0, N, out.shape[-1], 2 if relu else 0)
        outs.append(out)
    _launch("rba_token_linear_multi_f32", _p(x), ctypes.byref(arr), len(specs), M, K)
    return outs


@_hip_op
def patch_im2col(image, mean, std, Hp, Wp):
    if image.dtype not in (torch.uint8, torch.float32):
        raise RbaHipError("image must be uint8 or float32")
    _chk(image, "image", dtype=image.dtype, dim=3)
    if image.shape[0] != 3 or Hp % 4 or Wp % 4 or Hp < image.shape[1] or Wp < image.shape[2] or len(mean) != 3 or len(std) != 3:
        raise RbaHipError("patch_im2col needs a [3,h,w] image and Hp >= h, Wp >= w multiples of 4")
    h, w = int(image.shape[1]), int(image.shape[2])
    out = torch.empty(((Hp // 4) * (Wp // 4), 64), dtype=torch.float32, device=image.device)
    m = (ctypes.c_float * 3)(*[float(v) for v in mean])
    sd = (ctypes.c_float * 3)(*[float(v) for v in std])
    _launch("rba_patch_im2col_u8" if image.dtype == torch.uint8 else "rba_patch_im2col_f32", _p(image), _p(out), h, w, int(Hp), int(Wp),
            ctypes.addressof(m), ctypes.addressof(sd))
    return out


def _nhwc_rows(x):
    _chk(x, "x")
    if x.dim() not in (3, 4):
        raise RbaHipError("x must be [B,P,C] or [B,H,W,C]")
    B, C = x.shape[0], x.shape[-1]
    return B, (x.numel() // (B * C) if B * C else 0), C


@_hip_op
def group_norm_nhwc(x, num_groups, weight, bias, eps=1e-5, relu=False):
    B, P, C = _nhwc_rows(x)
    _vec(weight, "weight", C)
    _vec(bias, "bias", C)
    if not _gn_nhwc_ok(C, num_groups):
        raise RbaHipError("group_norm_nhwc needs C % G == 0, (C/G) % 4 == 0, C <= 1024 and 256 % (C/4) == 0")
    ws = _scratch(_query("rba_group_norm_nhwc_workspace_bytes", B, P, C, num_groups), x.device)
    y = torch.empty_like(x)
    _launch("rba_group_norm_nhwc_f32", _p(x), _p(weight), _p(bias), _p(y), _p(ws), B, P, C, num_groups, float(eps), int(bool(relu)))
    return y


@_hip_op
def resample_bilinear_nhwc(x, size, add=None, split_into=None, image=0):
    _chk(x, "x", dim=3)
    h, w, C = x.shape
    H, W = int(size[0]), int(size[1])
    if C % 4:
        raise RbaHipError("resample_bilinear_nhwc needs C % 4 == 0")
    _shaped(add, "add", (H, W, C), optional=True)
    if split_into is not None:
        _split_into_ok(split_into, image, H, W, C)
        _launch("rba_resample_bilinear_nhwc_split_out_f32", _p(x), _p(add), _p(split_into.data), C, h, w, H, W, image * H * W)
        return split_into
    out = torch.empty((H, W, C), dtype=torch.float32, device=x.device)
    _launch("rba_resample_bilinear_nhwc_f32", _p(x), _p(add), _p(out), C, h, w, H, W)
    return out


@_hip_op
def group_norm_nhwc_stats(x, num_groups, eps=1e-5):
    B, P, C = _nhwc_rows(x)
    if not _gn_nhwc_ok(C, num_groups):
        raise RbaHipError("group_norm_nhwc_stats needs C % G == 0, (C/G) % 4 == 0, C <= 1024 and 256 % (C/4) == 0")
    ws = _scratch(_query("rba_group_norm_nhwc_workspace_bytes", B, P, C, num_groups), x.device)
    mr = torch.empty((B, num_groups, 2), dtype=torch.float32, device=x.device)
    _launch("rba_group_norm_nhwc_stats_f32", _p(x), _p(mr), _p(ws), B, P, C, num_groups, float(eps))
    return mr


@_hip_op
def resample_bilinear_nhwc_gn(x, size, add, num_groups, x_norm=None, add_norm=None, split_into=None, image=0):
    _chk(x, "x", dim=3)
    _chk(add, "add", dim=3)
    h, w, C = x.shape
    H, W = int(size[0]), int(size[1])
    if tuple(add.shape) != (H, W, C) or not _gn_nhwc_ok(C, num_groups):
        raise RbaHipError("resample_bilinear_nhwc_gn: add must be [H, W, C]; C % G == 0, (C/G) % 4 == 0")

    def unpack(n, with_relu):
        if n is None:
            return 0, 0, 0, 0
        mr, wgt, b = n[0], n[1], n[2]
        _chk(mr, "mr")
        if mr.numel() != 2 * num_groups:
            raise RbaHipError("norm = (mr [G, 2], weight [C], bias [C])")
        return _p(mr), _p(_vec(wgt, "weight", C)), _p(_vec(b, "bias", C)), (int(bool(n[3])) if with_relu and len(n) > 3 else 0)
    xm, xg, xb, xr = unpack(x_norm, True)
    am, ag, ab, _ = unpack(add_norm, False)
    into = split_into is not None
    if into:
        _split_into_ok(split_into, image, H, W, C)
    out = split_into if into else torch.empty((H, W, C), dtype=torch.float32, device=x.device)
    _launch("rba_resample_bilinear_nhwc_gn_f32", _p(x), xm, xg, xb, xr, _p(add), am, ag, ab, _p(out.data) if into else _p(out), int(into), C, num_groups,
            h, w, H, W, image * H * W if into else 0)
    return out


@_hip_op
def bn_relu_conv1x1(x, scale, shift, weight, bias=None):
    _chk(x, "x")
    if x.dim() < 3:
        raise RbaHipError("x must be [B,C,...]")
    B, C = x.shape[:2]
    _chk(weight, "weight", dim=2)
    O = weight.shape[0]
    P = x.numel() // (B * C) if B * C else 0
    if weight.shape[1] != C or O not in (1, 2, 4):
        raise RbaHipError("bn_relu_conv1x1 needs weight [O,C] with O in {1,2,4}")
    _vec(scale, "scale", C)
    _vec(shift, "shift", C)
    _vec(bias, "bias", O, optional=True)
    out = torch.empty((B, O) + tuple(x.shape[2:]), dtype=torch.float32, device=x.device)
    _launch("rba_bn_relu_conv1x1_f32", _p(x), _p(scale), _p(shift), _p(weight), _p(bias), _p(out), B, C, O, P)
    return out


@_hip_op
def resample_bilinear_ac(x, size):
    _chk(x, "x")
    if x.dim() not in (3, 4):
        raise RbaHipError("x must be [C,h,w] or [B,C,h,w]")
    H, W = int(size[0]), int(size[1])
    lead = tuple(x.shape[:-2])
    h, w = x.shape[-2:]
    out = torch.empty(lead + (H, W), dtype=torch.float32, device=x.device)
    _launch("rba_resample_bilinear_ac_f32", _p(x), _p(out), math.prod(lead), h, w, H, W)
    return out


@_hip_op
def gaussian_blur(score, kernel_size=7, sigma=1.0):
    _chk(score, "score", dim=2)
    H, W = score.shape
    if kernel_size % 2 == 0 or not (1 <= kernel_size <= 15) or sigma <= 0 or (H and W and (H <= kernel_size // 2 or W <= kernel_size // 2)):
        raise RbaHipError("gaussian_blur needs an odd kernel_size <= 15, sigma > 0 and a map larger than the padding")
    out = torch.empty_like(score)
    _launch("rba_gaussian_blur_f32", _p(score), _p(out), H, W, int(kernel_size), float(sigma))
    return out


@_hip_op
def quad_mean(v):
    _chk(v, "v")
    if v.dim() < 2 or v.shape[-2] != 4:
        raise RbaHipError(f"quad_mean expects [..., 4, S], got {tuple(v.shape)}")
    S = v.shape[-1]
    out = torch.empty(v.shape[:-2] + (S,), dtype=torch.float32, device=v.device)
    _launch("rba_quad_mean_f32", _p(v), _p(out), v.numel() // (4 * S) if S else 0, S)
    return out


@_hip_op
def softmax_drop_last(logits):
    _chk(logits, "logits")
    K1 = logits.shape[-1]
    if not 2 <= K1 <= 64:
        raise RbaHipError(f"softmax_drop_last supports 2..64 classes, got {K1}")
    out = torch.empty(logits.shape[:-1] + (K1 - 1,), dtype=torch.float32, device=logits.device)
    _launch("rba_softmax_drop_last_f32", _p(logits), _p(out), logits.numel() // K1, K1)
    return out


@_hip_op
def ood_components(score, threshold, min_dummy=None):
    _chk(score, "score", dim=2)
    H, W = score.shape
    a = torch.empty((H, W), dtype=torch.uint8, device=score.device)
    b = torch.empty_like(a)
    st = _stream()
    _launch("rba_threshold_u8", _p(score), _p(a), H * W, float(threshold), stream=st)
    for dilate, (src, dst) in ((0, (a, b)), (1, (b, a)), (1, (a, b)), (0, (b, a))):
        _launch("rba_morph3x3_u8", _p(src), _p(dst), H, W, dilate, stream=st)
    roots = torch.empty((H, W), dtype=torch.int32, device=score.device)
    _launch("rba_ccl4_roots_i32", _p(a), _p(roots), H, W, stream=st)
    flat = roots.view(-1)
    is_root = flat == torch.arange(H * W, dtype=torch.int32, device=score.device)
    rank = torch.cumsum(is_root.to(torch.int32), 0, dtype=torch.int32)
    labels = torch.where(flat >= 0, rank[flat.clamp_min(0).long()], torch.zeros_like(flat))
    n = int(rank[-1].item()) if H * W else 0
    return labels.view(H, W), n
```

Baseline: 148.1.

## Defer mask-feature projection and compose query embeddings with the conv weight

```diff
diff --git a/include/rba_hip.h b/include/rba_hip.h
--- a/include/rba_hip.h
+++ b/include/rba_hip.h
@@ -156,6 +156,13 @@
                                            const void* weight_packed, const float* bias, float* out, int64_t M, int N, int K,
                                            int rows_per_image, void* stream);
 
+int rba_split_linear_nchw_out_gn_rows_f16x3_f32(const float* x, const float* mr, const float* gamma, const float* beta, int G, int relu,
+                                                const void* weight_packed, int64_t weight_image_stride, const float* bias,
+                                                int bias_image_stride, const int32_t* row_index, float* out, int B, int P, int R, int N,
+                                                int K, void* stream);
+int rba_compose_query_operand_f16x2(const float* embed, const float* weight, const float* bias, void* packed, float* bias_q, int B, int Q,
+                                    int C, int K, void* stream);
+
 int rba_conv3x3_nhwc_f32(const float* x, const void* weight_packed, const float* bias, float* out, int B, int H, int W, int C,
                          int N, void* stream);
 
diff --git a/rba_amd/_lib.py b/rba_amd/_lib.py
--- a/rba_amd/_lib.py
+++ b/rba_amd/_lib.py
@@ -64,6 +64,8 @@
     "rba_conv3x3_nhwc_f16x3_split_in_gn_moments_f32": [_vp, _vp, _vp, _vp, _i, _i, _i, _i, _i, _i, _vp, _vp],
     "rba_group_norm_nhwc_merge_f32": [_vp, _vp, _i, _i, _i, ctypes.c_float, _vp],
     "rba_split_linear_nchw_out_gn_f16x3_f32": [_vp, _vp, _vp, _vp, _i, _i, _vp, _vp, _vp, _i64, _i, _i, _i, _vp],
+    "rba_split_linear_nchw_out_gn_rows_f16x3_f32": [_vp, _vp, _vp, _vp, _i, _i, _vp, _i64, _vp, _i, _vp, _vp, _i, _i, _i, _i, _i, _vp],
+    "rba_compose_query_operand_f16x2": [_vp, _vp, _vp, _vp, _vp, _i, _i, _i, _i, _vp],
     "rba_conv3x3_nhwc_f32": [_vp, _vp, _vp, _vp, _i, _i, _i, _i, _i, _vp],
     "rba_conv3x3_nhwc_f16x3_f32": [_vp, _vp, _vp, _vp, _i, _i, _i, _i, _i, _vp],
     "rba_conv3x3_nhwc_f16x3_split_in_f32": [_vp, _vp, _vp, _vp, _i, _i, _i, _i, _i, _vp],
diff --git a/rba_amd/csrc/split_linear_dma.hip b/rba_amd/csrc/split_linear_dma.hip
--- a/rba_amd/csrc/split_linear_dma.hip
+++ b/rba_amd/csrc/split_linear_dma.hip
@@ -35,6 +35,71 @@
   const unsigned grid = (unsigned)((total + 255) / 256 < 4096 ? (total + 255) / 256 : 4096);
   hipLaunchKernelGGL(split_weight_f16x2_kernel, dim3(grid), dim3(256), 0, (hipStream_t)stream, weight, reinterpret_cast<u32x4_t*>(packed),
                      N, K);
+  return rba_launch_status();
+}
+
+__global__ __launch_bounds__(256) void compose_query_operand_kernel(const float* __restrict__ E, const float* __restrict__ W, const float* __restrict__ bias,
+                                                                    u32x4_t* __restrict__ packed, float* __restrict__ bias_q, int Q, int C, int K) {
+  __shared__ float part[3][64][8];
+  const int S = K >> 4, b = blockIdx.y, tid = threadIdx.x;
+  if ((int)blockIdx.x == S) {
+    if (blockIdx.z == 0 && tid < Q) {
+      const float* e = E + ((int64_t)b * Q + tid) * C;
+      float acc = 0.f;
+      if (bias)
+        for (int c = 0; c < C; ++c) acc = fmaf(e[c], bias[c], acc);
+      bias_q[(int64_t)b * Q + tid] = acc;
+    }
+    return;
+  }
+  const int s = blockIdx.x, lane = tid & 63, chunk = tid >> 6, slot = lane & 1, r = 32 * blockIdx.z + (lane >> 1);
+  const int h = slot ^ ((r >> 3) & 1);
+  const int k0 = 32 * (s >> 1) + 16 * h + 8 * (s & 1);
+  const int CC = ((C + 15) >> 4) << 2;
+  const int c0 = chunk * CC, c1 = c0 + CC < C ? c0 + CC : C;
+  f32x4 lo = {0.f, 0.f, 0.f, 0.f}, hi = {0.f, 0.f, 0.f, 0.f};
+  if (r < Q) {
+    const float* e = E + ((int64_t)b * Q + r) * C;
+    const float* w = W + k0;
+    for (int c = c0; c < c1; c += 4) {
+      const f32x4 e4 = *reinterpret_cast<const f32x4*>(e + c);
+#pragma unroll
+      for (int i = 0; i < 4; ++i) {
+        const f32x4 w0 = *reinterpret_cast<const f32x4*>(w + (int64_t)(c + i) * K), w1 = *reinterpret_cast<const f32x4*>(w + (int64_t)(c + i) * K + 4);
+#pragma unroll
+        for (int j = 0; j < 4; ++j) {
+          lo[j] = fmaf(e4[i], w0[j], lo[j]);
+          hi[j] = fmaf(e4[i], w1[j], hi[j]);
+        }
+      }
+    }
+  }
+  if (chunk > 0) {
+    *reinterpret_cast<f32x4*>(&part[chunk - 1][lane][0]) = lo;
+    *reinterpret_cast<f32x4*>(&part[chunk - 1][lane][4]) = hi;
+  }
+  __syncthreads();
+  if (chunk > 0) return;
+  const f32x4 l1 = *reinterpret_cast<const f32x4*>(&part[0][lane][0]), h1 = *reinterpret_cast<const f32x4*>(&part[0][lane][4]);
+  const f32x4 l2 = *reinterpret_cast<const f32x4*>(&part[1][lane][0]), h2 = *reinterpret_cast<const f32x4*>(&part[1][lane][4]);
+  const f32x4 l3 = *reinterpret_cast<const f32x4*>(&part[2][lane][0]), h3 = *reinterpret_cast<const f32x4*>(&part[2][lane][4]);
+  lo = (lo + l1) + (l2 + l3);
+  hi = (hi + h1) + (h2 + h3);
+  f16x8_t p0, p1;
+  split_h3(lo, hi, p0, p1);
+  u32x4_t* dst = packed + ((int64_t)b * S + s) * 512 + r * 2 + slot;
+  dst[0] = __builtin_bit_cast(u32x4_t, p0);
+  dst[256] = __builtin_bit_cast(u32x4_t, p1);
+}
+
+extern "C" int rba_compose_query_operand_f16x2(const float* embed, const float* weight, const float* bias, void* packed, float* bias_q, int B, int Q, int C,
+                                               int K, void* stream) {
+  RBA_CHECK_ARG(B >= 0 && Q >= 1 && Q <= 128 && C >= 4 && C <= 256 && (C % 4) == 0 && K >= 32 && (K % 32) == 0 && B <= 65535);
+  if (B == 0) return 0;
+  RBA_CHECK_ARG(embed && weight && packed && bias_q && (((uintptr_t)embed | (uintptr_t)weight | (uintptr_t)packed) & 15) == 0);
+  rba_begin();
+  hipLaunchKernelGGL(compose_query_operand_kernel, dim3((unsigned)(K >> 4) + 1, (unsigned)B, 4), dim3(256), 0, (hipStream_t)stream, embed, weight, bias,
+                     reinterpret_cast<u32x4_t*>(packed), bias_q, Q, C, K);
   return rba_launch_status();
 }
 
diff --git a/rba_amd/csrc/split_linear_gnf.hip b/rba_amd/csrc/split_linear_gnf.hip
--- a/rba_amd/csrc/split_linear_gnf.hip
+++ b/rba_amd/csrc/split_linear_gnf.hip
@@ -11,3 +11,23 @@
   a.gn = GnFold{mr, gamma, beta, G, K / G, relu ? 1 : 0};
   return rba_gemm_status(h3_wide(M, N) ? launch_h3l<0, 4, H3_NCHW | H3_GNF>(a) : launch_h3l<0, 2, H3_NCHW | H3_GNF>(a));
 }
+
+extern "C" int rba_split_linear_nchw_out_gn_rows_f16x3_f32(const float* x, const float* mr, const float* gamma, const float* beta, int G, int relu,
+                                                           const void* weight_packed, int64_t weight_image_stride, const float* bias, int bias_image_stride,
+                                                           const int32_t* row_index, float* out, int B, int P, int R, int N, int K, void* stream) {
+  RBA_CHECK_ARG(B >= 0 && N >= 1 && P >= 1 && R >= 1 && G >= 1 && (K % G) == 0 && ((K / G) % 4) == 0);
+  RBA_CHECK_ARG(weight_image_stride >= 0 && (weight_image_stride % 16) == 0 && bias_image_stride >= 0 && (row_index || R == P));
+  const int64_t M = (int64_t)B * R;
+  RBA_GEMM_PROLOGUE(M, K, x && mr && gamma && beta && weight_packed && out && (P % 128) == 0 && (R % 128) == 0 && (int64_t)P * K < (int64_t)1 << 30, x,
+                    weight_packed, out, gamma, beta);
+  H3Args a{x, reinterpret_cast<const u32x4_t*>(weight_packed), bias, out, M, N, K, (hipStream_t)stream};
+  a.rows_per_image = R;
+  a.gn = GnFold{mr, gamma, beta, G, K / G, relu ? 1 : 0};
+  a.rw = H3Rows{row_index, P, bias_image_stride, weight_image_stride};
+  const bool per_image = weight_image_stride != 0 || bias_image_stride != 0, wide = h3_wide(M, N);
+  constexpr unsigned F = H3_NCHW | H3_GNF;
+  if (row_index && per_image) return rba_gemm_status(wide ? launch_h3l<0, 4, F | H3_ROWIDX | H3_PERIMG>(a) : launch_h3l<0, 2, F | H3_ROWIDX | H3_PERIMG>(a));
+  if (row_index) return rba_gemm_status(wide ? launch_h3l<0, 4, F | H3_ROWIDX>(a) : launch_h3l<0, 2, F | H3_ROWIDX>(a));
+  if (per_image) return rba_gemm_status(wide ? launch_h3l<0, 4, F | H3_PERIMG>(a) : launch_h3l<0, 2, F | H3_PERIMG>(a));
+  return rba_gemm_status(wide ? launch_h3l<0, 4, F>(a) : launch_h3l<0, 2, F>(a));
+}
diff --git a/rba_amd/csrc/split_linear_h3.h b/rba_amd/csrc/split_linear_h3.h
--- a/rba_amd/csrc/split_linear_h3.h
+++ b/rba_amd/csrc/split_linear_h3.h
@@ -202,11 +202,13 @@
   H3_OCC1 = 1u << 9,
   H3_KS2 = 1u << 10,
   H3_RS2 = 1u << 11,
+  H3_ROWIDX = 1u << 12,
+  H3_PERIMG = 1u << 13,
   H3_PROBE_SHIFT = 16,
 };
 constexpr unsigned h3_probe(int p) { return (unsigned)p << H3_PROBE_SHIFT; }
 constexpr int h3_probe_of(unsigned form) { return (int)(form >> H3_PROBE_SHIFT); }
-constexpr unsigned H3_FORMS = H3_TIMING | H3_RES, H3L_FORMS = H3_FORMS | H3_GNM | H3_CONV | H3_NCHW | H3_GNF,
+constexpr unsigned H3_FORMS = H3_TIMING | H3_RES, H3L_FORMS = H3_FORMS | H3_GNM | H3_CONV | H3_NCHW | H3_GNF | H3_ROWIDX | H3_PERIMG,
                    H3P_FORMS = H3_FORMS | H3_GNM | H3_PRE | H3_FOUT | H3_CONVP | H3_OCC1 | H3_KS2 | H3_RS2;
 constexpr bool h3_form_within(unsigned form, unsigned allowed) { return (form & ~allowed & ((1u << H3_PROBE_SHIFT) - 1)) == 0; }
 constexpr int h3_tile_rows(unsigned form) { return (form & H3_RS2) ? 256 : 128; }
@@ -354,16 +356,24 @@
   const float* beta;
   int G, cpg, relu;
 };
+struct H3Rows {
+  const int* idx;
+  int P;
+  int bstride;
+  int64_t wstride;
+};
 template <int ACT, int CT, unsigned FORM = 0>
 __global__ __launch_bounds__(256, 2) void split_linear_h3l_kernel(const float* __restrict__ A, const u32x4_t* __restrict__ Wp,
                                                                  const float* __restrict__ bias, float* C, int M, int N,
                                                                  int K, int MT, int NT, unsigned long long* dbg = nullptr,
                                                                  ConvShape cs = ConvShape{0, 0, 0}, const float* R = nullptr, int rows_per_image = 0,
                                                                  GnFold gn = GnFold{nullptr, nullptr, nullptr, 1, 1, 0},
-                                                                 GnMoments gm = GnMoments{nullptr, 1, 1, 128}) {
-  static_assert(h3_form_within(FORM, H3L_FORMS), "split_linear_h3l_kernel: H3_TIMING, H3_RES, H3_GNM, H3_CONV, H3_NCHW, H3_GNF, h3_probe()");
+                                                                 GnMoments gm = GnMoments{nullptr, 1, 1, 128}, H3Rows rw = H3Rows{nullptr, 0, 0, 0}) {
+  static_assert(h3_form_within(FORM, H3L_FORMS), "split_linear_h3l_kernel: H3_TIMING, H3_RES, H3_GNM, H3_CONV, H3_NCHW, H3_GNF, H3_ROWIDX, H3_PERIMG, h3_probe()");
   constexpr int PROBE = h3_probe_of(FORM);
   constexpr bool TIMING = FORM & H3_TIMING, CONV = FORM & H3_CONV, RES = FORM & H3_RES, NCHW = FORM & H3_NCHW, GNF = FORM & H3_GNF, GNM = FORM & H3_GNM;
+  constexpr bool ROWIDX = FORM & H3_ROWIDX, PERIMG = FORM & H3_PERIMG;
+  static_assert(!(ROWIDX || PERIMG) || (NCHW && GNF && !CONV && !RES && !GNM), "H3_ROWIDX / H3_PERIMG: forms of the GroupNorm-folded channel-major projection");
   unsigned long long tm[4];
   if (TIMING) tm[0] = wall_clock64();
   constexpr int BM = 128, BN = 32 * CT;
@@ -387,12 +397,17 @@
 
   constexpr int QSTEP = (CT == 4) ? 256 : 512;
   const char* wbase = reinterpret_cast<const char*>(Wp + (int64_t)(n0 >> 7) * S16 * 512 + (n0 & 127) * 2);
+  const int img = (ROWIDX || PERIMG) ? m0 / rows_per_image : 0;
+  if (PERIMG) {
+    wbase += (int64_t)img * rw.wstride;
+    if (bias) bias += (int64_t)img * rw.bstride;
+  }
   uint32_t woff;
   {
     const int g = tid / SUBW, rem = tid - g * SUBW, p = rem / (2 * BN), rr = rem - p * (2 * BN);
     woff = (uint32_t)(g * 512 + p * 256 + rr) * 16u;
   }
-  const char* xbase = reinterpret_cast<const char*>(CONV ? A : A + (int64_t)m0 * K);
+  const char* xbase = reinterpret_cast<const char*>(CONV ? A : ROWIDX ? A + (int64_t)img * rw.P * K : A + (int64_t)m0 * K);
   uint32_t xoff[4];
   int py[4], px[4];
 #pragma unroll
@@ -404,6 +419,10 @@
       py[q] = pix / cs.W;
       px[q] = pix - py[q] * cs.W;
       xoff[q] = ((uint32_t)r * (uint32_t)cs.Cin + 4u * (tid & 7)) * 4u;
+    } else if (ROWIDX) {
+      int s = rw.idx[r];
+      s = s < 0 ? 0 : (s < rw.P ? s : rw.P - 1);
+      xoff[q] = ((uint32_t)s * (uint32_t)K + 4u * (tid & 7)) * 4u;
     } else {
       xoff[q] = ((uint32_t)(r - m0) * (uint32_t)K + 4u * (tid & 7)) * 4u;
     }
@@ -889,6 +908,7 @@
   GnFold gn = GnFold{nullptr, nullptr, nullptr, 1, 1, 0};
   GnMoments gm = GnMoments{nullptr, 1, 1, 128};
   int stagger = 0;
+  H3Rows rw = H3Rows{nullptr, 0, 0, 0};
 };
 
 inline bool h3_grid(const H3Args& a, int rows, int cols, int& MT, int& NT) {
@@ -912,7 +932,7 @@
   int MT, NT;
   if (!h3_grid(a, 128, 32 * CT, MT, NT)) return (int)hipErrorInvalidValue;
   hipLaunchKernelGGL((split_linear_h3l_kernel<ACT, CT, FORM>), dim3((unsigned)MT * NT), dim3(256), 0, a.stream, reinterpret_cast<const float*>(a.x), a.wp, a.bias,
-                     reinterpret_cast<float*>(a.out), (int)a.M, a.N, a.K, MT, NT, a.dbg, a.cs, a.res, a.rows_per_image, a.gn, a.gm);
+                     reinterpret_cast<float*>(a.out), (int)a.M, a.N, a.K, MT, NT, a.dbg, a.cs, a.res, a.rows_per_image, a.gn, a.gm, a.rw);
   return 0;
 }
 
diff --git a/rba_amd/maskformer_model.py b/rba_amd/maskformer_model.py
--- a/rba_amd/maskformer_model.py
+++ b/rba_amd/maskformer_model.py
@@ -267,7 +267,7 @@
         return GraphKey(tuple(image.shape), image.dtype, image.device, torch.cuda.current_stream(image.device).cuda_stream, bool(return_argmax), score,
                         self.fused_upsample, self.fused_front_end, ops.SPLIT_MODE, ops.SPLIT_ACTIVATIONS, ops.TILES_MIN, ops.MLP_FUSED_MIN_ROWS,
                         ops.concurrent_streams(), ops.SWIN_ATTN_FUSED,
-                        getattr(self.sem_seg_head.predictor, "sparse_intermediate_heads", None), self._weights_version())
+                        (getattr(self.sem_seg_head.predictor, "sparse_intermediate_heads", None), ops.COMPOSED_MASK_HEAD), self._weights_version())
 
     def drop_graphs(self, release_constants=False):
         if release_constants:
diff --git a/rba_amd/modeling/meta_arch/mask_former_head.py b/rba_amd/modeling/meta_arch/mask_former_head.py
--- a/rba_amd/modeling/meta_arch/mask_former_head.py
+++ b/rba_amd/modeling/meta_arch/mask_former_head.py
@@ -25,5 +25,7 @@
         return self.layers(features, mask)
 
     def layers(self, features, mask=None):
-        mask_features, _, multi_scale_features = self.pixel_decoder.forward_features(features)
+        defer = bool(getattr(self.predictor, "takes_deferred_mask_features", False))
+        mask_features, _, multi_scale_features = (self.pixel_decoder.forward_features(features, defer_mask_features=True) if defer
+                                                  else self.pixel_decoder.forward_features(features))
         return self.predictor(multi_scale_features, mask_features, mask)
diff --git a/rba_amd/modeling/pixel_decoder/msdeformattn.py b/rba_amd/modeling/pixel_decoder/msdeformattn.py
--- a/rba_amd/modeling/pixel_decoder/msdeformattn.py
+++ b/rba_amd/modeling/pixel_decoder/msdeformattn.py
@@ -12,6 +12,46 @@
 from .ops.ms_deform_attn import MSDeformAttn
 
 FOLD_MASK_FEATURE_NORM = os.environ.get("RBA_MF_GN_FOLD", "1") != "0"
+
+
+class DeferredMaskFeatures:
+
+    def __init__(self, prev, mr, norm, conv, planes, hw, num_groups=32, relu=True):
+        self.prev, self.mr, self.norm, self.conv, self.planes, self.hw = prev, mr, norm, conv, planes, hw
+        self.num_groups, self.relu = num_groups, relu
+        self.batch = mr.shape[0]
+        self._tensor = None
+
+    @property
+    def shape(self):
+        return torch.Size((self.batch, self.conv.weight.shape[0]) + tuple(self.hw))
+
+    @property
+    def device(self):
+        return self.prev.device
+
+    @property
+    def rows_per_image(self):
+        return self.hw[0] * self.hw[1]
+
+    def _project(self, planes, bias, N, rows=None):
+        return ops.split_linear_nchw_out_gn_rows(self.prev, self.mr, self.norm.weight, self.norm.bias, self.num_groups, self.relu, planes, bias,
+                                                 self.rows_per_image, out_features=N, rows=rows)
+
+    def materialize(self):
+        if self._tensor is None:
+            md = self.conv.weight.shape[0]
+            self._tensor = ops.split_linear_nchw_out_gn(self.prev, self.mr, self.norm.weight, self.norm.bias, self.num_groups, self.relu, self.planes,
+                                                        self.conv.bias, self.rows_per_image, out_features=md).view(self.shape)
+        return self._tensor
+
+    def gather(self, rows):
+        return self._project(self.planes, self.conv.bias, self.conv.weight.shape[0], rows)
+
+    def contract(self, embed):
+        w = self.conv.weight
+        planes, bias_q = ops.compose_query_operand(embed, w.detach().view(w.shape[0], -1), self.conv.bias)
+        return self._project(planes, bias_q, embed.shape[1]).view((self.batch, embed.shape[1]) + tuple(self.hw))
 
 
 class _LinearView:
@@ -174,7 +214,7 @@
         need = set(self.transformer_in_features) | set(self.in_features[:self.num_fpn_levels])
         return all(self._tokens(features[f]) is not None and features[f].shape[1] % 32 == 0 for f in need)
 
-    def _forward_features_channels_last(self, features):
+    def _forward_features_channels_last(self, features, defer_mask_features=False):
         srcs, pos, tks = [], [], []
         for idx, f in enumerate(self.transformer_in_features[::-1]):
             x = features[f]
@@ -242,8 +282,9 @@
                          lambda: ops.split_weight(mfw.detach().view(mfw.shape[0], -1).contiguous()))
         if prev_norm is not None and fold and FOLD_MASK_FEATURE_NORM and ops.split_linear_nchw_out_takes_gn(planes, ph * pw, d, 32):
             mr = prev_norm[0] if prev_norm[0] is not None else ops.group_norm_nhwc_stats(prev, 32, prev_norm[1].eps)
-            mf = ops.split_linear_nchw_out_gn(prev.view(B * ph * pw, d), mr, prev_norm[1].weight, prev_norm[1].bias, 32, True, planes,
-                                              self.mask_features.bias, ph * pw, out_features=mfw.shape[0]).view(B, mfw.shape[0], ph, pw)
+            mf = DeferredMaskFeatures(prev.view(B * ph * pw, d), mr, prev_norm[1], self.mask_features, planes, (ph, pw), num_groups=32, relu=True)
+            if not defer_mask_features:
+                mf = mf.materialize()
             return mf, outs[0], outs[:self.maskformer_num_feature_levels]
         if prev_norm is not None:
             prev = ops.group_norm_nhwc(prev, 32, prev_norm[1].weight, prev_norm[1].bias, prev_norm[1].eps, relu=True)
@@ -251,9 +292,9 @@
                                        out_features=mfw.shape[0]).view(B, mfw.shape[0], ph, pw)
         return mf, outs[0], outs[:self.maskformer_num_feature_levels]
 
-    def forward_features(self, features):
+    def forward_features(self, features, defer_mask_features=False):
         if self.num_fpn_levels > 0 and self._channels_last_ok(features):
-            return self._forward_features_channels_last(features)
+            return self._forward_features_channels_last(features, defer_mask_features)
         srcs, pos = [], []
         for idx, f in enumerate(self.transformer_in_features[::-1]):
             x = features[f].float().contiguous()
diff --git a/rba_amd/modeling/transformer_decoder/mask2former_transformer_decoder.py b/rba_amd/modeling/transformer_decoder/mask2former_transformer_decoder.py
--- a/rba_amd/modeling/transformer_decoder/mask2former_transformer_decoder.py
+++ b/rba_amd/modeling/transformer_decoder/mask2former_transformer_decoder.py
@@ -10,6 +10,7 @@
 from ... import ops
 from ...lru import ShapeCache, derived, source_key
 from ...registry import TRANSFORMER_DECODER_REGISTRY
+from ..pixel_decoder.msdeformattn import DeferredMaskFeatures
 from .position_encoding import PositionEmbeddingSine
 
 
@@ -203,6 +204,7 @@
 class MultiScaleMaskedTransformerDecoder(nn.Module):
 
     differentiable_heads = False
+    takes_deferred_mask_features = True
 
     def __init__(self, arch):
         super().__init__()
@@ -226,6 +228,7 @@
         self.sparse_intermediate_heads = True
         self.cache_initial_heads = True
         self._plan_cache = ShapeCache(8)
+        self._row_cache = ShapeCache(8)
 
     def _load_from_state_dict(self, state_dict, prefix, *args, **kwargs):
         for k in list(state_dict.keys()):
@@ -248,6 +251,34 @@
 
         plan = self._plan_cache.get(key, build)
         return None if plan is False else plan
+
+    def _row_plan(self, feat_hw, target_hw, device, B):
+        key = (tuple(feat_hw), tuple(target_hw), device, B)
+        if key not in self._row_cache and torch.cuda.is_current_stream_capturing():
+            return None
+
+        def build():
+            plan = self._sparse_plan(feat_hw, target_hw, device)
+            if plan is None or plan.numel() % 128:
+                return False
+            rows = ops.row_index(plan.reshape(1, -1).expand(B, -1), feat_hw[0] * feat_hw[1])
+            torch.cuda.current_stream(device).synchronize()
+            return rows
+
+        rows = self._row_cache.get(key, build)
+        return None if rows is False else rows
+
+    def _composed_mask_heads(self, mask_features, size_list):
+        if not (ops.COMPOSED_MASK_HEAD and ops.SPLIT_MODE == "f16x3" and self.sparse_intermediate_heads and not self.ood_prediction):
+            return False
+        md = mask_features.shape[1]
+        if self.num_queries > 128 or md > 256 or md % 4 or mask_features.rows_per_image * mask_features.prev.shape[1] >= 1 << 30:
+            return False
+        levels = {size_list[i % self.num_feature_levels] for i in range(self.num_layers)}
+        rows = [self._row_plan(mask_features.shape[-2:], lvl, mask_features.device, mask_features.shape[0]) for lvl in sorted(levels)]
+        if any(r is None for r in rows):
+            return False
+        return ops.composed_mask_head_pays(mask_features.rows_per_image, sum(r.data.shape[1] for r in rows))
 
     def _query_side_heads(self, output):
         dec = ops.add_layer_norm(output.contiguous(), self.decoder_norm.weight, self.decoder_norm.bias, self.decoder_norm.eps)[1]
@@ -298,10 +329,18 @@
             lvl = tuple(attn_mask_target_size)
             gathered = {} if gathered is None else gathered
             if lvl not in gathered:
-                gathered[lvl] = mask_features.flatten(2).index_select(2, plan.reshape(-1)).contiguous()
+                if isinstance(mask_features, DeferredMaskFeatures):
+                    gathered[lvl] = mask_features.gather(self._row_plan(mask_features.shape[-2:], lvl, mask_features.device, B))
+                else:
+                    gathered[lvl] = mask_features.flatten(2).index_select(2, plan.reshape(-1)).contiguous()
             cols = gathered[lvl]
             v = ops.mask_logits(mask_embed, cols).view(B, -1, 4, plan.shape[1])
             return outputs_class, None, ops.quad_mean(v)
+        if isinstance(mask_features, DeferredMaskFeatures):
+            if need_attn_mask:
+                mask_features = mask_features.materialize()
+            else:
+                return outputs_class, mask_features.contract(mask_embed), None
         outputs_mask = ops.mask_logits(mask_embed, mask_features)
         attn_logits = None
         if need_attn_mask:
@@ -316,7 +355,10 @@
     def forward(self, x, mask_features, mask=None):
         assert len(x) == self.num_feature_levels
         del mask
-        frozen = torch.no_grad if self.differentiable_heads and torch.is_grad_enabled() else contextlib.nullcontext
+        differentiable = self.differentiable_heads and torch.is_grad_enabled()
+        frozen = torch.no_grad if differentiable else contextlib.nullcontext
+        if differentiable and isinstance(mask_features, DeferredMaskFeatures):
+            mask_features = mask_features.materialize()
         with frozen():
             output, mask_features, side, predictions_class, predictions_mask = self._decode(x, mask_features)
         cls, msk, _ = self.forward_prediction_heads(output, mask_features, None, need_attn_mask=False, need_masks=True, query_side=side)
@@ -346,7 +388,10 @@
             output, side0 = first
         else:
             output, side0 = self.query_feat.weight[None].expand(B, -1, -1).contiguous(), None
-        mask_features = mask_features.contiguous()
+        if isinstance(mask_features, DeferredMaskFeatures) and not self._composed_mask_heads(mask_features, size_list):
+            mask_features = mask_features.materialize()
+        if not isinstance(mask_features, DeferredMaskFeatures):
+            mask_features = mask_features.contiguous()
         predictions_class, predictions_mask = [], []
         if self.num_layers == 0:
             return output, mask_features, side0, predictions_class, predictions_mask
diff --git a/rba_amd/ops.py b/rba_amd/ops.py
--- a/rba_amd/ops.py
+++ b/rba_amd/ops.py
@@ -1020,6 +1020,84 @@
     return out
 
 
+COMPOSED_MASK_HEAD = os.environ.get("RBA_COMPOSED_MASK_HEAD", "1") != "0"
+
+
+class RowIndex:
+    __slots__ = ("data", "rows_per_image")
+
+    def __init__(self, data, rows_per_image):
+        self.data, self.rows_per_image = data, rows_per_image
+
+
+def row_index(idx, rows_per_image):
+    if not isinstance(idx, torch.Tensor) or not idx.is_cuda or idx.dtype not in (torch.int32, torch.int64) or idx.dim() != 2 or idx.numel() == 0:
+        raise RbaHipError("row_index needs a HIP int32 / int64 tensor [B, R]")
+    lo, hi = int(idx.min()), int(idx.max())
+    if lo < 0 or hi >= rows_per_image:
+        raise RbaHipError(f"row_index: values must lie in [0, {rows_per_image}), got [{lo}, {hi}]")
+    return RowIndex(idx.to(torch.int32).contiguous(), int(rows_per_image))
+
+
+def _image_planes(planes, K, out_features, B):
+    if planes.dim() != 7:
+        return _packed(planes, K, out_features, bf16x6=False)[0], 0
+    _chk(planes, "planes", dtype=torch.float16, dim=7)
+    if planes.shape[0] != B:
+        raise RbaHipError(f"per-image planes must be [B = {B}, ...], got {tuple(planes.shape)}")
+    return _packed(planes[0], K, out_features, bf16x6=False)[0], planes.stride(0) * 2
+
+
+@_hip_op
+def split_linear_nchw_out_gn_rows(x, mr, weight, bias_gn, num_groups, relu, planes, bias, rows_per_image, out_features=None, rows=None):
+    _chk(x, "x", dim=2)
+    _chk(mr, "mr", dim=3)
+    M, K = x.shape
+    P = int(rows_per_image)
+    if P < 1 or M % P or planes.dtype != torch.float16 or not split_linear_nchw_out_takes_gn(planes, P, K, num_groups) or P * K >= 1 << 30:
+        raise RbaHipError("split_linear_nchw_out_gn_rows needs x [B*P, K], float16 planes, P % 128 == 0, (K / G) % 4 == 0 and P * K < 2^30")
+    B = M // P
+    N, wstride = _image_planes(planes, K, out_features, B)
+    if tuple(mr.shape) != (B, num_groups, 2):
+        raise RbaHipError("mr must be [B, G, 2]")
+    _vec(weight, "weight", K)
+    _vec(bias_gn, "bias_gn", K)
+    bstride = 0
+    if bias is not None and bias.dim() == 2:
+        _shaped(bias, "bias", (B, N))
+        bstride = N
+    else:
+        _vec(bias, "bias", N, optional=True)
+    R = P
+    if rows is not None:
+        if not isinstance(rows, RowIndex) or rows.rows_per_image != P or rows.data.shape[0] != B or rows.data.shape[1] % 128 or rows.data.device != x.device:
+            raise RbaHipError("rows must be ops.row_index(idx [B, R], rows_per_image) for this x, with R % 128 == 0")
+        R = rows.data.shape[1]
+    out = torch.empty((B, N, R), dtype=torch.float32, device=x.device)
+    _launch("rba_split_linear_nchw_out_gn_rows_f16x3_f32", _p(x), _p(mr), _p(weight), _p(bias_gn), int(num_groups), int(bool(relu)), _p(planes), wstride, _p(bias),
+            bstride, _p(None if rows is None else rows.data), _p(out), B, P, R, N, K)
+    return out
+
+
+@_hip_op
+def compose_query_operand(embed, weight, bias):
+    _chk(embed, "embed", dim=3)
+    _chk(weight, "weight", dim=2)
+    B, Q, C = embed.shape
+    K = weight.shape[1]
+    if weight.shape[0] != C or not (1 <= Q <= 128 and 4 <= C <= 256 and C % 4 == 0 and K >= 32 and K % 32 == 0):
+        raise RbaHipError("compose_query_operand needs embed [B, Q <= 128, C <= 256] (C % 4 == 0) and weight [C, K] with K % 32 == 0")
+    _vec(bias, "bias", C, optional=True)
+    planes = torch.empty((B, 1, K // 16, 2, 128, 2, 8), dtype=torch.float16, device=embed.device)
+    bias_q = torch.empty((B, Q), dtype=torch.float32, device=embed.device)
+    _launch("rba_compose_query_operand_f16x2", _p(embed), _p(weight), _p(bias), _p(planes), _p(bias_q), B, Q, C, K)
+    return planes, bias_q
+
+
+def composed_mask_head_pays(rows_per_image, sparse_rows):
+    return 2 * sparse_rows <= rows_per_image
+
+
 @_hip_op
 def conv3x3_weight(weight, mode=None):
     _chk(weight, "weight", dim=4)
```

New measurement: 150.0 (median of 6 runs). 1.3% higher.
